# Woody5962/Ranked-List-Truncation

Hardware: AMD Instinct MI355X
Metric: ranked-lists/sec (fwd+bwd) at len=300; F1@k vs CPU ref (higher is better)
Workload: dtype f32 (operands, accumulation, storage); products by exact 3xbf16 split, 6 MFMA products, per-product error < 2^-23; 1 GPU; AttnCut + DivLoss(js,f1,augmented) [BASELINE configs[1]], batch 4096 lists/GPU x len 300, full train step incl. Adam and cut metrics; global_batch=4096, seq_len=300, parallelism=dp1

## Files before the change

### ranked-list-truncation_amd/csrc/attention6h.hip

```cpp
#include "attention_common.h"
#include "split6.h"
#include <stdlib.h>

namespace {

constexpr int KTH = 64;
constexpr int PLH = KTH * 64;
constexpr int IMGH = 3 * PLH;
constexpr int RECH = IMGH * 2;

__device__ __forceinline__ f32x4 mmh(bf16x8 a, bf16x8 b, f32x4 c) { return __builtin_amdgcn_mfma_f32_16x16x32_bf16(a, b, c, 0, 0, 0); }

__host__ __device__ inline int swz(int row) { return 2 * ((row >> 1) & 3); }

__host__ __device__ inline size_t a6h_img_block(int npair, int ntile) { return (size_t)npair * (ntile + 1) * RECH; }
__global__ __launch_bounds__(256) void attn6h_prepare_kernel(const float* __restrict__ src0, const float* __restrict__ src1, size_t ld,
                                                             int S, int B, int H, uint8_t* __restrict__ img0, uint8_t* __restrict__ img1) {
    const int tid = threadIdx.x, ntile = rlt_cdiv_dev(B, KTH);
    const int pair = blockIdx.x / (ntile + 1), tile = blockIdx.x % (ntile + 1);
    const int s_ = pair / H, h = pair % H;
    const float* base = (blockIdx.y ? src1 : src0) + (size_t)s_ * B * ld + h * 64;
    uint16_t* rec = reinterpret_cast<uint16_t*>((blockIdx.y ? img1 : img0) + ((size_t)pair * (ntile + 1) + tile) * RECH);
    const int r = tid >> 2, row = tile * KTH + r, c0 = 2 * (tid & 3);
    const bool ok = row < B;
    const float* p = base + (size_t)min(row, B - 1) * ld + 8 * c0;
#pragma unroll
    for (int u = 0; u < 2; ++u) {
        const float4 v0 = *reinterpret_cast<const float4*>(p + 8 * u), v1 = *reinterpret_cast<const float4*>(p + 8 * u + 4);
        const float x[8] = {ok ? v0.x : 0.f, ok ? v0.y : 0.f, ok ? v0.z : 0.f, ok ? v0.w : 0.f,
                            ok ? v1.x : 0.f, ok ? v1.y : 0.f, ok ? v1.z : 0.f, ok ? v1.w : 0.f};
        bf16x8 hh_, mm_, ll_;
        split8x3_by_pair(x, hh_, mm_, ll_);
        uint16_t* im = rec + r * 64 + ((c0 + u) ^ swz(r)) * 8;
        *reinterpret_cast<bf16x8*>(im) = hh_;
        *reinterpret_cast<bf16x8*>(im + PLH) = mm_;
        *reinterpret_cast<bf16x8*>(im + 2 * PLH) = ll_;
    }
}

#ifndef RLT_A6H_FWD1_BODY
#define RLT_A6H_FWD1_BODY "attention6h_fwd1_body.inc"
#define RLT_A6H_FWD1_BODY_DROP "attention6h_fwd1_body_drop.inc"
#endif
#ifdef RLT_A6H_STAMPS
__device__ unsigned long long a6h_stamps[4 * 4 * 18];
#define A6H_STAMP(k) do { if (blockIdx.x == 64 && lane == 0 && t >= 8 && t < 12) \
    a6h_stamps[(wv * 4 + (t - 8)) * 18 + (k)] = __builtin_amdgcn_s_memtime(); } while (0)
#else
#define A6H_STAMP(k) do { } while (0)
#endif

template <bool DROP>
__global__ __launch_bounds__(256, 1) void attn6h_fwd1_kernel(AttnArgs a) {
    constexpr int NB = 4;
    extern __shared__ __attribute__((aligned(16))) float smem[];
    uint16_t* img0 = reinterpret_cast<uint16_t*>(smem);
    uint32_t* htab = reinterpret_cast<uint32_t*>(img0 + 4 * IMGH);
    const int tid = threadIdx.x, lane = tid & 63, wv = tid >> 6;
    const int l15 = lane & 15, g = lane >> 4;
    const int B = a.B, H = a.H, E = H * 64;
    const size_t ld = (size_t)3 * E;
    int pair, rt;
    map_block(blockIdx.x, a.S * H, rlt_cdiv_dev(B, 256), pair, rt);
    const int s_ = pair / H, h = pair % H;
    const float* base = a.qkv + (size_t)s_ * B * ld + h * 64;
    const int row0 = rt * 256 + wv * 64;

    int offR[2], offT[4];
    {
        const int swr = swz(l15);
#pragma unroll
        for (int ks = 0; ks < 2; ++ks) offR[ks] = l15 * 64 + (((4 * ks + g) ^ swr) * 8);
        const int rowt = 4 * g + (l15 >> 2), swt = swz(rowt);
#pragma unroll
        for (int db = 0; db < 4; ++db) offT[db] = rowt * 64 + (((2 * db) ^ swt) + ((l15 & 3) >> 1)) * 8 + 4 * (l15 & 1);
    }
    bf16x8 sel[2];
    {
        uint32_t s0[2] = {0u, 0u};
        if ((l15 >> 2) == g) s0[(l15 & 3) >> 1] = (l15 & 1) ? 0xBF800000u : 0x0000BF80u;
        sel[0] = frag4(s0[0], s0[1], 0u, 0u);
        sel[1] = frag4(0u, 0u, s0[0], s0[1]);
    }

    bf16x8 qf[NB][3][2];
    f32x4 seed_s[NB], acc[NB][4], acc2[NB][4];
    float l_run[NB], m_ref[NB];
    uint32_t hq[NB];
    const uint32_t ps = DROP ? pair_seed(a.seed, pair) : 0u;
    const float inv_keep = DROP ? 1.f / (1.f - a.drop_p) : 1.f;
    const float qmul = a.scale * LOG2E;
#pragma unroll
    for (int n = 0; n < NB; ++n) {
        const int r = row0 + 16 * n + l15, rc = min(r, B - 1);
        hq[n] = DROP ? rlt_row_hash(ps, (uint32_t)r) : 0u;
        const float* qp = base + (size_t)rc * ld;
#pragma unroll
        for (int ks = 0; ks < 2; ++ks) {
            const float4 v0 = *reinterpret_cast<const float4*>(qp + 32 * ks + 8 * g), v1 = *reinterpret_cast<const float4*>(qp + 32 * ks + 8 * g + 4);
            const float x[8] = {v0.x * qmul, v0.y * qmul, v0.z * qmul, v0.w * qmul, v1.x * qmul, v1.y * qmul, v1.z * qmul, v1.w * qmul};
            split8x3_by_pair(x, qf[n][0][ks], qf[n][1][ks], qf[n][2][ks]);
        }
#pragma unroll
        for (int db = 0; db < 4; ++db) { acc[n][db] = f32x4{0.f, 0.f, 0.f, 0.f}; acc2[n][db] = f32x4{0.f, 0.f, 0.f, 0.f}; }
        l_run[n] = 0.f;
    }
    const int nt = B / KTH;
    const int npair = a.S * H;
    const uint8_t* rec0 = reinterpret_cast<const uint8_t*>(a.img) + ((size_t)0 * npair + pair) * (size_t)(nt + 1) * RECH;
    const uint8_t* rec1 = reinterpret_cast<const uint8_t*>(a.img) + ((size_t)1 * npair + pair) * (size_t)(nt + 1) * RECH;
    auto dma = [&](int j, int tile, uint16_t* ibuf) __attribute__((always_inline)) {
        const int q = j % 6, grp = q < 4 ? 0 : 4;
        const uint8_t* rec = (j < 6 ? rec0 : rec1) + (size_t)tile * RECH + (6 * wv + grp) * 1024 + lane * 16;
        if (q == grp) {
            const uint32_t dst = __builtin_amdgcn_readfirstlane(
                (uint32_t)(uintptr_t)(__attribute__((address_space(3))) uint8_t*)(reinterpret_cast<uint8_t*>(ibuf) + (j / 6) * RECH + (6 * wv + grp) * 1024));
            asm volatile("s_mov_b32 m0, %0\n\ts_nop 0" :: "s"(dst) : "memory");
        }
        asm volatile("global_load_lds_dwordx4 %0, off offset:%1" :: "v"(rec), "n"((q - grp) * 1024) : "memory");
    };
#pragma unroll
    for (int j = 0; j < 12; ++j) dma(j, 0, img0);
    if (DROP) htab[lane] = rlt_col_hash(ps, (uint32_t)lane);
    asm volatile("s_waitcnt vmcnt(0)" ::: "memory");
    __syncthreads();
#pragma unroll
    for (int n = 0; n < NB; ++n) {
        float tmax = -INFINITY;
#pragma unroll
        for (int kb = 0; kb < 2; ++kb) {
            f32x4 t = {0.f, 0.f, 0.f, 0.f};
#pragma unroll
            for (int p = 0; p < 6; ++p)
#pragma unroll
                for (int ks = 0; ks < 2; ++ks)
                    t = mmh(*reinterpret_cast<const bf16x8*>(img0 + x6_plane_a(p) * PLH + 16 * kb * 64 + offR[ks]), qf[n][x6_plane_b(p)][ks], t);
            tmax = fmaxf(fmaxf(fmaxf(t[0], t[1]), fmaxf(t[2], t[3])), tmax);
        }
        m_ref[n] = col_max4(tmax);
        seed_s[n] = f32x4{-m_ref[n], -m_ref[n], -m_ref[n], -m_ref[n]};
    }

    f32x4 sc[4][2];
    uint32_t pln[3][4][4];
    bf16x8 kf[2][3][2];
    v4s vt[3][4][2];
    uint4 hcv[2][2];
    hcv[0][0] = hcv[0][1] = hcv[1][0] = hcv[1][1] = make_uint4(0u, 0u, 0u, 0u);
#pragma unroll
    for (int i = 0; i < 4; ++i)
#pragma unroll
        for (int kb = 0; kb < 2; ++kb) sc[i][kb] = f32x4{0.f, 0.f, 0.f, 0.f};
#pragma unroll
    for (int i = 0; i < 3 * 4 * 4; ++i) (&pln[0][0][0])[i] = 0u;
#pragma unroll
    for (int i = 0; i < 12; ++i) (&kf[0][0][0])[i] = frag4(0u, 0u, 0u, 0u);
#pragma unroll
    for (int i = 0; i < 24; ++i) (&vt[0][0][0])[i] = v4s{0, 0, 0, 0};

    for (int t = 0; t <= nt; ++t) {
        const int cur = t & 1;
        const uint16_t* Ic = img0 + cur * 2 * IMGH;
        uint16_t* In = img0 + (cur ^ 1) * 2 * IMGH;
        const int t_next = min(t + 1, nt);
        const float livef = t < nt ? 1.f : 0.f;
        const float prevf = t > 0 ? 1.f : 0.f;
#pragma unroll
        for (int n = 0; n < NB; ++n) {
#pragma unroll
            for (int i = 0; i < 6; ++i) asm volatile("" : "+a"((&qf[n][0][0])[i]));
#pragma unroll
            for (int db = 0; db < 4; ++db) asm volatile("" : "+a"(acc[n][db]), "+a"(acc2[n][db]));
        }
        asm volatile("" : "+a"(sel[0]), "+a"(sel[1]));
#define GAP_END __builtin_amdgcn_sched_barrier(0)
        auto mma_va = [&](f32x4& d, bf16x8 av, bf16x8 bv) __attribute__((always_inline)) {
            asm volatile("v_mfma_f32_16x16x32_bf16 %0, %1, %2, %0" : "+v"(d) : "v"(av), "a"(bv));
        };
        auto mma_va_c = [&](f32x4& d, bf16x8 av, bf16x8 bv, const f32x4& cv) __attribute__((always_inline)) {
            asm volatile("v_mfma_f32_16x16x32_bf16 %0, %1, %2, %3" : "=&v"(d) : "v"(av), "a"(bv), "v"(cv));
        };
        auto mma_av = [&](f32x4& d, bf16x8 av, bf16x8 bv) __attribute__((always_inline)) {
            asm volatile("v_mfma_f32_16x16x32_bf16 %0, %1, %2, %0" : "+v"(d) : "a"(av), "v"(bv));
        };
        auto mma_out = [&](f32x4& d, bf16x8 av, bf16x8 bv) __attribute__((always_inline)) {
            asm volatile("v_mfma_f32_16x16x32_bf16 %0, %1, %2, %0" : "+a"(d) : "v"(av), "v"(bv));
        };
        auto m_s = [&](int it, int n, int k) __attribute__((always_inline)) {
            const int kb = k / 12, p = (k % 12) / 2, ks = k % 2;
            if (k % 12 == 0) mma_va_c(sc[it][kb], kf[kb][x6_plane_a(p)][ks], qf[n][x6_plane_b(p)][ks], seed_s[n]);
            else mma_va(sc[it][kb], kf[kb][x6_plane_a(p)][ks], qf[n][x6_plane_b(p)][ks]);
        };
        auto plane = [&](int lvl, int it) __attribute__((always_inline)) {
            return frag4(pln[lvl][it][0], pln[lvl][it][1], pln[lvl][it][2], pln[lvl][it][3]);
        };
        auto m_r = [&](int it, int which, int level, int kb) __attribute__((always_inline)) {
            mma_av(sc[it][kb], sel[kb], plane(level - 1, it));
        };
        auto m_o = [&](int it, int n, int which, int k) __attribute__((always_inline)) {
            const int p = k >> 2, db = k & 3;
            const v4s x = vt[x6_plane_a(p)][db][0], y = vt[x6_plane_a(p)][db][1];
            mma_out(p < 5 ? acc2[n][db] : acc[n][db], cat_frag(x, y), plane(x6_plane_b(p), it));
        };
        auto e_exp = [&](int it, int kb, int r) __attribute__((always_inline)) { sc[it][kb][r] = rlt_exp2(sc[it][kb][r]); };
        auto e_exp_p = [&](int it, int kb, int r) __attribute__((always_inline)) { sc[it][kb][r] = rlt_exp2(sc[it][kb][r]) * prevf; };
        auto e_sum = [&](int it, int n, int kb, int r) __attribute__((always_inline)) { l_run[n] = __builtin_fmaf(sc[it][kb][r], livef, l_run[n]); };
        auto e_sum_p = [&](int it, int n, int kb, int r) __attribute__((always_inline)) { l_run[n] += sc[it][kb][r]; };
        auto c_pk = [&](int it, int which, int lvl, int j) __attribute__((always_inline)) {
            const f32x4& tile = sc[it][j >> 1];
            pln[lvl][it][j] = pk2(tile[2 * (j & 1)], tile[2 * (j & 1) + 1]);
        };
        auto rd_row = [&](int mat, int kb, int pl, int ks, int b32) __attribute__((always_inline)) {
            kf[kb][pl][ks] = *reinterpret_cast<const bf16x8*>(Ic + pl * PLH + (32 * b32 + 16 * kb) * 64 + offR[ks]);
        };
        auto rd_tr = [&](int mat, int pl, int db, int half, int b32) __attribute__((always_inline)) {
            vt[pl][db][half] = tr_read(Ic + IMGH + pl * PLH + (32 * b32 + 16 * half) * 64 + offT[db]);
        };
        auto st_dma = [&](int j) __attribute__((always_inline)) { dma(j, t_next, In); };
        const uint32_t* Hc = htab + cur * KTH;
        auto rd_hc = [&](int fb, int kb, int b32) __attribute__((always_inline)) {
            hcv[fb][kb] = *reinterpret_cast<const uint4*>(Hc + 32 * b32 + 16 * kb + 4 * g);
        };
        auto st_hcol = [&]() __attribute__((always_inline)) {
            htab[(cur ^ 1) * KTH + lane] = rlt_col_hash(ps, (uint32_t)(t_next * KTH + lane));
        };
        auto e_drop = [&](int it, int n, int kb, int r, int fb) __attribute__((always_inline)) {
            const uint4& h4 = hcv[fb][kb];
            const uint32_t hc = r == 0 ? h4.x : r == 1 ? h4.y : r == 2 ? h4.z : h4.w;
            sc[it][kb][r] = rlt_keep_rc(hq[n], hc, a.drop_thr) ? sc[it][kb][r] * inv_keep : 0.f;
        };
        if constexpr (DROP) {
#include RLT_A6H_FWD1_BODY_DROP
        } else {
#include RLT_A6H_FWD1_BODY
        }
#undef GAP_END
        A6H_STAMP(16);
        asm volatile("s_waitcnt vmcnt(0)" ::: "memory");
        __syncthreads();
        A6H_STAMP(17);
    }
    bool bad = false;
    float inv[NB], lse[NB];
#pragma unroll
    for (int n = 0; n < NB; ++n) {
        const float l_tot = col_sum4(l_run[n]);
        bad |= !(l_tot > 0.f && l_tot <= 1.2676506e30f);
        inv[n] = 1.f / l_tot;
        lse[n] = (m_ref[n] + log2f(l_tot)) * LN2;
    }
    const int any_bad = __syncthreads_or(bad ? 1 : 0);
    if (tid == 0 && a.redo) a.redo[blockIdx.x] = any_bad ? 1u : 0u;
#pragma unroll
    for (int n = 0; n < NB; ++n) {
        const int q = row0 + 16 * n + l15;
        if (q < B) {
            float* orow = a.o + ((size_t)s_ * B + q) * E + h * 64 + 4 * g;
#pragma unroll
            for (int db = 0; db < 4; ++db) {
                const f32x4 o = acc[n][db] + acc2[n][db];
                *reinterpret_cast<float4*>(orow + 16 * db) = make_float4(o[0] * inv[n], o[1] * inv[n], o[2] * inv[n], o[3] * inv[n]);
            }
            if (g == 0) a.lse_o[((size_t)s_ * H + h) * B + q] = lse[n];
        }
    }
}

}

#ifdef RLT_A6H_STAMPS
extern "C" int rlt_debug_a6h_stamps(unsigned long long* out) {
    return (int)hipMemcpyFromSymbol(out, HIP_SYMBOL(a6h_stamps), sizeof(unsigned long long) * 4 * 4 * 18);
}
#endif

size_t rlt_attn6h_fwd_images_bytes(int S, int B, int H) { return 2 * a6h_img_block(S * H, rlt_cdiv(B, KTH)); }

int rlt_attn6h_prepare2(int what0, int slot0, int what1, int slot1, const AttnArgs& a, hipStream_t st) {
    const int npair = a.S * a.H, ntile = rlt_cdiv(a.B, KTH), E = a.H * 64;
    uint8_t* img = reinterpret_cast<uint8_t*>(const_cast<void*>(a.img));
    const size_t blk = a6h_img_block(npair, ntile);
    RLT_CHECK_ARG((what0 == 3) == (what1 == 3));
    const float* s0 = what0 == 3 ? a.dout : a.qkv + what0 * E;
    const float* s1 = what1 == 3 ? a.dout : a.qkv + what1 * E;
    hipLaunchKernelGGL(attn6h_prepare_kernel, dim3(npair * (ntile + 1), what1 == what0 && slot1 == slot0 ? 1 : 2), dim3(256), 0, st,
                       s0, s1, what0 == 3 ? (size_t)E : (size_t)3 * E, a.S, a.B, a.H, img + slot0 * blk, img + slot1 * blk);
    return RLT_LAUNCH_RESULT();
}

int rlt_attn6h_run(int which, const AttnArgs& a, hipStream_t st) {
    RLT_CHECK_ARG(which == 0 && a.img && a.redo && a.B % KTH == 0);
    const size_t shm = (size_t)4 * IMGH * sizeof(uint16_t) + 2 * KTH * sizeof(uint32_t);
    const dim3 grid(a.S * a.H * rlt_cdiv(a.B, 256));
    int rc;
    if (a.drop_p > 0.f) {
        if ((rc = rlt_allow_lds(attn6h_fwd1_kernel<true>, shm))) return rc;
        hipLaunchKernelGGL(attn6h_fwd1_kernel<true>, grid, dim3(256), shm, st, a);
    } else {
        if ((rc = rlt_allow_lds(attn6h_fwd1_kernel<false>, shm))) return rc;
        hipLaunchKernelGGL(attn6h_fwd1_kernel<false>, grid, dim3(256), shm, st, a);
    }
    return RLT_LAUNCH_RESULT();
}
```

### ranked-list-truncation_amd/csrc/attention_common.h

```cpp
#pragma once
#include "common.h"

struct AttnArgs {
    const float* qkv; const float* out; const float* dout; const float* lse; const float* delta;
    const void* img; const void* dimg;
    float* o; float* lse_o; float* dqkv;
    int S, B, H;
    float scale;
    float drop_p; uint32_t drop_thr, seed;
    uint32_t* redo;
};

#define RLT_DMA_ASM(dst, src)                                                                                         \
    do {                                                                                                              \
        uint32_t m0_keep_;                                                                                            \
        asm volatile("s_mov_b32 %0, m0\n\ts_mov_b32 m0, %1\n\ts_nop 0\n\tglobal_load_lds_dwordx4 %2, off\n\ts_mov_b32 m0, %0" \
                     : "=&s"(m0_keep_) : "s"(dst), "v"(src) : "memory");                                              \
    } while (0)

namespace {

constexpr int KT = 64;
constexpr int QT = 128;
constexpr float LOG2E = 1.4426950408889634f;
constexpr float LN2 = 0.6931471805599453f;


__device__ __forceinline__ uint32_t pair_seed(uint32_t seed, int pair) { return rlt_mix32(seed ^ ((uint32_t)pair * 0x9E3779B9U)); }

__device__ __forceinline__ void map_block(int bid, int npair, int ntile, int& pair, int& tile) {
    if ((npair & 7) == 0) {
        const int xcd = bid & 7, j = bid >> 3;
        pair = (j / ntile) * 8 + xcd;
        tile = j % ntile;
    } else {
        pair = bid / ntile;
        tile = bid % ntile;
    }
}

template <int HD>
__device__ __forceinline__ void store_acc_T(float* __restrict__ dst_row, int hh, const f32x16 (&acc)[(HD + 31) / 32],
                                            float mul) {
    constexpr int DT = (HD + 31) / 32;
#pragma unroll
    for (int dt = 0; dt < DT; ++dt)
#pragma unroll
        for (int g = 0; g < 4; ++g) {
            const int d0 = dt * 32 + 8 * g + 4 * hh;
            if (d0 < HD) {
                float4 v;
                v.x = acc[dt][4 * g + 0] * mul; v.y = acc[dt][4 * g + 1] * mul;
                v.z = acc[dt][4 * g + 2] * mul; v.w = acc[dt][4 * g + 3] * mul;
                *reinterpret_cast<float4*>(dst_row + d0) = v;
            }
        }
}


}

int rlt_attn_f32_run(int kernel, int which, const AttnArgs& a, int HD, hipStream_t st);
int rlt_attn_delta_run(const float* out, const float* dout, int S, int B, int H, int HD, float* delta, hipStream_t st);
int rlt_attn16_run(int which, const AttnArgs& a, hipStream_t st);
size_t rlt_attn3_images_bytes(int S, int B, int H, int HD, int nmat);
int rlt_attn3_run(int which, const AttnArgs& a, int HD, void* images, void* dimages, hipStream_t st);
size_t rlt_attn6_images_bytes(int S, int B, int H, int HD, int nmat);
int rlt_attn6_prepare(bool dO, const AttnArgs& a, int HD, hipStream_t st);
int rlt_attn6_run(int kernel, int which, const AttnArgs& a, int HD, hipStream_t st);
size_t rlt_attn6n_fwd_images_bytes(int S, int B, int H);
size_t rlt_attn6n_images_bytes(int S, int B, int H);
int rlt_attn6n_prepare_at(int what, int slot, const AttnArgs& a, hipStream_t st);
int rlt_attn6n_prepare(int what, const AttnArgs& a, hipStream_t st);
int rlt_attn6n_run(int kernel, int which, const AttnArgs& a, hipStream_t st);
size_t rlt_attn6h_fwd_images_bytes(int S, int B, int H);
int rlt_attn6h_prepare2(int what0, int slot0, int what1, int slot1, const AttnArgs& a, hipStream_t st);
int rlt_attn6h_run(int which, const AttnArgs& a, hipStream_t st);
```

### ranked-list-truncation_amd/csrc/attention_dispatch.hip

```cpp
#include "attention_plan.h"
#include "attention_common.h"
#include <stdlib.h>
#include <string.h>

namespace {

struct AttnEnv {
    int mode;
    bool attn6;
    bool attn6_img;
    bool attn16;
    bool a6n;
    bool a6n_1;
    bool a6n_img;
    bool a6n_f1;
    bool a6h;
    bool a6_pp;
    bool a6_dkv1;
    bool a6_dq1;
    bool attn_sb;
    bool attn_sb_dq;
    bool dkv_occ1;
};
const AttnEnv& attn_env() {
    static const AttnEnv env = [] {
        auto on = [](const char* e, bool dflt) { return e ? atoi(e) != 0 : dflt; };
        AttnEnv v;
        const char* m = getenv("RLT_ATTN_MODE");
        v.mode = !m ? -1 : (!strcmp(m, "bf16x3") || !strcmp(m, "1")) ? 1 : 0;
        v.attn6 = on(getenv("RLT_ATTN6"), true);
        v.attn6_img = on(getenv("RLT_ATTN6_IMG"), false);
        v.attn16 = on(getenv("RLT_ATTN16"), true);
        v.a6n = on(getenv("RLT_A6N"), true);
        v.a6n_1 = on(getenv("RLT_A6N_1"), true);
        v.a6n_img = on(getenv("RLT_A6N_IMG"), true);
        v.a6n_f1 = on(getenv("RLT_A6N_F1"), true);
        v.a6h = on(getenv("RLT_A6H"), true);
        v.a6_pp = on(getenv("RLT_A6_PP"), true);
        v.a6_dkv1 = on(getenv("RLT_A6_DKV1"), true);
        v.a6_dq1 = on(getenv("RLT_A6_DQ1"), true);
        v.attn_sb = on(getenv("RLT_ATTN_SB"), true);
        v.attn_sb_dq = getenv("RLT_ATTN_SB_DQ") != nullptr;
        const char* o = getenv("RLT_DKV_OCC");
        v.dkv_occ1 = o && atoi(o) == 1;
        return v;
    }();
    return env;
}

bool hd_ok(int HD) { return HD == 16 || HD == 32 || HD == 64 || HD == 128; }
bool drop_ok(float drop_p) { return drop_p >= 0.f && drop_p < 1.f; }
size_t delta_bytes(int S, int B, int H) { return ((size_t)S * H * B * sizeof(float) + 1023) / 1024 * 1024; }
size_t flags_bytes(int S, int B, int H) { return ((size_t)S * H * rlt_cdiv(B, 256) * sizeof(uint32_t) + 255) / 256 * 256; }

}

AttnPlan attn_plan(int S, int B, int H, int HD, float drop_p, bool have_images) {
    const AttnEnv& e = attn_env();
    const int prec = rlt_precision();
    const bool drop = drop_p > 0.f;
    const bool x3 = HD <= 64 && (e.mode >= 0 ? e.mode == 1 : prec == RLT_PRECISION_BF16X3);
    const bool x6 = HD <= 64 && e.mode < 0 && prec == RLT_PRECISION_BF16X6 && e.attn6;
    const bool staged = x6 && e.attn6_img;
    const bool pipe16 = x6 && !staged && HD == 16 && B >= 512 && !drop && e.a6n && e.a6n_1 && e.a6n_img;
    const bool pipe16_fwd = pipe16 && B % 128 == 0 && e.a6n_f1;
    const bool pipe64_fwd = x6 && !staged && HD == 64 && B >= 512 && B % 64 == 0 && e.a6h;

    AttnPlan p{};
    p.delta_bytes = delta_bytes(S, B, H);
    if (x3) {
        p.images_kind = RLT_ATTN_IMAGES_X3_QKV; p.images_bytes = rlt_attn3_images_bytes(S, B, H, HD, 3); p.images_retained = 1;
        p.ws_kind = RLT_ATTN_WS_X3_DO; p.ws_extra_bytes = rlt_attn3_images_bytes(S, B, H, HD, 1);
    } else if (staged) {
        p.images_kind = RLT_ATTN_IMAGES_X6_QKV; p.images_bytes = rlt_attn6_images_bytes(S, B, H, HD, 3); p.images_retained = 1;
        p.ws_kind = RLT_ATTN_WS_X6_DO; p.ws_extra_bytes = rlt_attn6_images_bytes(S, B, H, HD, 1);
    } else {
        if (pipe16_fwd || pipe64_fwd) {
            p.images_kind = pipe16_fwd ? RLT_ATTN_IMAGES_X6N_KV : RLT_ATTN_IMAGES_X6H_KV;
            p.flags_offset = pipe16_fwd ? rlt_attn6n_fwd_images_bytes(S, B, H) : rlt_attn6h_fwd_images_bytes(S, B, H);
            p.flags_bytes = flags_bytes(S, B, H);
            p.images_bytes = p.flags_offset + p.flags_bytes;
        }
        if (pipe16) { p.ws_kind = RLT_ATTN_WS_X6N_BLOCKS; p.ws_extra_bytes = rlt_attn6n_images_bytes(S, B, H); }
    }
    p.ws_bytes = p.delta_bytes + p.ws_extra_bytes;

    const int f32 = HD == 16 && e.attn16 ? RLT_ATTN_F32_HD16 : RLT_ATTN_F32;
    p.fwd = HD == 64 && e.attn_sb ? RLT_ATTN_F32_SB : f32;
    p.dkv = f32 == RLT_ATTN_F32 && (HD == 128 || e.dkv_occ1) ? RLT_ATTN_F32_OCC1 : f32;
    p.dq = HD == 64 && e.attn_sb && e.attn_sb_dq ? RLT_ATTN_F32_SB : f32;
    p.bwd_prepare = RLT_ATTN_PREP_DELTA;
    p.ws_prepare_bytes = p.delta_bytes;
    p.ws_part_bytes = have_images || !x3 ? p.ws_bytes : p.delta_bytes;
    if (x3 && have_images) {
        p.fwd = p.dkv = p.dq = RLT_ATTN_X3;
        p.fwd_prepare = RLT_ATTN_PREP_Q | RLT_ATTN_PREP_K | RLT_ATTN_PREP_V;
        p.bwd_prepare = RLT_ATTN_PREP_DELTA | RLT_ATTN_PREP_DO;
        p.ws_prepare_bytes = p.ws_bytes;
    } else if (x6) {
        const int two_w = staged && have_images ? RLT_ATTN_X6_IMG
                        : HD == 16 && e.a6n ? (B >= 512 ? RLT_ATTN_X6N_2W_SEEDED : RLT_ATTN_X6N_2W) : RLT_ATTN_X6;
        p.fwd = p.dkv = p.dq = two_w;
        if (two_w == RLT_ATTN_X6_IMG) {
            p.fwd_prepare = RLT_ATTN_PREP_Q | RLT_ATTN_PREP_K | RLT_ATTN_PREP_V;
            p.bwd_prepare |= RLT_ATTN_PREP_DO;
            p.ws_prepare_bytes = p.ws_bytes;
        }
        if (HD == 64) {
            const bool small24 = (long long)B * 3 * H * HD < (1ll << 24);
            if (e.a6_pp) p.fwd = two_w == RLT_ATTN_X6_IMG ? RLT_ATTN_X6_PP_IMG : RLT_ATTN_X6_PP;
            if (e.a6_dkv1 && small24) p.dkv = RLT_ATTN_X6_DKV1;
            if (e.a6_dq1 && small24) p.dq = RLT_ATTN_X6_DQ1;
        }
        if (pipe64_fwd && have_images) {
            p.fwd = RLT_ATTN_X6H_PIPE; p.fwd_fixup = RLT_ATTN_X6_PP; p.fwd_prepare = RLT_ATTN_PREP_K | RLT_ATTN_PREP_V;
        }
        if (pipe16_fwd && have_images) {
            p.fwd = RLT_ATTN_X6N_PIPE; p.fwd_fixup = RLT_ATTN_X6N_2W_SEEDED; p.fwd_prepare = RLT_ATTN_PREP_K | RLT_ATTN_PREP_V;
        }
        if (pipe16) {
            p.dkv = p.dq = RLT_ATTN_X6N_PIPE;
            p.bwd_prepare |= RLT_ATTN_PREP_DO | RLT_ATTN_PREP_SEEDS;
            p.dkv_prepare = RLT_ATTN_PREP_Q;
            p.dq_prepare = RLT_ATTN_PREP_K | RLT_ATTN_PREP_V;
            p.ws_prepare_bytes = p.ws_bytes;
        }
    }
    return p;
}

namespace {

int run_kernel(int kernel, int which, const AttnArgs& a, int HD, void* images, void* dimages, hipStream_t st) {
    switch (kernel) {
    case RLT_ATTN_F32: case RLT_ATTN_F32_SB: case RLT_ATTN_F32_OCC1: return rlt_attn_f32_run(kernel, which, a, HD, st);
    case RLT_ATTN_F32_HD16: return rlt_attn16_run(which, a, st);
    case RLT_ATTN_X3: return rlt_attn3_run(which, a, HD, images, dimages, st);
    case RLT_ATTN_X6: case RLT_ATTN_X6_IMG: case RLT_ATTN_X6_PP: case RLT_ATTN_X6_PP_IMG: case RLT_ATTN_X6_DKV1: case RLT_ATTN_X6_DQ1:
        return rlt_attn6_run(kernel, which, a, HD, st);
    case RLT_ATTN_X6N_2W: case RLT_ATTN_X6N_2W_SEEDED: case RLT_ATTN_X6N_PIPE: return rlt_attn6n_run(kernel, which, a, st);
    case RLT_ATTN_X6H_PIPE: return rlt_attn6h_run(which, a, st);
    }
    return RLT_E_ARG;
}

int bwd_prepare(const float* out, const float* dout, const float* lse, int S, int B, int H, int HD,
                const void* images, void* ws, size_t ws_bytes, float drop_p, void* stream) {
    RLT_CHECK_ARG(out && dout && lse && ws && S > 0 && B > 0 && H > 0 && drop_ok(drop_p));
    RLT_CHECK_SHAPE(hd_ok(HD));
    const AttnPlan p = attn_plan(S, B, H, HD, drop_p, images != nullptr);
    if (ws_bytes < p.ws_prepare_bytes) return RLT_E_WORKSPACE;
    if (!rlt_aligned16(ws)) return RLT_E_ALIGN;
    hipStream_t st = rlt_stream(stream);
    uint8_t* extra = (uint8_t*)ws + p.delta_bytes;
    AttnArgs a{};
    a.dout = dout; a.lse = lse; a.delta = (const float*)ws; a.S = S; a.B = B; a.H = H;
    if (p.dkv == RLT_ATTN_X3) {
        a.o = const_cast<float*>(out);
        a.drop_p = drop_p;
        return rlt_attn3_run(3, a, HD, nullptr, extra, st);
    }
    int rc = rlt_attn_delta_run(out, dout, S, B, H, HD, (float*)ws, st);
    if (!rc && (p.bwd_prepare & RLT_ATTN_PREP_DO)) {
        if (p.ws_kind == RLT_ATTN_WS_X6_DO) { a.dimg = extra; rc = rlt_attn6_prepare(true, a, HD, st); }
        else { a.img = extra; rc = rlt_attn6n_prepare(3, a, st); }
    }
    if (!rc && (p.bwd_prepare & RLT_ATTN_PREP_SEEDS)) rc = rlt_attn6n_prepare(4, a, st);
    return rc;
}

int bwd_part(int which, const float* qkv, const float* dout, const float* lse, const void* images, void* ws, size_t ws_bytes,
             int S, int B, int H, int HD, float drop_p, uint32_t seed, float* dqkv, void* stream) {
    RLT_CHECK_ARG(qkv && dout && lse && ws && dqkv && S > 0 && B > 0 && H > 0 && drop_ok(drop_p));
    RLT_CHECK_SHAPE(hd_ok(HD));
    if (!(rlt_aligned16(qkv) && rlt_aligned16(dout) && rlt_aligned16(dqkv) && rlt_aligned16(ws))) return RLT_E_ALIGN;
    const AttnPlan p = attn_plan(S, B, H, HD, drop_p, images != nullptr);
    if (ws_bytes < p.ws_part_bytes) return RLT_E_WORKSPACE;
    const int kernel = which == 1 ? p.dkv : p.dq, prepare = which == 1 ? p.dkv_prepare : p.dq_prepare;
    uint8_t* extra = (uint8_t*)ws + p.delta_bytes;
    AttnArgs a{};
    a.qkv = qkv; a.dout = dout; a.lse = lse; a.delta = (const float*)ws; a.dqkv = dqkv;
    a.S = S; a.B = B; a.H = H;
    a.scale = 1.0f / sqrtf((float)HD);
    a.drop_p = drop_p; a.drop_thr = rlt_drop_threshold(drop_p); a.seed = seed;
    if (kernel == RLT_ATTN_X6_IMG) { a.img = images; a.dimg = extra; }
    if (kernel == RLT_ATTN_X6N_PIPE) a.img = extra;
    hipStream_t st = rlt_stream(stream);
    int rc = 0;
    for (int what = 0; what < 3 && !rc; ++what)
        if (prepare & (1 << what)) rc = rlt_attn6n_prepare(what, a, st);
    return rc ? rc : run_kernel(kernel, which, a, HD, const_cast<void*>(images), extra, st);
}

}

extern "C" {

int rlt_list_attention_plan(int S, int B, int H, int HD, float drop_p, int have_images, int precision, rlt_attention_plan* out) {
    RLT_PREC_SCOPE(precision);
    RLT_CHECK_ARG(out && S > 0 && B > 0 && H > 0 && drop_ok(drop_p));
    RLT_CHECK_SHAPE(hd_ok(HD));
    *out = attn_plan(S, B, H, HD, drop_p, have_images != 0);
    return 0;
}

size_t rlt_list_attention_fwd_workspace(int S, int B, int H, int HD, float drop_p, int precision) {
    RLT_PREC_SCOPE_SZ(precision);
    if (S <= 0 || B <= 0 || H <= 0 || !hd_ok(HD)) return 0;
    return attn_plan(S, B, H, HD, drop_p, true).images_bytes;
}

int rlt_list_attention_images_retained(int S, int B, int H, int HD, int precision) {
    RLT_PREC_SCOPE_SZ(precision);
    if (S <= 0 || B <= 0 || H <= 0 || !hd_ok(HD)) return 0;
    return attn_plan(S, B, H, HD, 0.f, true).images_retained;
}

int rlt_list_attention_fwd(const float* qkv, int S, int B, int H, int HD, float drop_p, uint32_t seed,
                           float* out, float* lse, void* images, size_t images_bytes, int precision, void* stream) {
    RLT_PREC_SCOPE(precision);
    RLT_CHECK_ARG(qkv && out && lse && S > 0 && B > 0 && H > 0 && drop_ok(drop_p));
    RLT_CHECK_SHAPE(hd_ok(HD));
    if (!(rlt_aligned16(qkv) && rlt_aligned16(out))) return RLT_E_ALIGN;
    AttnPlan p = attn_plan(S, B, H, HD, drop_p, images != nullptr);
    if (p.fwd_prepare && p.images_retained) {
        if (images_bytes < p.images_bytes) return RLT_E_WORKSPACE;
        if (!rlt_aligned16(images)) return RLT_E_ALIGN;
    } else if (p.fwd_prepare && !(rlt_aligned16(images) && images_bytes >= p.images_bytes)) {
        p = attn_plan(S, B, H, HD, drop_p, false);
    }
    AttnArgs a{};
    a.qkv = qkv; a.o = out; a.lse_o = lse; a.S = S; a.B = B; a.H = H;
    a.scale = 1.0f / sqrtf((float)HD);
    a.drop_p = drop_p; a.drop_thr = rlt_drop_threshold(drop_p); a.seed = seed;
    if (p.fwd_prepare) a.img = images;
    if (p.fwd_fixup) a.redo = reinterpret_cast<uint32_t*>(reinterpret_cast<uint8_t*>(images) + p.flags_offset);
    hipStream_t st = rlt_stream(stream);
    int rc = 0;
    switch (p.fwd) {
    case RLT_ATTN_X6_IMG: case RLT_ATTN_X6_PP_IMG: rc = rlt_attn6_prepare(false, a, HD, st); break;
    case RLT_ATTN_X6N_PIPE: rc = rlt_attn6n_prepare_at(1, 0, a, st); if (!rc) rc = rlt_attn6n_prepare_at(2, 1, a, st); break;
    case RLT_ATTN_X6H_PIPE: rc = rlt_attn6h_prepare2(1, 0, 2, 1, a, st); break;
    }
    if (!rc) rc = run_kernel(p.fwd, 0, a, HD, images, nullptr, st);
    if (!rc && p.fwd_fixup) rc = run_kernel(p.fwd_fixup, 0, a, HD, nullptr, nullptr, st);
    return rc;
}

size_t rlt_list_attention_bwd_workspace(int S, int B, int H, int HD, float drop_p, int precision) {
    RLT_PREC_SCOPE_SZ(precision);
    if (S <= 0 || B <= 0 || H <= 0 || !hd_ok(HD)) return 0;
    return attn_plan(S, B, H, HD, drop_p, true).ws_bytes;
}

int rlt_list_attention_bwd_prepare(const float* out, const float* dout, const float* lse, int S, int B, int H, int HD, float drop_p,
                                   const void* images, void* ws, size_t ws_bytes, int precision, void* stream) {
    RLT_PREC_SCOPE(precision);
    return bwd_prepare(out, dout, lse, S, B, H, HD, images, ws, ws_bytes, drop_p, stream);
}

int rlt_list_attention_bwd_dkv(const float* qkv, const float* dout, const float* lse, const void* images, void* ws, size_t ws_bytes,
                               int S, int B, int H, int HD, float drop_p, uint32_t seed, float* dqkv, int precision, void* stream) {
    RLT_PREC_SCOPE(precision);
    return bwd_part(1, qkv, dout, lse, images, ws, ws_bytes, S, B, H, HD, drop_p, seed, dqkv, stream);
}

int rlt_list_attention_bwd_dq(const float* qkv, const float* dout, const float* lse, const void* images, void* ws, size_t ws_bytes,
                              int S, int B, int H, int HD, float drop_p, uint32_t seed, float* dqkv, int precision, void* stream) {
    RLT_PREC_SCOPE(precision);
    return bwd_part(2, qkv, dout, lse, images, ws, ws_bytes, S, B, H, HD, drop_p, seed, dqkv, stream);
}

int rlt_list_attention_bwd(const float* qkv, const float* out, const float* dout, const float* lse,
                           int S, int B, int H, int HD, float drop_p, uint32_t seed, const void* images, float* dqkv,
                           void* ws, size_t ws_bytes, int precision, void* stream) {
    RLT_PREC_SCOPE(precision);
    RLT_CHECK_ARG(drop_ok(drop_p));
    int rc = bwd_prepare(out, dout, lse, S, B, H, HD, images, ws, ws_bytes, drop_p, stream);
    if (!rc) rc = bwd_part(1, qkv, dout, lse, images, ws, ws_bytes, S, B, H, HD, drop_p, seed, dqkv, stream);
    if (!rc) rc = bwd_part(2, qkv, dout, lse, images, ws, ws_bytes, S, B, H, HD, drop_p, seed, dqkv, stream);
    return rc;
}

}
```

### ranked-list-truncation_amd/csrc/gemm.hip

```cpp
#include "common.h"
#include "gemm6s.h"
#include "gemm_plan.h"
#include "split6.h"
#include <type_traits>

namespace {

constexpr int BM = 128, BN = 128, LDT = 132;

struct GemmArgs {
    const float* A; const float* B; float* C;
    const float* bias; const float* bias2;
    int M, N, K, lda, ldb, ldc;
    int vecA, vecB;
    int flags;
    int kchunk;
    float* slab;
    int tiles_m, tiles_n;
    const float* mask; int ldmask;
    float* colsum;
    float* cs_slab;
    float drop_p; uint32_t drop_thr, seed;
    float mask_scale;
    int slab_xcd;
// ... 1414 lines not shown
            vals6e<BKC>(vb, p, a, b, c, d);
            split4x3<true>(a, b, c, d, hi, mid, lo);
            *reinterpret_cast<uint2*>(wb + dB[p]) = hi;
            *reinterpret_cast<uint2*>(wb + dB[p] + HB6) = mid;
            *reinterpret_cast<uint2*>(wb + dB[p] + 2 * HB6) = lo;
        }
    };
    bf16x8 a[4][3], b[2][3];
    auto frag_a = [&](const uint16_t* base, int i, int q) { a[i][q] = *reinterpret_cast<const bf16x8*>(base + arow + q * HB6 + i * 32 * 16); };
    auto frag_b = [&](const uint16_t* base, int j, int q) { b[j & 1][q] = *reinterpret_cast<const bf16x8*>(base + brow + q * HB6 + j * 32 * 16); };

    {
        const float* pa = srcA(0); const float* pb = srcB(0);
#pragma unroll
        for (int i = 0; i < 4; ++i) { load6e<AKC>(pa, g.lda, i, ra[0][i]); load6e<BKC>(pb, g.ldb, i, rb[0][i]); }
        pa = srcA(1); pb = srcB(1);
#pragma unroll
        for (int i = 0; i < 4; ++i) { load6e<AKC>(pa, g.lda, i, ra[1][i]); load6e<BKC>(pb, g.ldb, i, rb[1][i]); }
        if (want_cs) { add_cs(ra[0]); add_cs(ra[1]); }
        stash_all(lds, ra[0], rb[0]);
        stash_all(lds + KB6, ra[1], rb[1]);
        if (PERSIST) decode_next();
        pa = srcA(2); pb = srcB(2);
#pragma unroll
        for (int i = 0; i < 4; ++i) { load6e<AKC>(pa, g.lda, i, ra[0][i]); load6e<BKC>(pb, g.ldb, i, rb[0][i]); }
        pa = srcA(3); pb = srcB(3);
#pragma unroll
        for (int i = 0; i < 4; ++i) { load6e<AKC>(pa, g.lda, i, ra[1][i]); load6e<BKC>(pb, g.ldb, i, rb[1][i]); }
    }
    __syncthreads();
#pragma unroll
    for (int q = 0; q < 3; ++q) { frag_a(lds, 0, q); frag_a(lds, 1, q); frag_b(lds, 0, q); }

    auto slot = [&](auto par_tag, int buf, int wbuf, int nbuf, const float* pa, const float* pb) {
        constexpr int PAR = decltype(par_tag)::value;
        const uint16_t* base = lds + buf * KB6;
        const uint16_t* nbase = lds + nbuf * KB6;
        uint16_t* wb = lds + wbuf * KB6;
        Split6 su;
#define GAP_END __builtin_amdgcn_sched_barrier(0)
#define MM(i_, j_, k_) acc[(i_) >> 1][(i_) & 1][j_] = __builtin_amdgcn_mfma_f32_32x32x16_bf16( \
            a[i_][(k_) == 0 || (k_) == 3 ? 1 : (k_) == 1 ? 2 : 0], b[(j_) & 1][(k_) == 0 || (k_) == 4 ? 1 : (k_) == 2 ? 2 : 0], acc[(i_) >> 1][(i_) & 1][j_], 0, 0, 0)
#define SP(p_, k_) do { float x0_, x1_, x2_, x3_; \
            if ((p_) < 4) vals6e<AKC>(ra[PAR], (p_) & 3, x0_, x1_, x2_, x3_); else vals6e<BKC>(rb[PAR], (p_) & 3, x0_, x1_, x2_, x3_); \
            split6_part(su, x0_, x1_, x2_, x3_, k_); } while (0)
#define ST(p_) do { const int d_ = (p_) < 4 ? dA[(p_) & 3] : dB[(p_) & 3]; \
            *reinterpret_cast<uint2*>(wb + d_) = su.hi; *reinterpret_cast<uint2*>(wb + d_ + HB6) = su.mid; \
            *reinterpret_cast<uint2*>(wb + d_ + 2 * HB6) = su.lo; \
            if ((p_) < 4) { if (AKC) load6e<AKC>(pa, g.lda, (p_) & 3, ra[PAR][(p_) & 3]); \
                            else if ((p_) == 3) { for (int i_ = 0; i_ < 4; ++i_) load6e<AKC>(pa, g.lda, i_, ra[PAR][i_]); } } \
            else { if (BKC) load6e<BKC>(pb, g.ldb, (p_) & 3, rb[PAR][(p_) & 3]); \
                   else if ((p_) == 7) { for (int i_ = 0; i_ < 4; ++i_) load6e<BKC>(pb, g.ldb, i_, rb[PAR][i_]); } } } while (0)
#define RA(i_, q_, n_) frag_a((n_) ? nbase : base, i_, q_)
#define RB(j_, q_, n_) frag_b((n_) ? nbase : base, j_, q_)
#include "gemm6e_slot.inc"
#undef GAP_END
#undef MM
#undef SP
#undef ST
#undef RA
#undef RB
    };

    int u = 0;
    while (true) {
        for (int s = 0; s < nks; s += 2) {
            const int u1 = u == 2 ? 0 : u + 1, u2 = u1 == 2 ? 0 : u1 + 1;
            if (want_cs && s + 2 < nks) add_cs(ra[0]);
            slot(std::integral_constant<int, 0>{}, u, u2, u1, srcA(s + 4), srcB(s + 4));
            __syncthreads();
            if (want_cs && s + 3 < nks) add_cs(ra[1]);
            slot(std::integral_constant<int, 1>{}, u1, u, u2, srcA(s + 5), srcB(s + 5));
            __syncthreads();
            u = u2;
        }
        write_output_simple<4>(g, acc[0], m0 + wm * 128, n0 + wn * 128, l31, hh, zslab);
        write_output_simple<4>(g, acc[1], m0 + wm * 128 + 64, n0 + wn * 128, l31, hh, zslab);
        if (!PERSIST || !has_next) break;
        m0 = nm0; n0 = nn0;
        decode_next();
#pragma unroll
        for (int i = 0; i < 4; ++i)
#pragma unroll
            for (int j = 0; j < 4; ++j)
#pragma unroll
                for (int r = 0; r < 16; ++r) acc[i >> 1][i & 1][j][r] = 0.f;
    }
    if (want_cs) {
        float4* red = reinterpret_cast<float4*>(gsm);
        __syncthreads();
        red[tid] = csum;
        __syncthreads();
        if (tid < 64) {
            float4 t = red[4 * tid];
#pragma unroll
            for (int j = 1; j < 4; ++j) {
                const float4 o = red[4 * tid + j];
                t.x += o.x; t.y += o.y; t.z += o.z; t.w += o.w;
            }
            float* dst = (g.cs_slab ? g.cs_slab + (size_t)zslab * g.M : g.colsum) + m0 + 4 * tid;
            dst[0] = t.x; dst[1] = t.y; dst[2] = t.z; dst[3] = t.w;
        }
    }
}

__device__ __forceinline__ float4 f4add(float4 a, float4 b) { return make_float4(a.x + b.x, a.y + b.y, a.z + b.z, a.w + b.w); }
__global__ __launch_bounds__(256) void splitk_reduce_kernel(GemmArgs g, int nsplit) {
    const size_t mn = (size_t)g.M * g.N;
    const size_t stride = (size_t)gridDim.x * 256;
    if ((g.N & 3) == 0) {
        const float4* slab4 = reinterpret_cast<const float4*>(g.slab);
        const size_t mn4 = mn / 4;
        for (size_t i = (size_t)blockIdx.x * 256 + threadIdx.x; i < mn4; i += stride) {
            float4 a0 = make_float4(0.f, 0.f, 0.f, 0.f), a1 = a0, a2 = a0, a3 = a0;
            int z = 0;
            for (; z + 3 < nsplit; z += 4) {
                a0 = f4add(a0, slab4[(size_t)z * mn4 + i]);
                a1 = f4add(a1, slab4[(size_t)(z + 1) * mn4 + i]);
                a2 = f4add(a2, slab4[(size_t)(z + 2) * mn4 + i]);
                a3 = f4add(a3, slab4[(size_t)(z + 3) * mn4 + i]);
            }
            for (; z < nsplit; ++z) a0 = f4add(a0, slab4[(size_t)z * mn4 + i]);
            const float4 v4 = f4add(f4add(a0, a1), f4add(a2, a3));
            const float v[4] = {v4.x, v4.y, v4.z, v4.w};
            const int row = (int)((4 * i) / g.N), col0 = (int)(4 * i - (size_t)row * g.N);
#pragma unroll
            for (int e = 0; e < 4; ++e) {
                const int col = col0 + e;
                float bv = 0.f;
                if (g.bias) bv += g.bias[col];
                if (g.bias2) bv += g.bias2[col];
                float* dst = g.C + (size_t)row * g.ldc + col;
                *dst = gemm_epilogue(g, v[e], bv, row, col, dst);
            }
        }
    } else {
        for (size_t i = (size_t)blockIdx.x * 256 + threadIdx.x; i < mn; i += stride) {
            float v = 0.f;
            for (int z = 0; z < nsplit; ++z) v += g.slab[(size_t)z * mn + i];
            const int row = (int)(i / g.N), col = (int)(i - (size_t)row * g.N);
            float bv = 0.f;
            if (g.bias) bv += g.bias[col];
            if (g.bias2) bv += g.bias2[col];
            float* dst = g.C + (size_t)row * g.ldc + col;
            *dst = gemm_epilogue(g, v, bv, row, col, dst);
        }
    }
    if (g.cs_slab)
        for (size_t i = (size_t)blockIdx.x * 256 + threadIdx.x; i < (size_t)g.M; i += stride) {
            float c0 = 0.f, c1 = 0.f, c2 = 0.f, c3 = 0.f;
            int z = 0;
            for (; z + 3 < nsplit; z += 4) {
                c0 += g.cs_slab[(size_t)z * g.M + i];
                c1 += g.cs_slab[(size_t)(z + 1) * g.M + i];
                c2 += g.cs_slab[(size_t)(z + 2) * g.M + i];
                c3 += g.cs_slab[(size_t)(z + 3) * g.M + i];
            }
            for (; z < nsplit; ++z) c0 += g.cs_slab[(size_t)z * g.M + i];
            g.colsum[i] = (c0 + c1) + (c2 + c3);
        }
}

#if defined(RLT_STAMPS)
extern "C" int rlt_debug_g6c_stamps(unsigned long long* host, size_t n) {
    return (int)hipMemcpyFromSymbol(host, HIP_SYMBOL(rlt_g6c_stamp_buf), n * sizeof(unsigned long long));
}
extern "C" int rlt_debug_gemm_stamps(unsigned long long* host, size_t n) {
    return (int)hipMemcpyFromSymbol(host, HIP_SYMBOL(rlt_gemm_stamp_buf), n * sizeof(unsigned long long));
}
#endif

constexpr int CS_ROWS_PER_WG = 512;
__global__ __launch_bounds__(256) void colsum_partial_kernel(const float* __restrict__ X, int ldx, int T, int N,
                                                             float* __restrict__ partial) {
    const int col = blockIdx.x * 64 + (threadIdx.x & 63);
    const int rphase = threadIdx.x >> 6;
    const int r0 = blockIdx.y * CS_ROWS_PER_WG, r1 = min(T, r0 + CS_ROWS_PER_WG);
    float acc = 0.f;
    if (col < N)
        for (int r = r0 + rphase; r < r1; r += 4) acc += X[(size_t)r * ldx + col];
    __shared__ float sm[4][64];
    sm[rphase][threadIdx.x & 63] = acc;
    __syncthreads();
    if (threadIdx.x < 64 && col < N)
        partial[(size_t)blockIdx.y * N + col] = sm[0][threadIdx.x] + sm[1][threadIdx.x] + sm[2][threadIdx.x] + sm[3][threadIdx.x];
}
__global__ __launch_bounds__(256) void segment_colsum_kernel(const float* __restrict__ X, int ldx, int R, int N,
                                                             float* __restrict__ out, int ldo, int accumulate) {
    const int g = blockIdx.x;
    const int lane = threadIdx.x & 63, rphase = threadIdx.x >> 6;
    __shared__ float sm[4][64];
    for (int c0 = 0; c0 < N; c0 += 64) {
        const int col = c0 + lane;
        float acc = 0.f;
        if (col < N)
            for (int r = rphase; r < R; r += 4) acc += X[((size_t)g * R + r) * ldx + col];
        sm[rphase][lane] = acc;
        __syncthreads();
        if (threadIdx.x < 64 && col < N) {
            const float v = sm[0][lane] + sm[1][lane] + sm[2][lane] + sm[3][lane];
            float* dst = out + (size_t)g * ldo + col;
            *dst = accumulate ? *dst + v : v;
        }
        __syncthreads();
    }
}

__global__ __launch_bounds__(256) void relu_bwd_kernel(float* __restrict__ dX, const float* __restrict__ Y, size_t n) {
    for (size_t i = (size_t)blockIdx.x * 256 + threadIdx.x; i < n; i += (size_t)gridDim.x * 256)
        if (!(Y[i] > 0.f)) dX[i] = 0.f;
}
__global__ __launch_bounds__(256) void scale_kernel(float* __restrict__ x, const float* __restrict__ s, size_t n) {
    const float f = s[0];
    for (size_t i = (size_t)blockIdx.x * 256 + threadIdx.x; i < n; i += (size_t)gridDim.x * 256) x[i] *= f;
}

constexpr int NDW_CHUNKS = 2048;
__global__ __launch_bounds__(256) void narrow_dw_partial_kernel(const float* __restrict__ A, int lda, const float* __restrict__ X,
                                                                int ldx, int I, int T, int M, int rows_per_wg,
                                                                float* __restrict__ partial) {
    const int m4 = blockIdx.y * 256 + threadIdx.x;
    const int t0 = blockIdx.x * rows_per_wg, t1 = min(T, t0 + rows_per_wg);
    float4 a0 = make_float4(0.f, 0.f, 0.f, 0.f), a1 = a0, a2 = a0, ab = a0;
    if (4 * m4 < M) {
        const float* ap = A + 4 * m4;
        for (int t = t0; t < t1; ++t) {
            const float4 v = *reinterpret_cast<const float4*>(ap + (size_t)t * lda);
            const float* xr = X + (size_t)t * ldx;
            const float x0 = xr[0], x1 = I > 1 ? xr[1] : 0.f, x2 = I > 2 ? xr[2] : 0.f;
            a0.x += v.x * x0; a0.y += v.y * x0; a0.z += v.z * x0; a0.w += v.w * x0;
            a1.x += v.x * x1; a1.y += v.y * x1; a1.z += v.z * x1; a1.w += v.w * x1;
            a2.x += v.x * x2; a2.y += v.y * x2; a2.z += v.z * x2; a2.w += v.w * x2;
            ab.x += v.x; ab.y += v.y; ab.z += v.z; ab.w += v.w;
        }
        float* pr = partial + (size_t)blockIdx.x * 4 * M + 4 * m4;
        *reinterpret_cast<float4*>(pr) = a0;
        *reinterpret_cast<float4*>(pr + M) = a1;
        *reinterpret_cast<float4*>(pr + 2 * M) = a2;
        *reinterpret_cast<float4*>(pr + 3 * M) = ab;
    }
}
__global__ __launch_bounds__(256) void narrow_dw_scatter_kernel(const float* __restrict__ sums, int M, int I,
                                                                float* __restrict__ dW, float* __restrict__ db) {
    const int m = blockIdx.x * 256 + threadIdx.x;
    if (m >= M) return;
    for (int f = 0; f < I; ++f) dW[(size_t)m * I + f] = sums[(size_t)f * M + m];
    if (db) db[m] = sums[(size_t)3 * M + m];
}

int ew_grid(size_t n) { size_t g = (n + 1023) / 1024; return (int)(g < 1 ? 1 : (g > 4096 ? 4096 : g)); }

constexpr bool family_is(int family, int bm, int bn, size_t lds) {
    return GEMM_FAMILY[family].bm == bm && GEMM_FAMILY[family].bn == bn && GEMM_FAMILY[family].lds == lds;
}
static_assert(family_is(RLT_GEMM_F32, BM, BN, (size_t)4 * 16 * LDT * sizeof(float)) &&
              family_is(RLT_GEMM_3, BM, BN, (size_t)2 * 4 * TILE3 * sizeof(uint16_t)) &&
              family_is(RLT_GEMM_3B, BM2, BN2, (size_t)2 * 4 * PL2 * sizeof(uint16_t)) &&
              family_is(RLT_GEMM_6, BM6, BN6, (size_t)2 * BUF6 * sizeof(uint16_t)) &&
              family_is(RLT_GEMM_6B, BM2, BN2, (size_t)6 * PL2 * sizeof(uint16_t)) &&
              family_is(RLT_GEMM_6C, BM2, BN2, (size_t)3 * KB6 * sizeof(uint16_t)) &&
              family_is(RLT_GEMM_6E, BM2, BN2, (size_t)3 * KB6 * sizeof(uint16_t)), "gemm_plan.h: GEMM_FAMILY");

template <typename F>
int with_layout(bool ta, bool tb, F f) {
    if (ta) return tb ? f(BoolTag<true>{}, BoolTag<true>{}) : f(BoolTag<true>{}, BoolTag<false>{});
    return tb ? f(BoolTag<false>{}, BoolTag<true>{}) : f(BoolTag<false>{}, BoolTag<false>{});
}

thread_local rlt_gemm_dispatch rlt_gemm_dispatch_rec = {};

template <typename Kern>
int launch(Kern kern, const GemmPlan& p, const GemmArgs& g, hipStream_t st) {
    const int rc = rlt_allow_lds(kern, p.lds_bytes);
    if (rc) return rc;
    rlt_gemm_dispatch_rec = p.d;
    hipLaunchKernelGGL(kern, dim3(p.grid_x, 1, p.grid_z), dim3(p.wg), p.lds_bytes, st, g);
    return RLT_LAUNCH_RESULT();
}

}

extern "C" {

int rlt_gemm_last_dispatch(rlt_gemm_dispatch* out) {
    RLT_CHECK_ARG(out);
    *out = rlt_gemm_dispatch_rec;
    return 0;
}

int rlt_gemm(int ta, int tb, int M, int N, int K,
             const float* A, int lda, const float* B, int ldb, float* C, int ldc,
             const float* bias, const float* bias2, int flags,
             void* ws, size_t ws_bytes, int precision, void* stream) {
    RLT_PREC_SCOPE(precision);
    return rlt_gemm_ex(ta, tb, M, N, K, A, lda, B, ldb, C, ldc, bias, bias2, flags, nullptr, 0, 1.0f, nullptr,
                       0.0f, 0u, ws, ws_bytes, RLT_PRECISION_DEFAULT, stream);
}

static int gemm_run(int ta, int tb, int M, int N, int K,
                    const float* A, int lda, const float* B, int ldb, float* C, int ldc,
                    const float* bias, const float* bias2, int flags,
                    const float* relu_mask, int ldmask, float mask_scale, float* colsum_a,
                    float drop_p, uint32_t seed, uint32_t* bits_out, const uint32_t* bits_in,
                    void* ws, size_t ws_bytes, void* stream) {
    rlt_gemm_dispatch_rec = rlt_gemm_dispatch{};
    RLT_CHECK_ARG(A && B && C && M > 0 && N > 0 && K > 0);
    RLT_CHECK_ARG(lda >= (ta ? M : K) && ldb >= (tb ? K : N) && ldc >= N);
    RLT_CHECK_ARG(!relu_mask || ldmask >= N);
    RLT_CHECK_ARG(!colsum_a || ta);
    RLT_CHECK_ARG(drop_p >= 0.f && drop_p < 1.f);

    GemmCall c{};
    c.ta = ta; c.tb = tb; c.M = M; c.N = N; c.K = K; c.lda = lda; c.ldb = ldb; c.ldc = ldc; c.flags = flags;
    auto bit = [](bool on, int b) { return on ? b : 0; };
    c.aligned16 = bit(rlt_aligned16(A), RLT_GEMM_PTR_A) | bit(rlt_aligned16(B), RLT_GEMM_PTR_B) | bit(rlt_aligned16(C), RLT_GEMM_PTR_C) |
                  bit(rlt_aligned16(bias), RLT_GEMM_PTR_BIAS) | bit(rlt_aligned16(bias2), RLT_GEMM_PTR_BIAS2) |
                  bit(rlt_aligned16(bits_out), RLT_GEMM_PTR_BITS_OUT) | bit(rlt_aligned16(bits_in), RLT_GEMM_PTR_BITS_IN);
    c.present = bit(bias, RLT_GEMM_PTR_BIAS) | bit(bias2, RLT_GEMM_PTR_BIAS2) | bit(bits_out, RLT_GEMM_PTR_BITS_OUT) |
                bit(bits_in, RLT_GEMM_PTR_BITS_IN) | bit(relu_mask, RLT_GEMM_PTR_RELU_MASK) | bit(colsum_a, RLT_GEMM_PTR_COLSUM);
    c.drop = drop_p > 0.f; c.ws_null = ws == nullptr; c.ws_bytes = ws_bytes;

    const GemmPlan p = gemm_plan(c);
    if (p.rc) return p.rc;

    hipStream_t st = rlt_stream(stream);
    if (p.d.family == RLT_GEMM_6S) {
        const Gemm6sArgs s6{A, B, C, bias, bias2, M, N, K, lda, ldb, ldc, bits_out, bits_in, mask_scale};
        const int rc = rlt_gemm6s_launch(s6, p, &rlt_gemm_dispatch_rec, st);
        return rc ? rc : RLT_LAUNCH_RESULT();
    }
    const int ns = p.d.ns;
    GemmArgs g;
    g.mask = relu_mask; g.ldmask = ldmask; g.colsum = colsum_a;
    g.bits_out = bits_out; g.bits_in = bits_in; g.ldbits = N;
    g.mask_scale = mask_scale; g.drop_p = drop_p; g.drop_thr = rlt_drop_threshold(drop_p); g.seed = seed;
    g.A = A; g.B = B; g.C = C; g.bias = bias; g.bias2 = bias2;
    g.M = M; g.N = N; g.K = K; g.lda = lda; g.ldb = ldb; g.ldc = ldc;
    g.vecA = (lda % 4 == 0) && rlt_aligned16(A);
    g.vecB = (ldb % 4 == 0) && rlt_aligned16(B);
    g.flags = flags;
    g.tiles_m = p.tiles_m; g.tiles_n = p.tiles_n;
    g.kchunk = p.d.kchunk;
    g.slab_xcd = p.d.slab_xcd;
    g.slab = ns > 1 ? (float*)ws : nullptr;
    g.cs_slab = (ns > 1 && colsum_a) ? (float*)ws + (size_t)ns * M * N : nullptr;
    const int rc = with_layout(ta, tb, [&](auto TA, auto TB) {
        constexpr bool A_ = decltype(TA)::value, B_ = decltype(TB)::value;
        auto go = [&](auto kern) { return launch(kern, p, g, st); };
        const bool persistent = !A_ && p.d.persistent;
        switch (p.d.family) {
        case RLT_GEMM_6E:
            if constexpr (!A_) if (persistent) return go(gemm6e_kernel<A_, B_, true>);
            return go(gemm6e_kernel<A_, B_, false>);
        case RLT_GEMM_6C:
            if constexpr (!A_) if (persistent) return go(gemm6c_kernel<A_, B_, true>);
            return go(gemm6c_kernel<A_, B_, false>);
        case RLT_GEMM_3B:
            if constexpr (!A_) if (persistent) return go(gemm3b_kernel<A_, B_, true>);
            return go(gemm3b_kernel<A_, B_>);
        case RLT_GEMM_6B: return go(gemm6b_kernel<A_, B_>);
        case RLT_GEMM_6: return go(gemm6_kernel<A_, B_>);
        case RLT_GEMM_3: return p.d.fast ? go(gemm3_kernel<A_, B_, true>) : go(gemm3_kernel<A_, B_, false>);
        case RLT_GEMM_F32: return p.d.fast ? go(gemm_kernel<A_, B_, 16, 4, true>) : go(gemm_kernel<A_, B_, 16, 4, false>);
        }
        return (int)RLT_E_ARG;
    });
    if (rc) return rc;
    if (p.reduce)
        hipLaunchKernelGGL(splitk_reduce_kernel, dim3(ew_grid((size_t)M * N)), dim3(256), 0, st, g, ns);
    return RLT_LAUNCH_RESULT();
}

int rlt_gemm_ex(int ta, int tb, int M, int N, int K,
                const float* A, int lda, const float* B, int ldb, float* C, int ldc,
                const float* bias, const float* bias2, int flags,
                const float* relu_mask, int ldmask, float mask_scale, float* colsum_a,
                float drop_p, uint32_t seed,
                void* ws, size_t ws_bytes, int precision, void* stream) {
    RLT_PREC_SCOPE(precision);
    return gemm_run(ta, tb, M, N, K, A, lda, B, ldb, C, ldc, bias, bias2, flags, relu_mask, ldmask, mask_scale, colsum_a,
                    drop_p, seed, nullptr, nullptr, ws, ws_bytes, stream);
}

size_t rlt_gemm_bits_words(int M, int N) { return M > 0 && N > 0 ? (size_t)rlt_cdiv(M, 32) * N : 0; }

int rlt_gemm_bits(int ta, int tb, int M, int N, int K,
                  const float* A, int lda, const float* B, int ldb, float* C, int ldc,
                  const float* bias, int flags, float drop_p, uint32_t seed,
                  uint32_t* relu_bits_out, const uint32_t* mask_bits_in, float mask_scale,
                  int precision, void* stream) {
    RLT_PREC_SCOPE(precision);
    RLT_CHECK_ARG((relu_bits_out != nullptr) != (mask_bits_in != nullptr));
    RLT_CHECK_ARG(!relu_bits_out || (flags & RLT_GEMM_RELU));
    RLT_CHECK_ARG(drop_p == 0.f || relu_bits_out);
    RLT_CHECK_SHAPE(N % 32 == 0);
    return gemm_run(ta, tb, M, N, K, A, lda, B, ldb, C, ldc, bias, nullptr, flags, nullptr, 0, mask_scale, nullptr,
                    drop_p, seed, relu_bits_out, mask_bits_in, nullptr, 0, stream);
}

size_t rlt_colsum_workspace(int T, int N) {
    if (T <= 0 || N <= 0) return 0;
    return (size_t)rlt_cdiv(T, CS_ROWS_PER_WG) * N * sizeof(float);
}

int rlt_colsum(const float* X, int ldx, int T, int N, float* out, int accumulate,
               void* ws, size_t ws_bytes, void* stream) {
    RLT_CHECK_ARG(X && out && ws && T > 0 && N > 0 && ldx >= N);
    if (ws_bytes < rlt_colsum_workspace(T, N)) return RLT_E_WORKSPACE;
    const int nchunk = rlt_cdiv(T, CS_ROWS_PER_WG);
    hipStream_t st = rlt_stream(stream);
    hipLaunchKernelGGL(colsum_partial_kernel, dim3(rlt_cdiv(N, 64), nchunk), dim3(256), 0, st, X, ldx, T, N, (float*)ws);
    hipLaunchKernelGGL(rlt_rows_reduce_kernel, dim3(rlt_cdiv(N, 16)), dim3(256), 0, st, (const float*)ws, nchunk, N, N, N, out, out, accumulate);
    return RLT_LAUNCH_RESULT();
}

int rlt_segment_colsum(const float* X, int ldx, int G, int R, int N, float* out, int ldo,
                       int accumulate, void* stream) {
    RLT_CHECK_ARG(X && out && G > 0 && R > 0 && N > 0 && ldx >= N && ldo >= N);
    hipLaunchKernelGGL(segment_colsum_kernel, dim3(G), dim3(256), 0, rlt_stream(stream), X, ldx, R, N, out, ldo, accumulate);
    return RLT_LAUNCH_RESULT();
}

size_t rlt_narrow_dw_workspace(int T, int M) {
    if (T <= 0 || M <= 0) return 0;
    const int rows = rlt_cdiv(T, NDW_CHUNKS);
    const int nchunk = rlt_cdiv(T, rows);
    return ((size_t)nchunk * 4 * M + (size_t)4 * M) * sizeof(float);
}

int rlt_narrow_dw(const float* A, int lda, const float* X, int ldx, int I, int T, int M,
                  float* dW, float* db, void* ws, size_t ws_bytes, void* stream) {
    RLT_CHECK_ARG(A && X && dW && ws && T > 0 && M > 0 && lda >= M && ldx >= I);
    RLT_CHECK_SHAPE(I >= 1 && I <= 3 && M % 4 == 0 && lda % 4 == 0);
    if (!rlt_aligned16(A)) return RLT_E_ALIGN;
    if (ws_bytes < rlt_narrow_dw_workspace(T, M)) return RLT_E_WORKSPACE;
    const int rows = rlt_cdiv(T, NDW_CHUNKS);
    const int nchunk = rlt_cdiv(T, rows);
    float* partial = (float*)ws;
    float* sums = partial + (size_t)nchunk * 4 * M;
    hipStream_t st = rlt_stream(stream);
    hipLaunchKernelGGL(narrow_dw_partial_kernel, dim3(nchunk, rlt_cdiv(M, 1024)), dim3(256), 0, st, A, lda, X, ldx, I, T, M, rows, partial);
    hipLaunchKernelGGL(rlt_rows_reduce_kernel, dim3(rlt_cdiv(4 * M, 16)), dim3(256), 0, st, (const float*)partial, nchunk, 4 * M,
                       4 * M, 4 * M, sums, sums, 0);
    hipLaunchKernelGGL(narrow_dw_scatter_kernel, dim3(rlt_cdiv(M, 256)), dim3(256), 0, st, (const float*)sums, M, I, dW, db);
    return RLT_LAUNCH_RESULT();
}

int rlt_relu_bwd(float* dX, const float* Y, size_t n, void* stream) {
    RLT_CHECK_ARG(dX && Y && n > 0);
    hipLaunchKernelGGL(relu_bwd_kernel, dim3(ew_grid(n)), dim3(256), 0, rlt_stream(stream), dX, Y, n);
    return RLT_LAUNCH_RESULT();
}

int rlt_scale(float* x, const float* scale, size_t n, void* stream) {
    RLT_CHECK_ARG(x && scale && n > 0);
    hipLaunchKernelGGL(scale_kernel, dim3(ew_grid(n)), dim3(256), 0, rlt_stream(stream), x, scale, n);
    return RLT_LAUNCH_RESULT();
}

}
```

### ranked-list-truncation_amd/csrc/gemm6s.h

```cpp
#pragma once
#include <stddef.h>
#include <stdint.h>
#include <hip/hip_runtime.h>
#include "gemm_plan.h"

struct Gemm6sArgs {
    const float* A; const float* B; float* C;
    const float* bias; const float* bias2;
    int M, N, K, lda, ldb, ldc;
    uint32_t* bits_out;
    const uint32_t* bits_in;
    float mask_scale;
};
int rlt_gemm6s_launch(const Gemm6sArgs& g, const GemmPlan& p, rlt_gemm_dispatch* rec, hipStream_t st);
```

### ranked-list-truncation_amd/csrc/gemm6s.hip

```cpp
#include "common.h"
#include "gemm6s.h"
#include "split6.h"
#include <type_traits>

namespace {

typedef unsigned int u32x4 __attribute__((ext_vector_type(4)));

template <int KS> constexpr int gs_rowb() { return 64 * KS; }
template <int KS> constexpr int gs_plane() { return 32 * gs_rowb<KS>(); }
template <int KS> constexpr int gs_buf() { return 3 * gs_plane<KS>(); }
template <int KS> constexpr int gs_wl() { return KS > 4 ? 4 * 4 * (KS - 4) * 64 * 16 : 0; }
template <int KS> constexpr size_t gs_lds() { return (size_t)2 * gs_buf<KS>() + gs_wl<KS>(); }
static_assert(gs_lds<8>() == 160 * 1024, "the K = 256 streaming product fills LDS exactly");

__device__ __forceinline__ __amdgpu_buffer_rsrc_t rsrc_s(const void* p, uint32_t bytes) {
    return __builtin_amdgcn_make_buffer_rsrc(const_cast<void*>(p), 0, bytes, 0x00020000);
}

template <int KS, int NCB, bool TB, int EPI>
__global__ __launch_bounds__(256, 1) void gemm6s_kernel(Gemm6sArgs g) {
    static_assert(NCB == 4 || (NCB == 2 && KS == 4 && EPI < 2), "128-column panels: K = 128, plain epilogues");
    constexpr int PW = 64 * NCB, WC = 16 * NCB;
    constexpr int GS_PLANE = gs_plane<KS>(), GS_BUF = gs_buf<KS>(), ROWB = gs_rowb<KS>(), CPR = 4 * KS, RPP = 256 / CPR, NI = 32 / RPP;
    extern __shared__ __attribute__((aligned(16))) uint8_t sm6s[];
    const int tid = threadIdx.x, lane = tid & 63, w = __builtin_amdgcn_readfirstlane(tid >> 6), n = lane & 15, q = lane >> 4;
    const int npanel = g.N / PW;
    const int panel = __builtin_amdgcn_readfirstlane(blockIdx.x % npanel), stream = __builtin_amdgcn_readfirstlane(blockIdx.x / npanel),
              nstream = __builtin_amdgcn_readfirstlane(gridDim.x / npanel);
    const int nblk = (g.M + 31) / 32;
    uint4* wl_s = reinterpret_cast<uint4*>(sm6s + 2 * GS_BUF);
    (void)wl_s;

    bf16x8 wh[NCB][KS], wm[NCB][KS], wlv[NCB][4];
    f32x4 bv[NCB];
#pragma unroll
    for (int pass = 0; pass < 2; ++pass) {
#pragma unroll
        for (int cb = 0; cb < NCB; ++cb) {
            const int col = PW * panel + WC * w + 16 * cb + n;
            const float* wp = TB ? g.B + (size_t)col * g.ldb + 8 * q : g.B + (size_t)(8 * q) * g.ldb + col;
#pragma unroll
            for (int ks = 0; ks < (pass ? 4 : KS); ++ks) {
                asm volatile("" : "+v"(wp));
                float v[8];
                if (TB) {
                    const float4 v0 = *reinterpret_cast<const float4*>(wp + 32 * ks), v1 = *reinterpret_cast<const float4*>(wp + 32 * ks + 4);
                    v[0] = v0.x; v[1] = v0.y; v[2] = v0.z; v[3] = v0.w; v[4] = v1.x; v[5] = v1.y; v[6] = v1.z; v[7] = v1.w;
                } else {
#pragma unroll
                    for (int j = 0; j < 8; ++j) v[j] = wp[(size_t)(32 * ks + j) * g.ldb];
                }
                uint2 h0, m0, l0, h1, m1, l1;
                split4x3<true>(v[0], v[1], v[2], v[3], h0, m0, l0);
                split4x3<true>(v[4], v[5], v[6], v[7], h1, m1, l1);
                if (pass == 0) {
                    wh[cb][ks] = frag4(h0.x, h0.y, h1.x, h1.y);
                    wm[cb][ks] = frag4(m0.x, m0.y, m1.x, m1.y);
                    asm volatile("" : "+a"(wh[cb][ks]), "+a"(wm[cb][ks]) : : "memory");
                    if (KS > 4 && ks >= 4) wl_s[((w * 4 + cb) * (KS - 4) + (ks - 4)) * 64 + lane] = make_uint4(l0.x, l0.y, l1.x, l1.y);
                } else {
                    wlv[cb][ks] = frag4(l0.x, l0.y, l1.x, l1.y);
                    asm volatile("" : "+v"(wlv[cb][ks]) : : "memory");
                }
            }
            if (pass == 0) {
                const int c4 = PW * panel + WC * w + 16 * cb + 4 * q;
                f32x4 b = {0.f, 0.f, 0.f, 0.f};
                if (g.bias) { const float4 t = *reinterpret_cast<const float4*>(g.bias + c4); b += f32x4{t.x, t.y, t.z, t.w}; }
                if (g.bias2) { const float4 t = *reinterpret_cast<const float4*>(g.bias2 + c4); b += f32x4{t.x, t.y, t.z, t.w}; }
                bv[cb] = b;
            }
        }
    }

    const int sc = tid % CPR, sr = tid / CPR;
    const uint32_t voff_a = (uint32_t)sr * g.lda * 4u + sc * 32u;
    uint32_t wro[NI];
#pragma unroll
    for (int i = 0; i < NI; ++i) wro[i] = (uint32_t)(sr + RPP * i) * ROWB + 16u * (sc ^ ((sr + RPP * i) & 15));
    uint32_t rdo[4];
#pragma unroll
    for (int j = 0; j < 4; ++j) rdo[j] = n * ROWB + 64u * (j ^ (n >> 2)) + 16u * (q ^ (n & 3));
    const uint8_t* wlrd = sm6s + 2 * GS_BUF + w * (4 * (KS - 4) * 1024) + lane * 16;
    const uint32_t voff_c = (uint32_t)n * g.ldc * 4u + ((uint32_t)WC * w + 4u * q) * 4u;
    const uint32_t voff_bo = lane < 16 ? ((uint32_t)WC * w + lane) * 4u : 0x7fff0000u;
    const uint32_t voff_bi = ((uint32_t)WC * w + 4u * q) * 4u;
    uint32_t bm[5];
#pragma unroll
    for (int r = 0; r < 4; ++r) bm[r] = (lane & 3) == r ? 0xffffffffu : 0u;
    bm[4] = ((lane >> 2) & 3) < 2 ? 0xffffffffu : 0u;
    const uint32_t bsh = 16u * ((lane >> 2) & 1);
#pragma unroll
    for (int r = 0; r < 5; ++r) asm volatile("" : "+v"(bm[r]));

    auto blk_of = [&](int i) { return stream + i * nstream; };
    auto rows_of = [&](int i) { const int r = g.M - 32 * blk_of(i); return __builtin_amdgcn_readfirstlane(i < 0 ? 0 : r < 0 ? 0 : r > 32 ? 32 : r); };
    auto rs_a = [&](int i) { return rsrc_s(g.A + (size_t)(i < 0 ? 0 : blk_of(i)) * 32 * g.lda, (uint32_t)rows_of(i) * g.lda * 4u); };
    auto rs_bits = [&](int i) {
        const uint32_t* base = EPI == 2 ? g.bits_out : g.bits_in;
        return rsrc_s(base + (size_t)(i < 0 ? 0 : blk_of(i)) * g.N + PW * panel, rows_of(i) > 0 ? (uint32_t)PW * 4u : 0u);
    };
    auto rs_c = [&](int i) { return rsrc_s(g.C + (size_t)(i < 0 ? 0 : blk_of(i)) * 32 * g.ldc + PW * panel, (uint32_t)rows_of(i) * g.ldc * 4u); };
    const int nb = __builtin_amdgcn_readfirstlane(stream < nblk ? (nblk - stream + nstream - 1) / nstream : 0);

    f32x4 acc[2][NCB], xs[2 * NI];
    u32x4 bw[NCB];
    bf16x8 bfr[2][3], lfr[NCB];
    uint4 sph, spm, spl;
    const f32x4 z4 = {0.f, 0.f, 0.f, 0.f};
#pragma unroll
    for (int i = 0; i < 2 * NCB; ++i) { acc[i / NCB][i % NCB] = z4; }
#pragma unroll
    for (int i = 0; i < 2 * NI; ++i) xs[i] = z4;
#pragma unroll
    for (int i = 0; i < 6; ++i) (&bfr[0][0])[i] = frag4(0u, 0u, 0u, 0u);
#pragma unroll
    for (int i = 0; i < NCB; ++i) lfr[i] = frag4(0u, 0u, 0u, 0u);
    sph = spm = spl = make_uint4(0u, 0u, 0u, 0u);
#pragma unroll
    for (int cb = 0; cb < NCB; ++cb) bw[cb] = u32x4{0u, 0u, 0u, 0u};
    auto load_x = [&](int i4, int part, __amdgpu_buffer_rsrc_t r) __attribute__((always_inline)) {
        xs[2 * i4 + part] = __builtin_bit_cast(f32x4, __builtin_amdgcn_raw_buffer_load_b128(r, voff_a + 16u * part, (uint32_t)(RPP * i4) * g.lda * 4u, 0));
    };
    auto split_x = [&](int i4, int part) __attribute__((always_inline)) {
        f32x4 &a = xs[2 * i4], &b = xs[2 * i4 + 1];
        if (part == 0) { sph = make_uint4(pk2(a[0], a[1]), pk2(a[2], a[3]), pk2(b[0], b[1]), pk2(b[2], b[3])); asm("" : "+v"(sph.x), "+v"(sph.y), "+v"(sph.z), "+v"(sph.w)); }
        if (part == 1) { a[0] -= lo16(sph.x); a[1] -= hi16(sph.x); a[2] -= lo16(sph.y); a[3] -= hi16(sph.y); }
        if (part == 2) { b[0] -= lo16(sph.z); b[1] -= hi16(sph.z); b[2] -= lo16(sph.w); b[3] -= hi16(sph.w); }
        if (part == 3) { spm = make_uint4(pk2(a[0], a[1]), pk2(a[2], a[3]), pk2(b[0], b[1]), pk2(b[2], b[3])); asm("" : "+v"(spm.x), "+v"(spm.y), "+v"(spm.z), "+v"(spm.w)); }
        if (part == 4) { a[0] -= lo16(spm.x); a[1] -= hi16(spm.x); a[2] -= lo16(spm.y); a[3] -= hi16(spm.y); }
        if (part == 5) { b[0] -= lo16(spm.z); b[1] -= hi16(spm.z); b[2] -= lo16(spm.w); b[3] -= hi16(spm.w); }
        if (part == 6) spl = make_uint4(pk2(a[0], a[1]), pk2(a[2], a[3]), pk2(b[0], b[1]), pk2(b[2], b[3]));
    };
    auto write_x = [&](int buf, int i4, int pl) __attribute__((always_inline)) {
        *reinterpret_cast<uint4*>(sm6s + buf * GS_BUF + pl * GS_PLANE + wro[i4]) = pl == 0 ? sph : pl == 1 ? spm : spl;
    };
    {
        const __amdgpu_buffer_rsrc_t r0 = rs_a(0), r1 = rs_a(1);
#pragma unroll
        for (int i4 = 0; i4 < NI; ++i4) { load_x(i4, 0, r0); load_x(i4, 1, r0); }
#pragma unroll
        for (int i4 = 0; i4 < NI; ++i4) {
#pragma unroll
            for (int part = 0; part < 7; ++part) split_x(i4, part);
#pragma unroll
            for (int pl = 0; pl < 3; ++pl) write_x(0, i4, pl);
            load_x(i4, 0, r1);
            load_x(i4, 1, r1);
        }
#pragma unroll
        for (int i = 0; i < 2 * NI; ++i) asm volatile("" : "+v"(xs[i]));
    }
    __syncthreads();

#define GAP_END __builtin_amdgcn_sched_barrier(0)
    auto tick = [&](auto XC, int i) __attribute__((always_inline)) {
        constexpr int X = decltype(XC)::value, Y = 1 - X;
        const __amdgpu_buffer_rsrc_t rc0 = rs_c(i), rc1 = rs_c(i - 1), ra2 = rs_a(i + 2);
        const __amdgpu_buffer_rsrc_t rb0 = EPI >= 2 ? rs_bits(i) : rc0, rb1 = EPI == 2 ? rs_bits(i - 1) : rc1;
        (void)rb0; (void)rb1;
        auto RB = [&](int half, int ks, int pl) __attribute__((always_inline)) {
            bfr[(KS * half + ks) & 1][pl] = *reinterpret_cast<const bf16x8*>(sm6s + X * GS_BUF + pl * GS_PLANE + half * 16 * ROWB + 256 * (ks >> 2) + rdo[ks & 3]);
        };
        auto RL = [&](int ks, int cb) __attribute__((always_inline)) { lfr[cb] = *reinterpret_cast<const bf16x8*>(wlrd + 1024 * ((KS - 4) * cb + ks - 4)); };
        auto MG = [&](int half, int ks, int p, int cb, int first) __attribute__((always_inline)) {
            const int bp = p == 2 ? 2 : (p == 0 || p == 4) ? 1 : 0;
            const bf16x8 xv = bfr[(KS * half + ks) & 1][bp];
            f32x4& d = acc[half][cb];
            if (p == 1) {
                const bf16x8 lv = ks < 4 ? wlv[cb][ks < 4 ? ks : 0] : lfr[cb];
                asm volatile("v_mfma_f32_16x16x32_bf16 %0, %1, %2, %0" : "+v"(d) : "v"(lv), "v"(xv));
            } else {
                const bf16x8 av = (p == 0 || p == 3) ? wm[cb][ks] : wh[cb][ks];
                const f32x4 seed = bv[cb];
                if (first) asm volatile("v_mfma_f32_16x16x32_bf16 %0, %1, %2, %3" : "+v"(d) : "a"(av), "v"(xv), "v"(seed));
                else asm volatile("v_mfma_f32_16x16x32_bf16 %0, %1, %2, %0" : "+v"(d) : "a"(av), "v"(xv));
            }
        };
        auto EP = [&](int half, int cb) __attribute__((always_inline)) {
            f32x4 v = acc[half][cb];
            if (EPI == 3) {
                const uint32_t sh = 16 * half + n;
#pragma unroll
                for (int r = 0; r < 4; ++r) v[r] = ((bw[cb][r] >> sh) & 1u) ? v[r] * g.mask_scale : 0.f;
                if (half == 1) bw[cb] = __builtin_amdgcn_raw_buffer_load_b128(rb0, voff_bi + 64u * cb, 0, 0);
            }
            if (EPI == 1 || EPI == 2) v = f32x4{fmaxf(v[0], 0.f), fmaxf(v[1], 0.f), fmaxf(v[2], 0.f), fmaxf(v[3], 0.f)};
            if (EPI == 2) {
                const uint64_t b0 = __builtin_amdgcn_ballot_w64(v[0] > 0.f), b1 = __builtin_amdgcn_ballot_w64(v[1] > 0.f),
                               b2 = __builtin_amdgcn_ballot_w64(v[2] > 0.f), b3 = __builtin_amdgcn_ballot_w64(v[3] > 0.f);
                const uint32_t lo = ((uint32_t)b0 & bm[0]) | ((uint32_t)b1 & bm[1]) | ((uint32_t)b2 & bm[2]) | ((uint32_t)b3 & bm[3]);
                const uint32_t hi = ((uint32_t)(b0 >> 32) & bm[0]) | ((uint32_t)(b1 >> 32) & bm[1]) | ((uint32_t)(b2 >> 32) & bm[2]) | ((uint32_t)(b3 >> 32) & bm[3]);
                const uint32_t piece = ((lo & bm[4]) | (hi & ~bm[4])) >> bsh;
                __builtin_amdgcn_raw_buffer_store_b16((short)piece, half ? rb1 : rb0, voff_bo + 64u * cb + 2u * half, 0, 0);
            }
            __builtin_amdgcn_raw_buffer_store_b128(__builtin_bit_cast(u32x4, v), half ? rc1 : rc0, voff_c + 64u * cb, (uint32_t)(16 * half) * g.ldc * 4u, 0);
        };
        auto SX = [&](int i4, int part) __attribute__((always_inline)) { split_x(i4, part); };
        auto LX = [&](int i4, int part) __attribute__((always_inline)) { load_x(i4, part, ra2); };
        auto WX = [&](int i4, int pl) __attribute__((always_inline)) { write_x(Y, i4, pl); };
        RB(0, 0, 0); RB(0, 0, 1); RB(0, 0, 2);
        GAP_END;
        if constexpr (KS == 8) {
#include "gemm6s_body.inc"
        } else if constexpr (NCB == 4) {
#include "gemm6s_k128_body.inc"
        } else {
#include "gemm6s_k128n128_body.inc"
        }
        asm volatile("s_waitcnt lgkmcnt(0)\n\ts_barrier" ::: "memory");
    };
    const std::integral_constant<int, 0> H0;
    const std::integral_constant<int, 1> H1;
    for (int i = 0; i < nb + 1; i += 2) {
#pragma unroll
        for (int cb = 0; cb < NCB; ++cb)
#pragma unroll
            for (int k4 = 0; k4 < KS; k4 += 4)
                asm volatile("" : "+a"(wh[cb][k4]), "+a"(wh[cb][k4 + 1]), "+a"(wh[cb][k4 + 2]), "+a"(wh[cb][k4 + 3]), "+a"(wm[cb][k4]), "+a"(wm[cb][k4 + 1]),
                             "+a"(wm[cb][k4 + 2]), "+a"(wm[cb][k4 + 3]));
        tick(H0, i);
        tick(H1, i + 1);
    }
#undef GAP_END
}

}

static_assert(gs_lds<8>() == GEMM6S_LDS_K256 && gs_lds<4>() == GEMM6S_LDS_K128, "gemm_plan.h: the LDS bytes of the streaming kernels");

int rlt_gemm6s_launch(const Gemm6sArgs& g, const GemmPlan& p, rlt_gemm_dispatch* rec, hipStream_t st) {
    const int epi = p.d.epilogue;
    auto go = [&](auto kern) {
        const int rc = rlt_allow_lds(kern, p.lds_bytes);
        if (rc) return rc;
        *rec = p.d;
        hipLaunchKernelGGL(kern, dim3(p.grid_x), dim3(p.wg), p.lds_bytes, st, g);
        return 0;
    };
    auto by_epilogue = [&](auto KS, auto TB) {
        constexpr int KS_ = decltype(KS)::value;
        constexpr bool TB_ = decltype(TB)::value;
        return epi == 3 ? go(gemm6s_kernel<KS_, 4, TB_, 3>) : epi == 2 ? go(gemm6s_kernel<KS_, 4, TB_, 2>)
             : epi == 1 ? go(gemm6s_kernel<KS_, 4, TB_, 1>) : go(gemm6s_kernel<KS_, 4, TB_, 0>);
    };
    const std::integral_constant<int, 8> K256;
    const std::integral_constant<int, 4> K128;
    const bool k256 = p.d.kchunk == 256;
    if (p.d.narrow)
        return p.d.tb ? (epi ? go(gemm6s_kernel<4, 2, true, 1>) : go(gemm6s_kernel<4, 2, true, 0>))
                      : (epi ? go(gemm6s_kernel<4, 2, false, 1>) : go(gemm6s_kernel<4, 2, false, 0>));
    if (p.d.tb) return k256 ? by_epilogue(K256, std::true_type{}) : by_epilogue(K128, std::true_type{});
    return k256 ? by_epilogue(K256, std::false_type{}) : by_epilogue(K128, std::false_type{});
}
```

### ranked-list-truncation_amd/csrc/gemm_plan.h

```cpp
#pragma once
#include <stddef.h>
#include "../../include/rlt_hip.h"

typedef rlt_gemm_call GemmCall;

struct GemmPlan {
    int rc;
    rlt_gemm_dispatch d;
    int tiles_m, tiles_n;
    unsigned grid_x, grid_z, wg;
    size_t lds_bytes;
    bool reduce;
    size_t ws_bytes;
};
GemmPlan gemm_plan(const GemmCall& c);

struct GemmFamily { int bm, bn, wg; size_t lds; };
constexpr GemmFamily GEMM_FAMILY[] = {
    {0, 0, 0, 0},
    {128, 128, 256, 4 * 16 * 132 * 4},
    {128, 128, 256, 2 * 4 * 128 * 40 * 2},
    {256, 256, 512, 2 * 4 * 256 * 32 * 2},
    {256, 128, 512, 2 * 3 * (256 + 128) * 32 * 2},
    {256, 256, 512, 6 * 256 * 32 * 2},
    {256, 256, 512, 3 * 6 * 256 * 16 * 2},
    {256, 256, 256, 3 * 6 * 256 * 16 * 2},
    {32, 256, 256, 0},
};
constexpr size_t GEMM6S_LDS_K256 = 160 * 1024, GEMM6S_LDS_K128 = 48 * 1024;
```

### ranked-list-truncation_amd/csrc/gemm_plan.hip

```cpp
#define RLT_HOST_ONLY
#include "gemm_plan.h"
#include "common.h"
#include <stdlib.h>
#include <string.h>

namespace {

struct GemmEnv {
    int mode;
    bool nofast;
    bool no_big;
    int persist;
    bool persist_nn;
    int persist6;
    bool small6;
    bool gemm6c;
    bool gemm6e;
    bool gemm6e_all;
    bool gemm6s;
    int split_kmin;
    int split_target;
    bool no_slab_xcd;
};
const GemmEnv& gemm_env() {
    static const GemmEnv env = [] {
        auto num = [](const char* name, int dflt) { const char* e = getenv(name); return e ? atoi(e) : dflt; };
        GemmEnv v;
        const char* m = getenv("RLT_GEMM_MODE");
        v.mode = !m ? -1 : (!strcmp(m, "bf16x6") || !strcmp(m, "2")) ? 2 : (!strcmp(m, "bf16x3") || !strcmp(m, "1")) ? 1 : 0;
        v.nofast = num("RLT_GEMM_NOFAST", 0) != 0;
        v.no_big = num("RLT_GEMM_NO_BIG", 0) != 0;
        v.persist = num("RLT_GEMM_PERSIST", 256);
        v.persist_nn = num("RLT_GEMM_PERSIST_NN", 0) != 0;
        v.persist6 = num("RLT_GEMM6_PERSIST", 256);
        v.small6 = getenv("RLT_GEMM6_SMALL") != nullptr;
        v.gemm6c = num("RLT_GEMM6C", 1) != 0;
        v.gemm6e = num("RLT_GEMM6E", 1) != 0;
        v.gemm6e_all = num("RLT_GEMM6E_ALL", 0) != 0;
        v.gemm6s = num("RLT_GEMM6S", 1) != 0;
        v.split_kmin = num("RLT_GEMM_SPLIT_KMIN", 1024);
        v.split_target = num("RLT_GEMM_SPLIT_TARGET", 1024);
        v.no_slab_xcd = getenv("RLT_GEMM_NO_SLAB_XCD") != nullptr;
        return v;
    }();
    return env;
}

int wanted_slabs(int M, int N, int K) {
    const GemmEnv& e = gemm_env();
    const long long tiles = (long long)rlt_cdiv(M, 128) * rlt_cdiv(N, 128);
    if (tiles >= 256 || K < e.split_kmin) return 1;
    long long want = e.split_target / tiles > 0 ? e.split_target / tiles : 1;
    const long long per = K >= 4096 ? 512 : 256;
    const long long maxs = K / per > 0 ? K / per : 1;
    if (want > maxs) want = maxs;
    if (want > 256) want = 256;
    if (want >= 8) want = want / 8 * 8;
    return (int)want;
}
size_t slab_bytes(int slabs, int M, int N) { return slabs > 1 ? ((size_t)slabs * M * N + (size_t)slabs * M) * sizeof(float) : 0; }

}

GemmPlan gemm_plan(const GemmCall& c) {
    const GemmEnv& e = gemm_env();
    const int mode = e.mode >= 0 ? e.mode : rlt_precision();
    const int M = c.M, N = c.N, K = c.K;
    const bool ta = c.ta != 0, tb = c.tb != 0;
    auto has = [&](int bit) { return (c.present & bit) != 0; };
    auto al = [&](int bit) { return (c.aligned16 & bit) != 0; };
    const bool bias = has(RLT_GEMM_PTR_BIAS), bias2 = has(RLT_GEMM_PTR_BIAS2), mask = has(RLT_GEMM_PTR_RELU_MASK),
               colsum = has(RLT_GEMM_PTR_COLSUM), bits_out = has(RLT_GEMM_PTR_BITS_OUT), bits_in = has(RLT_GEMM_PTR_BITS_IN);
    const bool relu = (c.flags & RLT_GEMM_RELU) != 0, accumulate = (c.flags & RLT_GEMM_ACCUMULATE) != 0, drop = c.drop != 0;
    const bool vec = c.lda % 4 == 0 && al(RLT_GEMM_PTR_A) && c.ldb % 4 == 0 && al(RLT_GEMM_PTR_B);

    GemmPlan p{};
    const int want = bits_out || bits_in ? 1 : wanted_slabs(M, N, K);
    p.ws_bytes = slab_bytes(want, M, N);
    int ns = want;
    if (ns > 1 && (c.ws_null || c.ws_bytes < p.ws_bytes)) {
        if (c.ws_null && c.ws_bytes == 0) ns = 1;
        else { p.rc = RLT_E_WORKSPACE; return p; }
    }
    const int kchunk = rlt_cdiv(rlt_cdiv(K, ns), 32) * 32;
    ns = rlt_cdiv(K, kchunk);
    const int slab_xcd = ns > 1 && ns % 8 == 0 && !e.no_slab_xcd;

    const bool wide = N % 256 == 0;
    const bool gemm6s = mode == 2 && e.gemm6s && !ta && ns == 1 && !mask && !colsum && !drop && !accumulate &&
        (!bits_in || (!bias && !bias2 && !relu)) && !(bits_out && bits_in) &&
        (K == 256 || K == 128) && (wide || (K == 128 && N % 128 == 0 && !bits_out && !bits_in)) && N <= 256 * 256 && M >= 32 * 256 &&
        vec && c.ldc % 4 == 0 && al(RLT_GEMM_PTR_C) && (!bias || al(RLT_GEMM_PTR_BIAS)) && (!bias2 || al(RLT_GEMM_PTR_BIAS2)) &&
        (!bits_out || al(RLT_GEMM_PTR_BITS_OUT)) && (!bits_in || al(RLT_GEMM_PTR_BITS_IN)) &&
        (size_t)c.lda * 4 * 32 < (1u << 31) && (size_t)c.ldc * 4 * 32 < (1u << 31);
    const bool tile6 = mode == 2 && vec && M % 256 == 0 && N % 128 == 0 && K % 32 == 0;
    const bool big6 = tile6 && wide && !e.small6;
    const bool pipe6 = big6 && e.gemm6c && kchunk >= 64 && (K % kchunk == 0 || K % kchunk >= 64);
    const bool plain_epilogue = !mask && !bits_in && !bits_out && !drop;
    const bool big3 = mode == 1 && !e.no_big && vec && M % 256 == 0 && N % 256 == 0 && K % 32 == 0;
    const int family = gemm6s ? RLT_GEMM_6S
                     : pipe6 ? (e.gemm6e && plain_epilogue && (ta || K >= 1024 || K == 768 || e.gemm6e_all) ? RLT_GEMM_6E : RLT_GEMM_6C)
                     : big6 ? RLT_GEMM_6B
                     : tile6 ? RLT_GEMM_6
                     : big3 ? RLT_GEMM_3B
                     : mode == 1 ? RLT_GEMM_3 : RLT_GEMM_F32;
    const GemmFamily& f = GEMM_FAMILY[family];
    p.wg = f.wg;
    p.lds_bytes = f.lds;
    p.reduce = ns > 1;

    if (family == RLT_GEMM_6S) {
        if (bits_out && !relu) { p.rc = -1; return p; }
        const int narrow = !wide;
        const int npanel = N / (narrow ? 128 : 256), nblk = (M + 31) / 32;
        int nstream = 256 / npanel;
        if (nstream < 1) nstream = 1;
        if (nstream > nblk) nstream = nblk;
        p.tiles_m = nstream; p.tiles_n = npanel;
        p.grid_x = npanel * nstream; p.grid_z = 1;
        p.lds_bytes = K == 256 ? GEMM6S_LDS_K256 : GEMM6S_LDS_K128;
        p.d = rlt_gemm_dispatch{family, 0, tb, 1, 0, 1, K, 0, bits_in ? 3 : bits_out ? 2 : relu ? 1 : 0, narrow};
        return p;
    }
    p.tiles_m = rlt_cdiv(M, f.bm); p.tiles_n = rlt_cdiv(N, f.bn);
    const long long tiles = (long long)p.tiles_m * p.tiles_n;
    const bool small = family == RLT_GEMM_F32 || family == RLT_GEMM_3;
    const bool fast = !small || (!e.nofast && vec && K % 4 == 0 && K >= 4 && (!ta || (M % 4 == 0 && M >= 4)) && (tb || (N % 4 == 0 && N >= 4)));
    const int wgs = family == RLT_GEMM_3B ? e.persist : e.persist6;
    const bool persistent = !ta && ns == 1 && wgs > 0 && wgs % 8 == 0 && tiles > wgs &&
        (family == RLT_GEMM_3B ? (tb || (e.persist_nn && !bits_in)) && K / 32 >= 2 : family == RLT_GEMM_6C || family == RLT_GEMM_6E);
    p.grid_x = persistent ? wgs : (unsigned)(tiles * (slab_xcd ? ns : 1));
    p.grid_z = slab_xcd ? 1 : ns;
    p.d = rlt_gemm_dispatch{family, ta, tb, fast, persistent, ns, kchunk, slab_xcd, 0, 0};
    return p;
}

extern "C" {

size_t rlt_gemm_workspace(int ta, int tb, int M, int N, int K) {
    (void)ta; (void)tb;
    if (M <= 0 || N <= 0 || K <= 0) return 0;
    return slab_bytes(wanted_slabs(M, N, K), M, N);
}

int rlt_gemm_plan(const rlt_gemm_call* c, int precision, rlt_gemm_dispatch* out) {
    RLT_PREC_SCOPE(precision);
    RLT_CHECK_ARG(c && out && c->M > 0 && c->N > 0 && c->K > 0);
    RLT_CHECK_ARG(c->lda >= (c->ta ? c->M : c->K) && c->ldb >= (c->tb ? c->K : c->N) && c->ldc >= c->N);
    RLT_CHECK_ARG(!(c->present & RLT_GEMM_PTR_COLSUM) || c->ta);
    const GemmPlan p = gemm_plan(*c);
    *out = p.d;
    return p.rc;
}

}
```

### ranked-list-truncation_amd/csrc/path.hip

```cpp
#include "common.h"
#include <stdio.h>
#include <stdlib.h>

namespace {

constexpr size_t ALIGN = 256;
inline size_t rup(size_t b) { return (b + ALIGN - 1) / ALIGN * ALIGN; }

struct Cursor {
    uint8_t* base; size_t off, cap;
    explicit Cursor(void* p, size_t cap_ = (size_t)-1) : base((uint8_t*)p), off(0), cap(cap_) {}
    template <typename T = float> T* take(size_t bytes) {
        T* p = (T*)(base ? base + off : nullptr);
#ifdef RLT_BOUNDS_CHECK
        if (base && cap != (size_t)-1 && off + bytes > cap) {
            fprintf(stderr, "rlt bounds check: region of %zu bytes at offset %zu leaves a %zu-byte buffer\n", bytes, off, cap);
            abort();
        }
#endif
        off += rup(bytes);
        return p;
    }
};

struct EncDims { int S, B, E, H, FF; size_t T; int HD; bool bits; };

inline int enc_dims(int S, int B, int E, int H, int FF, EncDims& d) {
    if (S <= 0 || B <= 0 || E <= 0 || H <= 0 || FF <= 0 || E % H) return RLT_E_ARG;
    d = EncDims{S, B, E, H, FF, (size_t)S * B, E / H, FF % 32 == 0};
    if ((size_t)S * B > 0x7fffffffu) return RLT_E_SHAPE;
    return 0;
}

struct EncStash {
    float *qkv, *att, *lse, *proj, *st1, *h1, *hid, *ff, *st2;
    uint32_t* bits;
    void* images; size_t images_bytes;
    size_t bytes;
};
inline EncStash enc_stash(const EncDims& d, void* base, size_t cap = (size_t)-1) {
    Cursor c(base, cap);
    EncStash s{};
    const size_t T = d.T, f = sizeof(float);
    s.qkv = c.take(T * 3 * d.E * f);
    s.att = c.take(T * d.E * f);
    s.lse = c.take((size_t)d.S * d.H * d.B * f);
    s.proj = c.take(T * d.E * f);
    s.st1 = c.take(T * 2 * f);
    s.h1 = c.take(T * d.E * f);
    s.hid = c.take(T * d.FF * f);
    s.bits = d.bits ? c.take<uint32_t>(rlt_gemm_bits_words((int)T, d.FF) * sizeof(uint32_t)) : nullptr;
    s.ff = c.take(T * d.E * f);
    s.st2 = c.take(T * 2 * f);
    const bool keep = rlt_list_attention_images_retained(d.S, d.B, d.H, d.HD, RLT_PRECISION_DEFAULT) != 0;
    s.images_bytes = keep ? rlt_list_attention_fwd_workspace(d.S, d.B, d.H, d.HD, 0.f, RLT_PRECISION_DEFAULT) : 0;
    s.images = s.images_bytes ? c.take<uint8_t>(s.images_bytes) : nullptr;
    s.bytes = c.off;
    return s;
}
inline size_t enc_fwd_images_scratch(const EncDims& d, float drop_p) {
    if (rlt_list_attention_images_retained(d.S, d.B, d.H, d.HD, RLT_PRECISION_DEFAULT)) return 0;
    return rlt_list_attention_fwd_workspace(d.S, d.B, d.H, d.HD, drop_p, RLT_PRECISION_DEFAULT);
}

struct EncScratch {
    float *dz2, *dr2, *dhid, *dr1, *datt, *dqkv;
    void *attn_ws, *ln_ws, *gemm_ws;
    size_t attn_ws_bytes, ln_ws_bytes, gemm_ws_bytes, bytes;
};
inline size_t enc_gemm_ws(const EncDims& d) {
    const int T = (int)d.T;
    size_t m = 0;
    auto up = [&](size_t v) { if (v > m) m = v; };
    up(rlt_gemm_workspace(1, 0, d.E, d.FF, T));
    up(rlt_gemm_workspace(1, 0, d.FF, d.E, T));
    up(rlt_gemm_workspace(1, 0, d.E, d.E, T));
    up(rlt_gemm_workspace(1, 0, 3 * d.E, d.E, T));
    up(rlt_gemm_workspace(0, 1, T, 3 * d.E, d.E));
    up(rlt_gemm_workspace(0, 1, T, d.FF, d.E));
    up(rlt_gemm_workspace(0, 1, T, d.E, d.FF));
    up(rlt_gemm_workspace(0, 0, T, d.FF, d.E));
    up(rlt_gemm_workspace(0, 0, T, d.E, d.FF));
    up(rlt_gemm_workspace(0, 0, T, d.E, 3 * d.E));
    return m;
}
inline EncScratch enc_scratch(const EncDims& d, bool drop, void* base, size_t cap = (size_t)-1) {
    Cursor c(base, cap);
    EncScratch w{};
    const size_t T = d.T, f = sizeof(float);
    w.dz2 = c.take(T * d.E * f);
    w.dr2 = drop ? c.take(T * d.E * f) : nullptr;
    const size_t mid = c.off;
    w.dhid = c.take(T * d.FF * f);
    const size_t end_ffn = c.off;
    c.off = mid;
    w.dr1 = drop ? c.take(T * d.E * f) : nullptr;
    w.datt = c.take(T * d.E * f);
    w.dqkv = c.take(T * 3 * d.E * f);
    w.attn_ws_bytes = rlt_list_attention_bwd_workspace(d.S, d.B, d.H, d.HD, drop ? 0.5f : 0.f, RLT_PRECISION_DEFAULT);
    w.attn_ws = c.take<uint8_t>(w.attn_ws_bytes);
    if (c.off < end_ffn) c.off = end_ffn;
    w.ln_ws_bytes = rlt_add_layernorm_bwd_workspace((int)T, d.E);
    w.ln_ws = c.take<uint8_t>(w.ln_ws_bytes);
    w.gemm_ws_bytes = enc_gemm_ws(d);
    w.gemm_ws = c.take<uint8_t>(w.gemm_ws_bytes);
    w.bytes = c.off;
    return w;
}

#define RLT_TRY(expr) do { int rc_ = (expr); if (rc_) return rc_; } while (0)

inline int gemm(int ta, int tb, int M, int N, int K, const float* A, int lda, const float* B, int ldb, float* C, int ldc,
                const float* bias, int flags, float* colsum_a, void* ws, size_t ws_bytes, void* st) {
    return rlt_gemm_ex(ta, tb, M, N, K, A, lda, B, ldb, C, ldc, bias, nullptr, flags, nullptr, 0, 1.f, colsum_a, 0.f, 0u,
                       ws, ws_bytes, RLT_PRECISION_DEFAULT, st);
}

struct LstmStash { float *gates[2], *c[2], *h0; size_t bytes; };
inline LstmStash lstm_stash(size_t T, void* base, size_t cap = (size_t)-1) {
    Cursor cur(base, cap);
    LstmStash s{};
    for (int l = 0; l < 2; ++l) {
        s.gates[l] = cur.take(T * 1024 * sizeof(float));
        s.c[l] = cur.take(T * 256 * sizeof(float));
    }
    s.h0 = cur.take(T * 256 * sizeof(float));
    s.bytes = cur.off;
    return s;
}
struct LstmScratch { float *wcat, *bcat, *dh0, *dwcat, *dbcat; void* ws; size_t ws_bytes, bytes; };
inline LstmScratch lstm_scratch(size_t T, int I, void* base, size_t cap = (size_t)-1) {
    Cursor cur(base, cap);
    LstmScratch w{};
    const int Imax = I > 256 ? I : 256;
    w.wcat = cur.take((size_t)1024 * Imax * sizeof(float));
    w.bcat = cur.take(2 * 1024 * sizeof(float));
    w.dh0 = cur.take(T * 256 * sizeof(float));
    w.dwcat = cur.take((size_t)1024 * Imax * sizeof(float));
    w.dbcat = cur.take(1024 * sizeof(float));
    size_t m = rlt_narrow_dw_workspace((int)T, 1024);
    auto up = [&](size_t v) { if (v > m) m = v; };
    up(rlt_gemm_workspace(1, 0, 1024, Imax, (int)T));
    up(rlt_gemm_workspace(1, 0, 512, 128, (int)T));
    up(rlt_gemm_workspace(0, 1, (int)T, 1024, Imax));
    up(rlt_gemm_workspace(0, 0, (int)T, Imax, 1024));
    w.ws_bytes = m;
    w.ws = cur.take<uint8_t>(m);
    w.bytes = cur.off;
    return w;
}

__global__ __launch_bounds__(256) void pack2_kernel(const float* __restrict__ a, const float* __restrict__ b, size_t n,
                                                    float* __restrict__ out) {
    for (size_t i = (size_t)blockIdx.x * 256 + threadIdx.x; i < 2 * n; i += (size_t)gridDim.x * 256)
        out[i] = i < n ? a[i] : b[i - n];
}
__global__ __launch_bounds__(256) void unpack2_kernel(const float* __restrict__ in, size_t n, float* __restrict__ a,
                                                      float* __restrict__ b) {
    for (size_t i = (size_t)blockIdx.x * 256 + threadIdx.x; i < 2 * n; i += (size_t)gridDim.x * 256) {
        if (i < n) a[i] = in[i]; else b[i - n] = in[i];
    }
}
inline int pack2(const float* a, const float* b, size_t n, float* out, hipStream_t st) {
    const int grid = (int)((2 * n + 255) / 256 < 512 ? (2 * n + 255) / 256 : 512);
    hipLaunchKernelGGL(pack2_kernel, dim3(grid), dim3(256), 0, st, a, b, n, out);
    return RLT_LAUNCH_RESULT();
}
inline int unpack2(const float* in, size_t n, float* a, float* b, hipStream_t st) {
    const int grid = (int)((2 * n + 255) / 256 < 512 ? (2 * n + 255) / 256 : 512);
    hipLaunchKernelGGL(unpack2_kernel, dim3(grid), dim3(256), 0, st, in, n, a, b);
    return RLT_LAUNCH_RESULT();
}

int lstm_layer_fwd(const float* x, int I, const rlt_lstm_layer_weights& w, int S, int B, float* gates, float* c, float* h,
                   const LstmScratch& sc, void* stream, const rlt_sparse_batch* sp = nullptr) {
    const int T = S * B;
    if (sp) {
        RLT_TRY(rlt_sparse_inproj_fwd(sp, S, B, w.w_ih[0], w.w_ih[1], w.b_ih[0], w.b_hh[0], w.b_ih[1], w.b_hh[1], gates, stream));
        return rlt_bilstm_rec_fwd(gates, w.w_hh[0], w.w_hh[1], S, B, h, c, RLT_PRECISION_DEFAULT, stream);
    }
    if (I <= 3)
        return rlt_bilstm_rec_fwd_x(x, I, w.w_ih[0], w.b_ih[0], w.b_hh[0], w.w_ih[1], w.b_ih[1], w.b_hh[1], w.w_hh[0], w.w_hh[1],
                                    S, B, gates, h, c, RLT_PRECISION_DEFAULT, stream);
    hipStream_t st = rlt_stream(stream);
    RLT_TRY(pack2(w.w_ih[0], w.w_ih[1], (size_t)512 * I, sc.wcat, st));
    RLT_TRY(pack2(w.b_ih[0], w.b_ih[1], 512, sc.bcat, st));
    RLT_TRY(pack2(w.b_hh[0], w.b_hh[1], 512, sc.bcat + 1024, st));
    RLT_TRY(rlt_gemm_ex(0, 1, T, 1024, I, x, I, sc.wcat, I, gates, 1024, sc.bcat, sc.bcat + 1024, 0, nullptr, 0, 1.f, nullptr,
                        0.f, 0u, sc.ws, sc.ws_bytes, RLT_PRECISION_DEFAULT, stream));
    return rlt_bilstm_rec_fwd(gates, w.w_hh[0], w.w_hh[1], S, B, h, c, RLT_PRECISION_DEFAULT, stream);
}

int lstm_layer_bwd(const float* x, int I, const rlt_lstm_layer_weights& w, const float* h, float* gates, const float* c,
                   const float* dh, int S, int B, float* dx, const rlt_lstm_layer_grads& g, const LstmScratch& sc, void* stream,
                   const rlt_sparse_batch* sp = nullptr, void* sp_ws = nullptr, size_t sp_ws_bytes = 0) {
    const int T = S * B;
    hipStream_t st = rlt_stream(stream);
    RLT_TRY(rlt_bilstm_rec_bwd(gates, c, w.w_hh[0], w.w_hh[1], dh, S, B, RLT_PRECISION_DEFAULT, stream));
    const float* dA = gates;
    if (sp) {
        RLT_TRY(rlt_sparse_inproj_bwd(sp, S, B, dA, g.w_ih[0], g.w_ih[1], g.b_ih[0], g.b_hh[0], g.b_ih[1], g.b_hh[1],
                                      sp_ws, sp_ws_bytes, stream));
    } else if (I <= 3) {
        RLT_TRY(rlt_narrow_dw(dA, 1024, x, I, I, T, 1024, sc.dwcat, sc.dbcat, sc.ws, sc.ws_bytes, stream));
    } else {
        RLT_TRY(gemm(1, 0, 1024, I, T, dA, 1024, x, I, sc.dwcat, I, nullptr, 0, sc.dbcat, sc.ws, sc.ws_bytes, stream));
    }
    if (!sp) {
        RLT_TRY(unpack2(sc.dwcat, (size_t)512 * I, g.w_ih[0], g.w_ih[1], st));
        RLT_TRY(unpack2(sc.dbcat, 512, g.b_ih[0], g.b_ih[1], st));
        RLT_TRY(unpack2(sc.dbcat, 512, g.b_hh[0], g.b_hh[1], st));
    }
    if (S > 1) {
        const int K = T - B;
        RLT_TRY(gemm(1, 0, 512, 128, K, dA + (size_t)B * 1024, 1024, h, 256, g.w_hh[0], 128, nullptr, 0, nullptr, sc.ws, sc.ws_bytes, stream));
        RLT_TRY(gemm(1, 0, 512, 128, K, dA + 512, 1024, h + (size_t)B * 256 + 128, 256, g.w_hh[1], 128, nullptr, 0, nullptr, sc.ws, sc.ws_bytes, stream));
    } else {
        RLT_TRY((int)hipMemsetAsync(g.w_hh[0], 0, 512 * 128 * sizeof(float), st));
        RLT_TRY((int)hipMemsetAsync(g.w_hh[1], 0, 512 * 128 * sizeof(float), st));
    }
    if (dx) {
        RLT_TRY(pack2(w.w_ih[0], w.w_ih[1], (size_t)512 * I, sc.wcat, st));
        RLT_TRY(gemm(0, 0, T, I, 1024, dA, 1024, sc.wcat, I, dx, I, nullptr, 0, nullptr, sc.ws, sc.ws_bytes, stream));
    }
    return 0;
}

bool lstm_weights_ok(const rlt_lstm_layer_weights& w) {
    for (int d = 0; d < 2; ++d)
        if (!w.w_ih[d] || !w.w_hh[d] || !w.b_ih[d] || !w.b_hh[d]) return false;
    return true;
}
bool lstm_grads_ok(const rlt_lstm_layer_grads& g) {
    for (int d = 0; d < 2; ++d)
        if (!g.w_ih[d] || !g.w_hh[d] || !g.b_ih[d] || !g.b_hh[d]) return false;
    return true;
}

}

extern "C" {

size_t rlt_workspace_bytes(int op, int S, int B, int E, int H, int FF, int train_dropout, int precision) {
    RLT_PREC_SCOPE_SZ(precision);
    if (op == RLT_OP_ENCODER_STASH || op == RLT_OP_ENCODER_BWD_WS || op == RLT_OP_ENCODER_FWD_WS) {
        EncDims d;
        if (enc_dims(S, B, E, H, FF, d)) return 0;
        if (op == RLT_OP_ENCODER_STASH) return enc_stash(d, nullptr).bytes;
        if (op == RLT_OP_ENCODER_FWD_WS) return rup(enc_gemm_ws(d)) + rup(enc_fwd_images_scratch(d, train_dropout ? 0.5f : 0.f));
        return enc_scratch(d, train_dropout != 0, nullptr).bytes;
    }
    if (op == RLT_OP_BILSTM_STASH || op == RLT_OP_BILSTM_WS) {
        if (S <= 0 || B <= 0 || E <= 0) return 0;
        const size_t T = (size_t)S * B;
        return op == RLT_OP_BILSTM_STASH ? lstm_stash(T, nullptr).bytes : lstm_scratch(T, E, nullptr).bytes;
    }
    return 0;
}

int rlt_encoder_layer_fwd(const float* x, const rlt_encoder_weights* w, int S, int B, int E, int H, int FF, float eps,
                          float drop_p, const uint32_t* seeds, float* y, void* stash, size_t stash_bytes,
                          void* ws, size_t ws_bytes, int precision, void* stream) {
    RLT_PREC_SCOPE(precision);
    RLT_CHECK_ARG(x && w && y && stash && drop_p >= 0.f && drop_p < 1.f && (drop_p == 0.f || seeds));
    RLT_CHECK_ARG(w->in_proj_weight && w->in_proj_bias && w->out_proj_weight && w->out_proj_bias && w->norm1_weight &&
                  w->norm1_bias && w->linear1_weight && w->linear1_bias && w->linear2_weight && w->linear2_bias &&
                  w->norm2_weight && w->norm2_bias);
    EncDims d;
    RLT_TRY(enc_dims(S, B, E, H, FF, d));
    const size_t gemm_ws = rup(enc_gemm_ws(d)), img_scratch = enc_fwd_images_scratch(d, drop_p);
    if (stash_bytes < enc_stash(d, nullptr).bytes || ws_bytes < gemm_ws + img_scratch || (gemm_ws + img_scratch && !ws)) return RLT_E_WORKSPACE;
    EncStash s = enc_stash(d, stash, stash_bytes);
    if (img_scratch) { s.images = static_cast<uint8_t*>(ws) + gemm_ws; s.images_bytes = img_scratch; }
    const int T = (int)d.T;
    const uint32_t s_attn = drop_p > 0.f ? seeds[0] : 0u, s_ln1 = drop_p > 0.f ? seeds[1] : 0u,
                   s_ffn = drop_p > 0.f ? seeds[2] : 0u, s_ln2 = drop_p > 0.f ? seeds[3] : 0u;
    RLT_TRY(gemm(0, 1, T, 3 * E, E, x, E, w->in_proj_weight, E, s.qkv, 3 * E, w->in_proj_bias, 0, nullptr, ws, ws_bytes, stream));
    RLT_TRY(rlt_list_attention_fwd(s.qkv, S, B, H, d.HD, drop_p, s_attn, s.att, s.lse, s.images, s.images_bytes, RLT_PRECISION_DEFAULT, stream));
    RLT_TRY(gemm(0, 1, T, E, E, s.att, E, w->out_proj_weight, E, s.proj, E, w->out_proj_bias, 0, nullptr, ws, ws_bytes, stream));
    RLT_TRY(rlt_add_layernorm_fwd(x, s.proj, w->norm1_weight, w->norm1_bias, T, E, eps, drop_p, s_ln1, s.h1, s.st1, stream));
    if (d.bits) {
        RLT_TRY(rlt_gemm_bits(0, 1, T, FF, E, s.h1, E, w->linear1_weight, E, s.hid, FF, w->linear1_bias, RLT_GEMM_RELU,
                              drop_p, s_ffn, s.bits, nullptr, 1.f, RLT_PRECISION_DEFAULT, stream));
    } else {
        RLT_TRY(rlt_gemm_ex(0, 1, T, FF, E, s.h1, E, w->linear1_weight, E, s.hid, FF, w->linear1_bias, nullptr, RLT_GEMM_RELU,
                            nullptr, 0, 1.f, nullptr, drop_p, s_ffn, ws, ws_bytes, RLT_PRECISION_DEFAULT, stream));
    }
    RLT_TRY(gemm(0, 1, T, E, FF, s.hid, FF, w->linear2_weight, FF, s.ff, E, w->linear2_bias, 0, nullptr, ws, ws_bytes, stream));
    return rlt_add_layernorm_fwd(s.h1, s.ff, w->norm2_weight, w->norm2_bias, T, E, eps, drop_p, s_ln2, y, s.st2, stream);
}

int rlt_encoder_layer_bwd(const float* x, const rlt_encoder_weights* w, int S, int B, int E, int H, int FF, float eps,
                          float drop_p, const uint32_t* seeds, const float* dy, const void* stash, size_t stash_bytes,
                          float* dx, const rlt_encoder_grads* g, void* ws, size_t ws_bytes, int precision, void* stream) {
    RLT_PREC_SCOPE(precision);
    (void)eps;
    RLT_CHECK_ARG(x && w && dy && stash && dx && g && ws && drop_p >= 0.f && drop_p < 1.f && (drop_p == 0.f || seeds));
    RLT_CHECK_ARG(g->in_proj_weight && g->in_proj_bias && g->out_proj_weight && g->out_proj_bias && g->norm1_weight &&
                  g->norm1_bias && g->linear1_weight && g->linear1_bias && g->linear2_weight && g->linear2_bias &&
                  g->norm2_weight && g->norm2_bias);
    EncDims d;
    RLT_TRY(enc_dims(S, B, E, H, FF, d));
    const bool drop = drop_p > 0.f;
    if (stash_bytes < enc_stash(d, nullptr).bytes || ws_bytes < enc_scratch(d, drop, nullptr).bytes) return RLT_E_WORKSPACE;
    const EncStash s = enc_stash(d, const_cast<void*>(stash), stash_bytes);
    const EncScratch k = enc_scratch(d, drop, ws, ws_bytes);
    const int T = (int)d.T;
    const uint32_t s_attn = drop ? seeds[0] : 0u, s_ln1 = drop ? seeds[1] : 0u, s_ln2 = drop ? seeds[3] : 0u;
    const float keep_scale = 1.f / (1.f - drop_p);
    RLT_TRY(rlt_add_layernorm_bwd(s.h1, s.ff, w->norm2_weight, s.st2, dy, T, E, drop_p, s_ln2, k.dz2, k.dr2,
                                  g->norm2_weight, g->norm2_bias, 0, k.ln_ws, k.ln_ws_bytes, stream));
    const float* dr2 = drop ? k.dr2 : k.dz2;
    RLT_TRY(gemm(1, 0, E, FF, T, dr2, E, s.hid, FF, g->linear2_weight, FF, nullptr, 0, g->linear2_bias, k.gemm_ws, k.gemm_ws_bytes, stream));
    if (d.bits) {
        RLT_TRY(rlt_gemm_bits(0, 0, T, FF, E, dr2, E, w->linear2_weight, FF, k.dhid, FF, nullptr, 0, 0.f, 0u, nullptr, s.bits,
                              keep_scale, RLT_PRECISION_DEFAULT, stream));
    } else {
        RLT_TRY(rlt_gemm_ex(0, 0, T, FF, E, dr2, E, w->linear2_weight, FF, k.dhid, FF, nullptr, nullptr, 0, s.hid, FF, keep_scale,
                            nullptr, 0.f, 0u, k.gemm_ws, k.gemm_ws_bytes, RLT_PRECISION_DEFAULT, stream));
    }
    RLT_TRY(gemm(1, 0, FF, E, T, k.dhid, FF, s.h1, E, g->linear1_weight, E, nullptr, 0, g->linear1_bias, k.gemm_ws, k.gemm_ws_bytes, stream));
    RLT_TRY(gemm(0, 0, T, E, FF, k.dhid, FF, w->linear1_weight, E, k.dz2, E, nullptr, RLT_GEMM_ACCUMULATE, nullptr, k.gemm_ws, k.gemm_ws_bytes, stream));
    RLT_TRY(rlt_add_layernorm_bwd(x, s.proj, w->norm1_weight, s.st1, k.dz2, T, E, drop_p, s_ln1, dx, k.dr1,
                                  g->norm1_weight, g->norm1_bias, 0, k.ln_ws, k.ln_ws_bytes, stream));
    const float* dr1 = drop ? k.dr1 : dx;
    RLT_TRY(gemm(1, 0, E, E, T, dr1, E, s.att, E, g->out_proj_weight, E, nullptr, 0, g->out_proj_bias, k.gemm_ws, k.gemm_ws_bytes, stream));
    RLT_TRY(gemm(0, 0, T, E, E, dr1, E, w->out_proj_weight, E, k.datt, E, nullptr, 0, nullptr, k.gemm_ws, k.gemm_ws_bytes, stream));
    RLT_TRY(rlt_list_attention_bwd(s.qkv, s.att, k.datt, s.lse, S, B, H, d.HD, drop_p, s_attn, s.images, k.dqkv,
                                   k.attn_ws, k.attn_ws_bytes, RLT_PRECISION_DEFAULT, stream));
    RLT_TRY(gemm(1, 0, 3 * E, E, T, k.dqkv, 3 * E, x, E, g->in_proj_weight, E, nullptr, 0, g->in_proj_bias, k.gemm_ws, k.gemm_ws_bytes, stream));
    return gemm(0, 0, T, E, 3 * E, k.dqkv, 3 * E, w->in_proj_weight, E, dx, E, nullptr, RLT_GEMM_ACCUMULATE, nullptr, k.gemm_ws, k.gemm_ws_bytes, stream);
}

int rlt_bilstm_fwd(const float* x, int I, const rlt_lstm_layer_weights* w, int S, int B, float* h_out,
                   void* stash, size_t stash_bytes, void* ws, size_t ws_bytes, int precision, void* stream) {
    RLT_PREC_SCOPE(precision);
    RLT_CHECK_ARG(x && w && h_out && stash && ws && I > 0 && S > 0 && B > 0 && lstm_weights_ok(w[0]) && lstm_weights_ok(w[1]));
    const size_t T = (size_t)S * B;
    RLT_CHECK_SHAPE(T <= 0x7fffffffu);
    if (stash_bytes < lstm_stash(T, nullptr).bytes || ws_bytes < lstm_scratch(T, I, nullptr).bytes) return RLT_E_WORKSPACE;
    const LstmStash s = lstm_stash(T, stash, stash_bytes);
    const LstmScratch k = lstm_scratch(T, I, ws, ws_bytes);
    RLT_TRY(lstm_layer_fwd(x, I, w[0], S, B, s.gates[0], s.c[0], s.h0, k, stream));
    return lstm_layer_fwd(s.h0, 256, w[1], S, B, s.gates[1], s.c[1], h_out, k, stream);
}

int rlt_bilstm_bwd(const float* x, int I, const rlt_lstm_layer_weights* w, const float* h_out, const float* dh_out, int S, int B,
                   void* stash, size_t stash_bytes, float* dx, const rlt_lstm_layer_grads* g,
                   void* ws, size_t ws_bytes, int precision, void* stream) {
    RLT_PREC_SCOPE(precision);
    RLT_CHECK_ARG(x && w && h_out && dh_out && stash && g && ws && I > 0 && S > 0 && B > 0);
    RLT_CHECK_ARG(lstm_weights_ok(w[0]) && lstm_weights_ok(w[1]) && lstm_grads_ok(g[0]) && lstm_grads_ok(g[1]));
    const size_t T = (size_t)S * B;
    RLT_CHECK_SHAPE(T <= 0x7fffffffu);
    if (stash_bytes < lstm_stash(T, nullptr).bytes || ws_bytes < lstm_scratch(T, I, nullptr).bytes) return RLT_E_WORKSPACE;
    const LstmStash s = lstm_stash(T, stash, stash_bytes);
    const LstmScratch k = lstm_scratch(T, I, ws, ws_bytes);
    RLT_TRY(lstm_layer_bwd(s.h0, 256, w[1], h_out, s.gates[1], s.c[1], dh_out, S, B, k.dh0, g[1], k, stream));
    return lstm_layer_bwd(x, I, w[0], s.h0, s.gates[0], s.c[0], k.dh0, S, B, dx, g[0], k, stream);
}

size_t rlt_bilstm_sparse_workspace(int S, int B, int Dn, int n_docs, int V, int n_chunks) {
    const size_t sp = rlt_sparse_inproj_workspace(S, B, Dn, n_docs, V, n_chunks);
    if (!sp) return 0;
    return lstm_scratch((size_t)S * B, 256, nullptr).bytes + rup(sp);
}

int rlt_bilstm_sparse_fwd(const rlt_sparse_batch* sb, const rlt_lstm_layer_weights* w, int S, int B, float* h_out,
                          void* stash, size_t stash_bytes, void* ws, size_t ws_bytes, int precision, void* stream) {
    RLT_PREC_SCOPE(precision);
    RLT_CHECK_ARG(sb && w && h_out && stash && ws && S > 0 && B > 0 && lstm_weights_ok(w[0]) && lstm_weights_ok(w[1]));
    const size_t T = (size_t)S * B;
    RLT_CHECK_SHAPE(T <= 0x7fffffffu);
    if (stash_bytes < lstm_stash(T, nullptr).bytes || ws_bytes < lstm_scratch(T, 256, nullptr).bytes) return RLT_E_WORKSPACE;
    const LstmStash s = lstm_stash(T, stash, stash_bytes);
    const LstmScratch k = lstm_scratch(T, 256, ws, ws_bytes);
    RLT_TRY(lstm_layer_fwd(nullptr, 0, w[0], S, B, s.gates[0], s.c[0], s.h0, k, stream, sb));
    return lstm_layer_fwd(s.h0, 256, w[1], S, B, s.gates[1], s.c[1], h_out, k, stream);
}

int rlt_bilstm_sparse_bwd(const rlt_sparse_batch* sb, const rlt_lstm_layer_weights* w, const float* h_out, const float* dh_out,
                          int S, int B, void* stash, size_t stash_bytes, const rlt_lstm_layer_grads* g,
                          void* ws, size_t ws_bytes, int precision, void* stream) {
    RLT_PREC_SCOPE(precision);
    RLT_CHECK_ARG(sb && w && h_out && dh_out && stash && g && ws && S > 0 && B > 0);
    RLT_CHECK_ARG(lstm_weights_ok(w[0]) && lstm_weights_ok(w[1]) && lstm_grads_ok(g[0]) && lstm_grads_ok(g[1]));
    const size_t T = (size_t)S * B;
    RLT_CHECK_SHAPE(T <= 0x7fffffffu);
    const size_t sp_bytes = rlt_sparse_inproj_workspace(S, B, sb->Dn, sb->n_docs, sb->V, sb->n_chunks);
    RLT_CHECK_ARG(sp_bytes > 0);
    const size_t dense_bytes = lstm_scratch(T, 256, nullptr).bytes;
    if (stash_bytes < lstm_stash(T, nullptr).bytes || ws_bytes < dense_bytes + rup(sp_bytes)) return RLT_E_WORKSPACE;
    const LstmStash s = lstm_stash(T, stash, stash_bytes);
    const LstmScratch k = lstm_scratch(T, 256, ws, dense_bytes);
    RLT_TRY(lstm_layer_bwd(s.h0, 256, w[1], h_out, s.gates[1], s.c[1], dh_out, S, B, k.dh0, g[1], k, stream));
    return lstm_layer_bwd(nullptr, 0, w[0], s.h0, s.gates[0], s.c[0], k.dh0, S, B, nullptr, g[0], k, stream,
                          sb, static_cast<uint8_t*>(ws) + dense_bytes, sp_bytes);
}

}
```

### ranked-list-truncation_amd/rlt_hip/build.py

```python
import os
import subprocess
import sys
from concurrent.futures import ThreadPoolExecutor

PKG_DIR = os.path.dirname(os.path.dirname(os.path.abspath(__file__)))
CSRC = os.path.join(PKG_DIR, "csrc")
LIB = os.path.join(CSRC, "librlt_hip.so")
HIPCC = os.environ.get("HIPCC", "/opt/rocm/bin/hipcc")
FLAGS = ["-O3", "--offload-arch=gfx950", "-fPIC", "-std=c++17", "-Wall", "-Wno-unused-function",
         "-ffp-contract=off"]
FILE_FLAGS = {"attention6.hip": ["-fno-slp-vectorize"], "attention6n.hip": ["-fno-slp-vectorize", "-mllvm", "-amdgpu-mfma-vgpr-form"],
              "attention6h.hip": ["-fno-slp-vectorize", "-mllvm", "-amdgpu-mfma-vgpr-form"],
              "lstm6w.hip": ["-fno-slp-vectorize"], "gemm6s.hip": ["-fno-slp-vectorize"]}


def sources():
    return sorted(os.path.join(CSRC, f) for f in os.listdir(CSRC) if f.endswith(".hip"))


def _stale(target, deps):
    if not os.path.exists(target):
        return True
    t = os.path.getmtime(target)
    return any(os.path.getmtime(d) > t for d in deps)


def build(force=False, verbose=True):
    srcs = sources()
    headers = [os.path.join(CSRC, f) for f in os.listdir(CSRC) if f.endswith((".h", ".inc"))]
    headers.append(os.path.join(os.path.dirname(PKG_DIR), "include", "rlt_hip.h"))
    objs = []
    jobs = []
    for s in srcs:
        o = s[:-4] + ".o"
        objs.append(o)
        if force or _stale(o, [s] + headers):
            jobs.append([HIPCC] + FLAGS + FILE_FLAGS.get(os.path.basename(s), []) + ["-c", s, "-o", o])

    def run(cmd):
        if verbose:
            print(" ".join(cmd), flush=True)
        res = subprocess.run(cmd, capture_output=True, text=True)
        if res.returncode != 0:
            raise RuntimeError("hipcc failed:\n" + res.stdout + res.stderr)
        if verbose and res.stderr.strip():
            print(res.stderr, file=sys.stderr)

    with ThreadPoolExecutor(max_workers=min(6, max(1, len(jobs)))) as ex:
        list(ex.map(run, jobs))
    if force or jobs or _stale(LIB, objs):
        run([HIPCC, "--offload-arch=gfx950", "-shared", "-fPIC", "-o", LIB] + objs)
    return LIB


SAN_LIB = os.path.join(CSRC, "librlt_hip_asan.so")
SAN_FLAGS = ["-O1", "-g", "-std=c++17", "-fPIC", "--offload-arch=gfx950", "--offload-host-only", "-fsanitize=address,undefined",
             "-fno-omit-frame-pointer", "-shared-libsan", "-DRLT_BOUNDS_CHECK", "-Wall", "-Wno-unused-function", "-ffp-contract=off"]


def sanitizer_runtime():
    res = subprocess.run([HIPCC, "-print-file-name=libclang_rt.asan-x86_64.so"], capture_output=True, text=True)
    path = res.stdout.strip()
    return path if os.path.isabs(path) and os.path.exists(path) else None


def build_sanitized(verbose=True):
    srcs = sources()
    headers = [os.path.join(CSRC, f) for f in os.listdir(CSRC) if f.endswith((".h", ".inc"))]
    headers.append(os.path.join(os.path.dirname(PKG_DIR), "include", "rlt_hip.h"))
    if _stale(SAN_LIB, srcs + headers + [os.path.abspath(__file__)]):
        def run(cmd):
            if verbose:
                print(" ".join(cmd), flush=True)
            res = subprocess.run(cmd, capture_output=True, text=True)
            if res.returncode != 0:
                raise RuntimeError("hipcc (sanitized host build) failed:\n" + res.stdout + res.stderr)
            return res.stdout
        objs = [src[:-4] + ".asan.o" for src in srcs]
        with ThreadPoolExecutor(max_workers=6) as ex:
            list(ex.map(lambda so: run([HIPCC] + SAN_FLAGS + ["-c", so[0], "-o", so[1]]), zip(srcs, objs)))
        undefined = sorted({l.split()[-1] for o in objs for l in run(["nm", "-u", o]).splitlines() if "__hip_fatbin_" in l})
        stub = SAN_LIB + ".fatbin_stubs.c"
        with open(stub, "w") as f:
            f.write("/* generated by rlt_hip/build.py: empty offload bundles for the host-only sanitizer build */\n")
            for sym in undefined:
                f.write('__attribute__((aligned(4096))) const char %s[32] = "__CLANG_OFFLOAD_BUNDLE__";\n' % sym)
        stub_o = stub[:-2] + ".o"
        run(["gcc", "-c", "-fPIC", stub, "-o", stub_o])
        run([HIPCC, "--offload-arch=gfx950", "--offload-host-only", "-fsanitize=address,undefined", "-shared-libsan", "-shared", "-fPIC",
             "-o", SAN_LIB] + objs + [stub_o])
        for f in objs + [stub, stub_o]:
            os.remove(f)
    return SAN_LIB


if __name__ == "__main__":
    if "--sanitize" in sys.argv:
        print(build_sanitized())
    else:
        print(build(force="--force" in sys.argv))
```

Baseline: 25740 lists/s.

## Fuse K/V bf16 split-image production into the in-projection GEMM epilogue

Adds a new epilogue (EPI 4) to the streaming 6-product GEMM that, besides storing qkv, splits each output into hi/mid/lo bf16 planes and writes them straight into the attention K/V image layout. The attention forward then skips the separate prepare kernel and runs only a small drain kernel that zeroes the padding tile. The aim is to avoid re-reading qkv from global memory and one kernel launch. In exchange the GEMM epilogue does extra splitting and scattered 64-bit stores, and the path only applies for K=256, N=768 with the pipelined attention plan.

Measured after the change: 25750 lists/s (median of 6 runs). No clear change (+0.1%).

```diff
diff --git a/ranked-list-truncation_amd/csrc/attention6h.hip b/ranked-list-truncation_amd/csrc/attention6h.hip
--- a/ranked-list-truncation_amd/csrc/attention6h.hip
+++ b/ranked-list-truncation_amd/csrc/attention6h.hip
@@ -36,6 +36,12 @@
         *reinterpret_cast<bf16x8*>(im + PLH) = mm_;
         *reinterpret_cast<bf16x8*>(im + 2 * PLH) = ll_;
     }
+}
+
+__global__ __launch_bounds__(256) void attn6h_drain_kernel(uint8_t* __restrict__ img, int ntile) {
+    uint4* rec = reinterpret_cast<uint4*>(img + ((size_t)blockIdx.x * (ntile + 1) + ntile) * RECH);
+#pragma unroll
+    for (int i = 0; i < RECH / 16 / 256; ++i) rec[i * 256 + threadIdx.x] = make_uint4(0u, 0u, 0u, 0u);
 }
 
 #ifndef RLT_A6H_FWD1_BODY
@@ -288,6 +294,13 @@
     return RLT_LAUNCH_RESULT();
 }
 
+int rlt_attn6h_drain2(const AttnArgs& a, hipStream_t st) {
+    RLT_CHECK_ARG(a.img && a.B % KTH == 0);
+    hipLaunchKernelGGL(attn6h_drain_kernel, dim3(2 * a.S * a.H), dim3(256), 0, st,
+                       reinterpret_cast<uint8_t*>(const_cast<void*>(a.img)), a.B / KTH);
+    return RLT_LAUNCH_RESULT();
+}
+
 int rlt_attn6h_run(int which, const AttnArgs& a, hipStream_t st) {
     RLT_CHECK_ARG(which == 0 && a.img && a.redo && a.B % KTH == 0);
     const size_t shm = (size_t)4 * IMGH * sizeof(uint16_t) + 2 * KTH * sizeof(uint32_t);
diff --git a/ranked-list-truncation_amd/csrc/attention_common.h b/ranked-list-truncation_amd/csrc/attention_common.h
--- a/ranked-list-truncation_amd/csrc/attention_common.h
+++ b/ranked-list-truncation_amd/csrc/attention_common.h
@@ -75,4 +75,8 @@
 int rlt_attn6n_run(int kernel, int which, const AttnArgs& a, hipStream_t st);
 size_t rlt_attn6h_fwd_images_bytes(int S, int B, int H);
 int rlt_attn6h_prepare2(int what0, int slot0, int what1, int slot1, const AttnArgs& a, hipStream_t st);
+int rlt_attn6h_drain2(const AttnArgs& a, hipStream_t st);
 int rlt_attn6h_run(int which, const AttnArgs& a, hipStream_t st);
+
+int rlt_list_attention_fwd_images_ready(const float* qkv, int S, int B, int H, int HD, float drop_p, uint32_t seed,
+                                        float* out, float* lse, void* images, size_t images_bytes, void* stream);
diff --git a/ranked-list-truncation_amd/csrc/attention_dispatch.hip b/ranked-list-truncation_amd/csrc/attention_dispatch.hip
--- a/ranked-list-truncation_amd/csrc/attention_dispatch.hip
+++ b/ranked-list-truncation_amd/csrc/attention_dispatch.hip
@@ -144,6 +144,37 @@
     return RLT_E_ARG;
 }
 
+int fwd(const float* qkv, int S, int B, int H, int HD, float drop_p, uint32_t seed, float* out, float* lse, void* images,
+        size_t images_bytes, bool images_ready, void* stream) {
+    RLT_CHECK_ARG(qkv && out && lse && S > 0 && B > 0 && H > 0 && drop_ok(drop_p));
+    RLT_CHECK_SHAPE(hd_ok(HD));
+    if (!(rlt_aligned16(qkv) && rlt_aligned16(out))) return RLT_E_ALIGN;
+    AttnPlan p = attn_plan(S, B, H, HD, drop_p, images != nullptr);
+    if (p.fwd_prepare && p.images_retained) {
+        if (images_bytes < p.images_bytes) return RLT_E_WORKSPACE;
+        if (!rlt_aligned16(images)) return RLT_E_ALIGN;
+    } else if (p.fwd_prepare && !(rlt_aligned16(images) && images_bytes >= p.images_bytes)) {
+        p = attn_plan(S, B, H, HD, drop_p, false);
+    }
+    RLT_CHECK_ARG(!images_ready || p.fwd == RLT_ATTN_X6H_PIPE);
+    AttnArgs a{};
+    a.qkv = qkv; a.o = out; a.lse_o = lse; a.S = S; a.B = B; a.H = H;
+    a.scale = 1.0f / sqrtf((float)HD);
+    a.drop_p = drop_p; a.drop_thr = rlt_drop_threshold(drop_p); a.seed = seed;
+    if (p.fwd_prepare) a.img = images;
+    if (p.fwd_fixup) a.redo = reinterpret_cast<uint32_t*>(reinterpret_cast<uint8_t*>(images) + p.flags_offset);
+    hipStream_t st = rlt_stream(stream);
+    int rc = 0;
+    switch (p.fwd) {
+    case RLT_ATTN_X6_IMG: case RLT_ATTN_X6_PP_IMG: rc = rlt_attn6_prepare(false, a, HD, st); break;
+    case RLT_ATTN_X6N_PIPE: rc = rlt_attn6n_prepare_at(1, 0, a, st); if (!rc) rc = rlt_attn6n_prepare_at(2, 1, a, st); break;
+    case RLT_ATTN_X6H_PIPE: rc = images_ready ? rlt_attn6h_drain2(a, st) : rlt_attn6h_prepare2(1, 0, 2, 1, a, st); break;
+    }
+    if (!rc) rc = run_kernel(p.fwd, 0, a, HD, images, nullptr, st);
+    if (!rc && p.fwd_fixup) rc = run_kernel(p.fwd_fixup, 0, a, HD, nullptr, nullptr, st);
+    return rc;
+}
+
 int bwd_prepare(const float* out, const float* dout, const float* lse, int S, int B, int H, int HD,
                 const void* images, void* ws, size_t ws_bytes, float drop_p, void* stream) {
     RLT_CHECK_ARG(out && dout && lse && ws && S > 0 && B > 0 && H > 0 && drop_ok(drop_p));
@@ -219,32 +250,7 @@
 int rlt_list_attention_fwd(const float* qkv, int S, int B, int H, int HD, float drop_p, uint32_t seed,
                            float* out, float* lse, void* images, size_t images_bytes, int precision, void* stream) {
     RLT_PREC_SCOPE(precision);
-    RLT_CHECK_ARG(qkv && out && lse && S > 0 && B > 0 && H > 0 && drop_ok(drop_p));
-    RLT_CHECK_SHAPE(hd_ok(HD));
-    if (!(rlt_aligned16(qkv) && rlt_aligned16(out))) return RLT_E_ALIGN;
-    AttnPlan p = attn_plan(S, B, H, HD, drop_p, images != nullptr);
-    if (p.fwd_prepare && p.images_retained) {
-        if (images_bytes < p.images_bytes) return RLT_E_WORKSPACE;
-        if (!rlt_aligned16(images)) return RLT_E_ALIGN;
-    } else if (p.fwd_prepare && !(rlt_aligned16(images) && images_bytes >= p.images_bytes)) {
-        p = attn_plan(S, B, H, HD, drop_p, false);
-    }
-    AttnArgs a{};
-    a.qkv = qkv; a.o = out; a.lse_o = lse; a.S = S; a.B = B; a.H = H;
-    a.scale = 1.0f / sqrtf((float)HD);
-    a.drop_p = drop_p; a.drop_thr = rlt_drop_threshold(drop_p); a.seed = seed;
-    if (p.fwd_prepare) a.img = images;
-    if (p.fwd_fixup) a.redo = reinterpret_cast<uint32_t*>(reinterpret_cast<uint8_t*>(images) + p.flags_offset);
-    hipStream_t st = rlt_stream(stream);
-    int rc = 0;
-    switch (p.fwd) {
-    case RLT_ATTN_X6_IMG: case RLT_ATTN_X6_PP_IMG: rc = rlt_attn6_prepare(false, a, HD, st); break;
-    case RLT_ATTN_X6N_PIPE: rc = rlt_attn6n_prepare_at(1, 0, a, st); if (!rc) rc = rlt_attn6n_prepare_at(2, 1, a, st); break;
-    case RLT_ATTN_X6H_PIPE: rc = rlt_attn6h_prepare2(1, 0, 2, 1, a, st); break;
-    }
-    if (!rc) rc = run_kernel(p.fwd, 0, a, HD, images, nullptr, st);
-    if (!rc && p.fwd_fixup) rc = run_kernel(p.fwd_fixup, 0, a, HD, nullptr, nullptr, st);
-    return rc;
+    return fwd(qkv, S, B, H, HD, drop_p, seed, out, lse, images, images_bytes, false, stream);
 }
 
 size_t rlt_list_attention_bwd_workspace(int S, int B, int H, int HD, float drop_p, int precision) {
@@ -283,3 +289,8 @@
 }
 
 }
+
+int rlt_list_attention_fwd_images_ready(const float* qkv, int S, int B, int H, int HD, float drop_p, uint32_t seed,
+                                        float* out, float* lse, void* images, size_t images_bytes, void* stream) {
+    return fwd(qkv, S, B, H, HD, drop_p, seed, out, lse, images, images_bytes, true, stream);
+}
diff --git a/ranked-list-truncation_amd/csrc/gemm.hip b/ranked-list-truncation_amd/csrc/gemm.hip
--- a/ranked-list-truncation_amd/csrc/gemm.hip
+++ b/ranked-list-truncation_amd/csrc/gemm.hip
@@ -1740,7 +1740,7 @@
                     const float* bias, const float* bias2, int flags,
                     const float* relu_mask, int ldmask, float mask_scale, float* colsum_a,
                     float drop_p, uint32_t seed, uint32_t* bits_out, const uint32_t* bits_in,
-                    void* ws, size_t ws_bytes, void* stream) {
+                    void* ws, size_t ws_bytes, void* stream, uint8_t* kv_img = nullptr, int kv_ntile = 0) {
     rlt_gemm_dispatch_rec = rlt_gemm_dispatch{};
     RLT_CHECK_ARG(A && B && C && M > 0 && N > 0 && K > 0);
     RLT_CHECK_ARG(lda >= (ta ? M : K) && ldb >= (tb ? K : N) && ldc >= N);
@@ -1763,7 +1763,8 @@
 
     hipStream_t st = rlt_stream(stream);
     if (p.d.family == RLT_GEMM_6S) {
-        const Gemm6sArgs s6{A, B, C, bias, bias2, M, N, K, lda, ldb, ldc, bits_out, bits_in, mask_scale};
+        RLT_CHECK_ARG(p.d.epilogue != 4 || (kv_img && rlt_aligned16(kv_img) && kv_ntile > 0 && M % (64 * kv_ntile) == 0));
+        const Gemm6sArgs s6{A, B, C, bias, bias2, M, N, K, lda, ldb, ldc, bits_out, bits_in, mask_scale, kv_img, kv_ntile};
         const int rc = rlt_gemm6s_launch(s6, p, &rlt_gemm_dispatch_rec, st);
         return rc ? rc : RLT_LAUNCH_RESULT();
     }
@@ -1816,8 +1817,8 @@
                 float drop_p, uint32_t seed,
                 void* ws, size_t ws_bytes, int precision, void* stream) {
     RLT_PREC_SCOPE(precision);
-    return gemm_run(ta, tb, M, N, K, A, lda, B, ldb, C, ldc, bias, bias2, flags, relu_mask, ldmask, mask_scale, colsum_a,
-                    drop_p, seed, nullptr, nullptr, ws, ws_bytes, stream);
+    return gemm_run(ta, tb, M, N, K, A, lda, B, ldb, C, ldc, bias, bias2, flags & ~RLT_GEMM_INTERNAL_FLAGS, relu_mask, ldmask, mask_scale,
+                    colsum_a, drop_p, seed, nullptr, nullptr, ws, ws_bytes, stream);
 }
 
 size_t rlt_gemm_bits_words(int M, int N) { return M > 0 && N > 0 ? (size_t)rlt_cdiv(M, 32) * N : 0; }
@@ -1832,9 +1833,22 @@
     RLT_CHECK_ARG(!relu_bits_out || (flags & RLT_GEMM_RELU));
     RLT_CHECK_ARG(drop_p == 0.f || relu_bits_out);
     RLT_CHECK_SHAPE(N % 32 == 0);
-    return gemm_run(ta, tb, M, N, K, A, lda, B, ldb, C, ldc, bias, nullptr, flags, nullptr, 0, mask_scale, nullptr,
+    return gemm_run(ta, tb, M, N, K, A, lda, B, ldb, C, ldc, bias, nullptr, flags & ~RLT_GEMM_INTERNAL_FLAGS, nullptr, 0, mask_scale, nullptr,
                     drop_p, seed, relu_bits_out, mask_bits_in, nullptr, 0, stream);
 }
+
+}
+
+int rlt_gemm_inproj_kv_images(int T, int E, int B, const float* x, const float* w, const float* bias, float* qkv, void* images,
+                              void* ws, size_t ws_bytes, int* wrote, void* stream) {
+    RLT_CHECK_ARG(wrote && images && B > 0 && B % 64 == 0 && T % B == 0);
+    const int rc = gemm_run(0, 1, T, 3 * E, E, x, E, w, E, qkv, 3 * E, bias, nullptr, RLT_GEMM_KV_IMAGES, nullptr, 0, 1.f, nullptr,
+                            0.f, 0u, nullptr, nullptr, ws, ws_bytes, stream, static_cast<uint8_t*>(images), B / 64);
+    *wrote = !rc && rlt_gemm_dispatch_rec.epilogue == 4;
+    return rc;
+}
+
+extern "C" {
 
 size_t rlt_colsum_workspace(int T, int N) {
     if (T <= 0 || N <= 0) return 0;
diff --git a/ranked-list-truncation_amd/csrc/gemm6s.h b/ranked-list-truncation_amd/csrc/gemm6s.h
--- a/ranked-list-truncation_amd/csrc/gemm6s.h
+++ b/ranked-list-truncation_amd/csrc/gemm6s.h
@@ -11,5 +11,11 @@
     uint32_t* bits_out;
     const uint32_t* bits_in;
     float mask_scale;
+    uint8_t* kv_img;
+    int kv_ntile;
 };
 int rlt_gemm6s_launch(const Gemm6sArgs& g, const GemmPlan& p, rlt_gemm_dispatch* rec, hipStream_t st);
+int rlt_gemm6s_kv_launch(const Gemm6sArgs& g, const GemmPlan& p, rlt_gemm_dispatch* rec, hipStream_t st);
+
+int rlt_gemm_inproj_kv_images(int T, int E, int B, const float* x, const float* w, const float* bias, float* qkv, void* images,
+                              void* ws, size_t ws_bytes, int* wrote, void* stream);
diff --git a/ranked-list-truncation_amd/csrc/gemm6s.hip b/ranked-list-truncation_amd/csrc/gemm6s.hip
--- a/ranked-list-truncation_amd/csrc/gemm6s.hip
+++ b/ranked-list-truncation_amd/csrc/gemm6s.hip
@@ -1,237 +1,11 @@
-#include "common.h"
-#include "gemm6s.h"
-#include "split6.h"
-#include <type_traits>
+#include "gemm6s_kernel.h"
 
-namespace {
-
-typedef unsigned int u32x4 __attribute__((ext_vector_type(4)));
-
-template <int KS> constexpr int gs_rowb() { return 64 * KS; }
-template <int KS> constexpr int gs_plane() { return 32 * gs_rowb<KS>(); }
-template <int KS> constexpr int gs_buf() { return 3 * gs_plane<KS>(); }
-template <int KS> constexpr int gs_wl() { return KS > 4 ? 4 * 4 * (KS - 4) * 64 * 16 : 0; }
-template <int KS> constexpr size_t gs_lds() { return (size_t)2 * gs_buf<KS>() + gs_wl<KS>(); }
-static_assert(gs_lds<8>() == 160 * 1024, "the K = 256 streaming product fills LDS exactly");
-
-__device__ __forceinline__ __amdgpu_buffer_rsrc_t rsrc_s(const void* p, uint32_t bytes) {
-    return __builtin_amdgcn_make_buffer_rsrc(const_cast<void*>(p), 0, bytes, 0x00020000);
-}
-
-template <int KS, int NCB, bool TB, int EPI>
-__global__ __launch_bounds__(256, 1) void gemm6s_kernel(Gemm6sArgs g) {
-    static_assert(NCB == 4 || (NCB == 2 && KS == 4 && EPI < 2), "128-column panels: K = 128, plain epilogues");
-    constexpr int PW = 64 * NCB, WC = 16 * NCB;
-    constexpr int GS_PLANE = gs_plane<KS>(), GS_BUF = gs_buf<KS>(), ROWB = gs_rowb<KS>(), CPR = 4 * KS, RPP = 256 / CPR, NI = 32 / RPP;
-    extern __shared__ __attribute__((aligned(16))) uint8_t sm6s[];
-    const int tid = threadIdx.x, lane = tid & 63, w = __builtin_amdgcn_readfirstlane(tid >> 6), n = lane & 15, q = lane >> 4;
-    const int npanel = g.N / PW;
-    const int panel = __builtin_amdgcn_readfirstlane(blockIdx.x % npanel), stream = __builtin_amdgcn_readfirstlane(blockIdx.x / npanel),
-              nstream = __builtin_amdgcn_readfirstlane(gridDim.x / npanel);
-    const int nblk = (g.M + 31) / 32;
-    uint4* wl_s = reinterpret_cast<uint4*>(sm6s + 2 * GS_BUF);
-    (void)wl_s;
-
-    bf16x8 wh[NCB][KS], wm[NCB][KS], wlv[NCB][4];
-    f32x4 bv[NCB];
-#pragma unroll
-    for (int pass = 0; pass < 2; ++pass) {
-#pragma unroll
-        for (int cb = 0; cb < NCB; ++cb) {
-            const int col = PW * panel + WC * w + 16 * cb + n;
-            const float* wp = TB ? g.B + (size_t)col * g.ldb + 8 * q : g.B + (size_t)(8 * q) * g.ldb + col;
-#pragma unroll
-            for (int ks = 0; ks < (pass ? 4 : KS); ++ks) {
-                asm volatile("" : "+v"(wp));
-                float v[8];
-                if (TB) {
-                    const float4 v0 = *reinterpret_cast<const float4*>(wp + 32 * ks), v1 = *reinterpret_cast<const float4*>(wp + 32 * ks + 4);
-                    v[0] = v0.x; v[1] = v0.y; v[2] = v0.z; v[3] = v0.w; v[4] = v1.x; v[5] = v1.y; v[6] = v1.z; v[7] = v1.w;
-                } else {
-#pragma unroll
-                    for (int j = 0; j < 8; ++j) v[j] = wp[(size_t)(32 * ks + j) * g.ldb];
-                }
-                uint2 h0, m0, l0, h1, m1, l1;
-                split4x3<true>(v[0], v[1], v[2], v[3], h0, m0, l0);
-                split4x3<true>(v[4], v[5], v[6], v[7], h1, m1, l1);
-                if (pass == 0) {
-                    wh[cb][ks] = frag4(h0.x, h0.y, h1.x, h1.y);
-                    wm[cb][ks] = frag4(m0.x, m0.y, m1.x, m1.y);
-                    asm volatile("" : "+a"(wh[cb][ks]), "+a"(wm[cb][ks]) : : "memory");
-                    if (KS > 4 && ks >= 4) wl_s[((w * 4 + cb) * (KS - 4) + (ks - 4)) * 64 + lane] = make_uint4(l0.x, l0.y, l1.x, l1.y);
-                } else {
-                    wlv[cb][ks] = frag4(l0.x, l0.y, l1.x, l1.y);
-                    asm volatile("" : "+v"(wlv[cb][ks]) : : "memory");
-                }
-            }
-            if (pass == 0) {
-                const int c4 = PW * panel + WC * w + 16 * cb + 4 * q;
-                f32x4 b = {0.f, 0.f, 0.f, 0.f};
-                if (g.bias) { const float4 t = *reinterpret_cast<const float4*>(g.bias + c4); b += f32x4{t.x, t.y, t.z, t.w}; }
-                if (g.bias2) { const float4 t = *reinterpret_cast<const float4*>(g.bias2 + c4); b += f32x4{t.x, t.y, t.z, t.w}; }
-                bv[cb] = b;
-            }
-        }
-    }
-
-    const int sc = tid % CPR, sr = tid / CPR;
-    const uint32_t voff_a = (uint32_t)sr * g.lda * 4u + sc * 32u;
-    uint32_t wro[NI];
-#pragma unroll
-    for (int i = 0; i < NI; ++i) wro[i] = (uint32_t)(sr + RPP * i) * ROWB + 16u * (sc ^ ((sr + RPP * i) & 15));
-    uint32_t rdo[4];
-#pragma unroll
-    for (int j = 0; j < 4; ++j) rdo[j] = n * ROWB + 64u * (j ^ (n >> 2)) + 16u * (q ^ (n & 3));
-    const uint8_t* wlrd = sm6s + 2 * GS_BUF + w * (4 * (KS - 4) * 1024) + lane * 16;
-    const uint32_t voff_c = (uint32_t)n * g.ldc * 4u + ((uint32_t)WC * w + 4u * q) * 4u;
-    const uint32_t voff_bo = lane < 16 ? ((uint32_t)WC * w + lane) * 4u : 0x7fff0000u;
-    const uint32_t voff_bi = ((uint32_t)WC * w + 4u * q) * 4u;
-    uint32_t bm[5];
-#pragma unroll
-    for (int r = 0; r < 4; ++r) bm[r] = (lane & 3) == r ? 0xffffffffu : 0u;
-    bm[4] = ((lane >> 2) & 3) < 2 ? 0xffffffffu : 0u;
-    const uint32_t bsh = 16u * ((lane >> 2) & 1);
-#pragma unroll
-    for (int r = 0; r < 5; ++r) asm volatile("" : "+v"(bm[r]));
-
-    auto blk_of = [&](int i) { return stream + i * nstream; };
-    auto rows_of = [&](int i) { const int r = g.M - 32 * blk_of(i); return __builtin_amdgcn_readfirstlane(i < 0 ? 0 : r < 0 ? 0 : r > 32 ? 32 : r); };
-    auto rs_a = [&](int i) { return rsrc_s(g.A + (size_t)(i < 0 ? 0 : blk_of(i)) * 32 * g.lda, (uint32_t)rows_of(i) * g.lda * 4u); };
-    auto rs_bits = [&](int i) {
-        const uint32_t* base = EPI == 2 ? g.bits_out : g.bits_in;
-        return rsrc_s(base + (size_t)(i < 0 ? 0 : blk_of(i)) * g.N + PW * panel, rows_of(i) > 0 ? (uint32_t)PW * 4u : 0u);
-    };
-    auto rs_c = [&](int i) { return rsrc_s(g.C + (size_t)(i < 0 ? 0 : blk_of(i)) * 32 * g.ldc + PW * panel, (uint32_t)rows_of(i) * g.ldc * 4u); };
-    const int nb = __builtin_amdgcn_readfirstlane(stream < nblk ? (nblk - stream + nstream - 1) / nstream : 0);
-
-    f32x4 acc[2][NCB], xs[2 * NI];
-    u32x4 bw[NCB];
-    bf16x8 bfr[2][3], lfr[NCB];
-    uint4 sph, spm, spl;
-    const f32x4 z4 = {0.f, 0.f, 0.f, 0.f};
-#pragma unroll
-    for (int i = 0; i < 2 * NCB; ++i) { acc[i / NCB][i % NCB] = z4; }
-#pragma unroll
-    for (int i = 0; i < 2 * NI; ++i) xs[i] = z4;
-#pragma unroll
-    for (int i = 0; i < 6; ++i) (&bfr[0][0])[i] = frag4(0u, 0u, 0u, 0u);
-#pragma unroll
-    for (int i = 0; i < NCB; ++i) lfr[i] = frag4(0u, 0u, 0u, 0u);
-    sph = spm = spl = make_uint4(0u, 0u, 0u, 0u);
-#pragma unroll
-    for (int cb = 0; cb < NCB; ++cb) bw[cb] = u32x4{0u, 0u, 0u, 0u};
-    auto load_x = [&](int i4, int part, __amdgpu_buffer_rsrc_t r) __attribute__((always_inline)) {
-        xs[2 * i4 + part] = __builtin_bit_cast(f32x4, __builtin_amdgcn_raw_buffer_load_b128(r, voff_a + 16u * part, (uint32_t)(RPP * i4) * g.lda * 4u, 0));
-    };
-    auto split_x = [&](int i4, int part) __attribute__((always_inline)) {
-        f32x4 &a = xs[2 * i4], &b = xs[2 * i4 + 1];
-        if (part == 0) { sph = make_uint4(pk2(a[0], a[1]), pk2(a[2], a[3]), pk2(b[0], b[1]), pk2(b[2], b[3])); asm("" : "+v"(sph.x), "+v"(sph.y), "+v"(sph.z), "+v"(sph.w)); }
-        if (part == 1) { a[0] -= lo16(sph.x); a[1] -= hi16(sph.x); a[2] -= lo16(sph.y); a[3] -= hi16(sph.y); }
-        if (part == 2) { b[0] -= lo16(sph.z); b[1] -= hi16(sph.z); b[2] -= lo16(sph.w); b[3] -= hi16(sph.w); }
-        if (part == 3) { spm = make_uint4(pk2(a[0], a[1]), pk2(a[2], a[3]), pk2(b[0], b[1]), pk2(b[2], b[3])); asm("" : "+v"(spm.x), "+v"(spm.y), "+v"(spm.z), "+v"(spm.w)); }
-        if (part == 4) { a[0] -= lo16(spm.x); a[1] -= hi16(spm.x); a[2] -= lo16(spm.y); a[3] -= hi16(spm.y); }
-        if (part == 5) { b[0] -= lo16(spm.z); b[1] -= hi16(spm.z); b[2] -= lo16(spm.w); b[3] -= hi16(spm.w); }
-        if (part == 6) spl = make_uint4(pk2(a[0], a[1]), pk2(a[2], a[3]), pk2(b[0], b[1]), pk2(b[2], b[3]));
-    };
-    auto write_x = [&](int buf, int i4, int pl) __attribute__((always_inline)) {
-        *reinterpret_cast<uint4*>(sm6s + buf * GS_BUF + pl * GS_PLANE + wro[i4]) = pl == 0 ? sph : pl == 1 ? spm : spl;
-    };
-    {
-        const __amdgpu_buffer_rsrc_t r0 = rs_a(0), r1 = rs_a(1);
-#pragma unroll
-        for (int i4 = 0; i4 < NI; ++i4) { load_x(i4, 0, r0); load_x(i4, 1, r0); }
-#pragma unroll
-        for (int i4 = 0; i4 < NI; ++i4) {
-#pragma unroll
-            for (int part = 0; part < 7; ++part) split_x(i4, part);
-#pragma unroll
-            for (int pl = 0; pl < 3; ++pl) write_x(0, i4, pl);
-            load_x(i4, 0, r1);
-            load_x(i4, 1, r1);
-        }
-#pragma unroll
-        for (int i = 0; i < 2 * NI; ++i) asm volatile("" : "+v"(xs[i]));
-    }
-    __syncthreads();
-
-#define GAP_END __builtin_amdgcn_sched_barrier(0)
-    auto tick = [&](auto XC, int i) __attribute__((always_inline)) {
-        constexpr int X = decltype(XC)::value, Y = 1 - X;
-        const __amdgpu_buffer_rsrc_t rc0 = rs_c(i), rc1 = rs_c(i - 1), ra2 = rs_a(i + 2);
-        const __amdgpu_buffer_rsrc_t rb0 = EPI >= 2 ? rs_bits(i) : rc0, rb1 = EPI == 2 ? rs_bits(i - 1) : rc1;
-        (void)rb0; (void)rb1;
-        auto RB = [&](int half, int ks, int pl) __attribute__((always_inline)) {
-            bfr[(KS * half + ks) & 1][pl] = *reinterpret_cast<const bf16x8*>(sm6s + X * GS_BUF + pl * GS_PLANE + half * 16 * ROWB + 256 * (ks >> 2) + rdo[ks & 3]);
-        };
-        auto RL = [&](int ks, int cb) __attribute__((always_inline)) { lfr[cb] = *reinterpret_cast<const bf16x8*>(wlrd + 1024 * ((KS - 4) * cb + ks - 4)); };
-        auto MG = [&](int half, int ks, int p, int cb, int first) __attribute__((always_inline)) {
-            const int bp = p == 2 ? 2 : (p == 0 || p == 4) ? 1 : 0;
-            const bf16x8 xv = bfr[(KS * half + ks) & 1][bp];
-            f32x4& d = acc[half][cb];
-            if (p == 1) {
-                const bf16x8 lv = ks < 4 ? wlv[cb][ks < 4 ? ks : 0] : lfr[cb];
-                asm volatile("v_mfma_f32_16x16x32_bf16 %0, %1, %2, %0" : "+v"(d) : "v"(lv), "v"(xv));
-            } else {
-                const bf16x8 av = (p == 0 || p == 3) ? wm[cb][ks] : wh[cb][ks];
-                const f32x4 seed = bv[cb];
-                if (first) asm volatile("v_mfma_f32_16x16x32_bf16 %0, %1, %2, %3" : "+v"(d) : "a"(av), "v"(xv), "v"(seed));
-                else asm volatile("v_mfma_f32_16x16x32_bf16 %0, %1, %2, %0" : "+v"(d) : "a"(av), "v"(xv));
-            }
-        };
-        auto EP = [&](int half, int cb) __attribute__((always_inline)) {
-            f32x4 v = acc[half][cb];
-            if (EPI == 3) {
-                const uint32_t sh = 16 * half + n;
-#pragma unroll
-                for (int r = 0; r < 4; ++r) v[r] = ((bw[cb][r] >> sh) & 1u) ? v[r] * g.mask_scale : 0.f;
-                if (half == 1) bw[cb] = __builtin_amdgcn_raw_buffer_load_b128(rb0, voff_bi + 64u * cb, 0, 0);
-            }
-            if (EPI == 1 || EPI == 2) v = f32x4{fmaxf(v[0], 0.f), fmaxf(v[1], 0.f), fmaxf(v[2], 0.f), fmaxf(v[3], 0.f)};
-            if (EPI == 2) {
-                const uint64_t b0 = __builtin_amdgcn_ballot_w64(v[0] > 0.f), b1 = __builtin_amdgcn_ballot_w64(v[1] > 0.f),
-                               b2 = __builtin_amdgcn_ballot_w64(v[2] > 0.f), b3 = __builtin_amdgcn_ballot_w64(v[3] > 0.f);
-                const uint32_t lo = ((uint32_t)b0 & bm[0]) | ((uint32_t)b1 & bm[1]) | ((uint32_t)b2 & bm[2]) | ((uint32_t)b3 & bm[3]);
-                const uint32_t hi = ((uint32_t)(b0 >> 32) & bm[0]) | ((uint32_t)(b1 >> 32) & bm[1]) | ((uint32_t)(b2 >> 32) & bm[2]) | ((uint32_t)(b3 >> 32) & bm[3]);
-                const uint32_t piece = ((lo & bm[4]) | (hi & ~bm[4])) >> bsh;
-                __builtin_amdgcn_raw_buffer_store_b16((short)piece, half ? rb1 : rb0, voff_bo + 64u * cb + 2u * half, 0, 0);
-            }
-            __builtin_amdgcn_raw_buffer_store_b128(__builtin_bit_cast(u32x4, v), half ? rc1 : rc0, voff_c + 64u * cb, (uint32_t)(16 * half) * g.ldc * 4u, 0);
-        };
-        auto SX = [&](int i4, int part) __attribute__((always_inline)) { split_x(i4, part); };
-        auto LX = [&](int i4, int part) __attribute__((always_inline)) { load_x(i4, part, ra2); };
-        auto WX = [&](int i4, int pl) __attribute__((always_inline)) { write_x(Y, i4, pl); };
-        RB(0, 0, 0); RB(0, 0, 1); RB(0, 0, 2);
-        GAP_END;
-        if constexpr (KS == 8) {
-#include "gemm6s_body.inc"
-        } else if constexpr (NCB == 4) {
-#include "gemm6s_k128_body.inc"
-        } else {
-#include "gemm6s_k128n128_body.inc"
-        }
-        asm volatile("s_waitcnt lgkmcnt(0)\n\ts_barrier" ::: "memory");
-    };
-    const std::integral_constant<int, 0> H0;
-    const std::integral_constant<int, 1> H1;
-    for (int i = 0; i < nb + 1; i += 2) {
-#pragma unroll
-        for (int cb = 0; cb < NCB; ++cb)
-#pragma unroll
-            for (int k4 = 0; k4 < KS; k4 += 4)
-                asm volatile("" : "+a"(wh[cb][k4]), "+a"(wh[cb][k4 + 1]), "+a"(wh[cb][k4 + 2]), "+a"(wh[cb][k4 + 3]), "+a"(wm[cb][k4]), "+a"(wm[cb][k4 + 1]),
-                             "+a"(wm[cb][k4 + 2]), "+a"(wm[cb][k4 + 3]));
-        tick(H0, i);
-        tick(H1, i + 1);
-    }
-#undef GAP_END
-}
-
-}
 
 static_assert(gs_lds<8>() == GEMM6S_LDS_K256 && gs_lds<4>() == GEMM6S_LDS_K128, "gemm_plan.h: the LDS bytes of the streaming kernels");
 
 int rlt_gemm6s_launch(const Gemm6sArgs& g, const GemmPlan& p, rlt_gemm_dispatch* rec, hipStream_t st) {
     const int epi = p.d.epilogue;
+    if (epi == 4) return rlt_gemm6s_kv_launch(g, p, rec, st);
     auto go = [&](auto kern) {
         const int rc = rlt_allow_lds(kern, p.lds_bytes);
         if (rc) return rc;
diff --git a/ranked-list-truncation_amd/csrc/gemm6s_kernel.h b/ranked-list-truncation_amd/csrc/gemm6s_kernel.h
--- /dev/null
+++ b/ranked-list-truncation_amd/csrc/gemm6s_kernel.h
@@ -0,0 +1,253 @@
+#pragma once
+#include "common.h"
+#include "gemm6s.h"
+#include "split6.h"
+#include <type_traits>
+
+namespace {
+
+typedef unsigned int u32x4 __attribute__((ext_vector_type(4)));
+typedef unsigned int u32x2 __attribute__((ext_vector_type(2)));
+
+template <int KS> constexpr int gs_rowb() { return 64 * KS; }
+template <int KS> constexpr int gs_plane() { return 32 * gs_rowb<KS>(); }
+template <int KS> constexpr int gs_buf() { return 3 * gs_plane<KS>(); }
+template <int KS> constexpr int gs_wl() { return KS > 4 ? 4 * 4 * (KS - 4) * 64 * 16 : 0; }
+template <int KS> constexpr size_t gs_lds() { return (size_t)2 * gs_buf<KS>() + gs_wl<KS>(); }
+static_assert(gs_lds<8>() == 160 * 1024, "the K = 256 streaming product fills LDS exactly");
+
+__device__ __forceinline__ __amdgpu_buffer_rsrc_t rsrc_s(const void* p, uint32_t bytes) {
+    return __builtin_amdgcn_make_buffer_rsrc(const_cast<void*>(p), 0, bytes, 0x00020000);
+}
+
+template <int KS, int NCB, bool TB, int EPI>
+__global__ __launch_bounds__(256, 1) void gemm6s_kernel(Gemm6sArgs g) {
+    static_assert(NCB == 4 || (NCB == 2 && KS == 4 && EPI < 2), "128-column panels: K = 128, plain epilogues");
+    static_assert(EPI != 4 || (KS == 8 && NCB == 4 && TB), "the image epilogue: the attention in-projection");
+    constexpr int PW = 64 * NCB, WC = 16 * NCB;
+    constexpr int GS_PLANE = gs_plane<KS>(), GS_BUF = gs_buf<KS>(), ROWB = gs_rowb<KS>(), CPR = 4 * KS, RPP = 256 / CPR, NI = 32 / RPP;
+    extern __shared__ __attribute__((aligned(16))) uint8_t sm6s[];
+    const int tid = threadIdx.x, lane = tid & 63, w = __builtin_amdgcn_readfirstlane(tid >> 6), n = lane & 15, q = lane >> 4;
+    const int npanel = g.N / PW;
+    const int panel = __builtin_amdgcn_readfirstlane(blockIdx.x % npanel), stream = __builtin_amdgcn_readfirstlane(blockIdx.x / npanel),
+              nstream = __builtin_amdgcn_readfirstlane(gridDim.x / npanel);
+    const int nblk = (g.M + 31) / 32;
+    uint4* wl_s = reinterpret_cast<uint4*>(sm6s + 2 * GS_BUF);
+    (void)wl_s;
+
+    bf16x8 wh[NCB][KS], wm[NCB][KS], wlv[NCB][4];
+    f32x4 bv[NCB];
+#pragma unroll
+    for (int pass = 0; pass < 2; ++pass) {
+#pragma unroll
+        for (int cb = 0; cb < NCB; ++cb) {
+            const int col = PW * panel + WC * w + 16 * cb + n;
+            const float* wp = TB ? g.B + (size_t)col * g.ldb + 8 * q : g.B + (size_t)(8 * q) * g.ldb + col;
+#pragma unroll
+            for (int ks = 0; ks < (pass ? 4 : KS); ++ks) {
+                asm volatile("" : "+v"(wp));
+                float v[8];
+                if (TB) {
+                    const float4 v0 = *reinterpret_cast<const float4*>(wp + 32 * ks), v1 = *reinterpret_cast<const float4*>(wp + 32 * ks + 4);
+                    v[0] = v0.x; v[1] = v0.y; v[2] = v0.z; v[3] = v0.w; v[4] = v1.x; v[5] = v1.y; v[6] = v1.z; v[7] = v1.w;
+                } else {
+#pragma unroll
+                    for (int j = 0; j < 8; ++j) v[j] = wp[(size_t)(32 * ks + j) * g.ldb];
+                }
+                uint2 h0, m0, l0, h1, m1, l1;
+                split4x3<true>(v[0], v[1], v[2], v[3], h0, m0, l0);
+                split4x3<true>(v[4], v[5], v[6], v[7], h1, m1, l1);
+                if (pass == 0) {
+                    wh[cb][ks] = frag4(h0.x, h0.y, h1.x, h1.y);
+                    wm[cb][ks] = frag4(m0.x, m0.y, m1.x, m1.y);
+                    asm volatile("" : "+a"(wh[cb][ks]), "+a"(wm[cb][ks]) : : "memory");
+                    if (KS > 4 && ks >= 4) wl_s[((w * 4 + cb) * (KS - 4) + (ks - 4)) * 64 + lane] = make_uint4(l0.x, l0.y, l1.x, l1.y);
+                } else {
+                    wlv[cb][ks] = frag4(l0.x, l0.y, l1.x, l1.y);
+                    asm volatile("" : "+v"(wlv[cb][ks]) : : "memory");
+                }
+            }
+            if (pass == 0) {
+                const int c4 = PW * panel + WC * w + 16 * cb + 4 * q;
+                f32x4 b = {0.f, 0.f, 0.f, 0.f};
+                if (g.bias) { const float4 t = *reinterpret_cast<const float4*>(g.bias + c4); b += f32x4{t.x, t.y, t.z, t.w}; }
+                if (g.bias2) { const float4 t = *reinterpret_cast<const float4*>(g.bias2 + c4); b += f32x4{t.x, t.y, t.z, t.w}; }
+                bv[cb] = b;
+            }
+        }
+    }
+
+    const int sc = tid % CPR, sr = tid / CPR;
+    const uint32_t voff_a = (uint32_t)sr * g.lda * 4u + sc * 32u;
+    uint32_t wro[NI];
+#pragma unroll
+    for (int i = 0; i < NI; ++i) wro[i] = (uint32_t)(sr + RPP * i) * ROWB + 16u * (sc ^ ((sr + RPP * i) & 15));
+    uint32_t rdo[4];
+#pragma unroll
+    for (int j = 0; j < 4; ++j) rdo[j] = n * ROWB + 64u * (j ^ (n >> 2)) + 16u * (q ^ (n & 3));
+    const uint8_t* wlrd = sm6s + 2 * GS_BUF + w * (4 * (KS - 4) * 1024) + lane * 16;
+    const uint32_t voff_c = (uint32_t)n * g.ldc * 4u + ((uint32_t)WC * w + 4u * q) * 4u;
+    const uint32_t voff_bo = lane < 16 ? ((uint32_t)WC * w + lane) * 4u : 0x7fff0000u;
+    const uint32_t voff_bi = ((uint32_t)WC * w + 4u * q) * 4u;
+    const uint32_t voff_i = 128u * n + 32u * ((n >> 1) & 3) + 8u * q;
+    uint32_t bm[5];
+#pragma unroll
+    for (int r = 0; r < 4; ++r) bm[r] = (lane & 3) == r ? 0xffffffffu : 0u;
+    bm[4] = ((lane >> 2) & 3) < 2 ? 0xffffffffu : 0u;
+    const uint32_t bsh = 16u * ((lane >> 2) & 1);
+#pragma unroll
+    for (int r = 0; r < 5; ++r) asm volatile("" : "+v"(bm[r]));
+
+    auto blk_of = [&](int i) { return stream + i * nstream; };
+    auto rows_of = [&](int i) { const int r = g.M - 32 * blk_of(i); return __builtin_amdgcn_readfirstlane(i < 0 ? 0 : r < 0 ? 0 : r > 32 ? 32 : r); };
+    auto rs_a = [&](int i) { return rsrc_s(g.A + (size_t)(i < 0 ? 0 : blk_of(i)) * 32 * g.lda, (uint32_t)rows_of(i) * g.lda * 4u); };
+    auto rs_bits = [&](int i) {
+        const uint32_t* base = EPI == 2 ? g.bits_out : g.bits_in;
+        return rsrc_s(base + (size_t)(i < 0 ? 0 : blk_of(i)) * g.N + PW * panel, rows_of(i) > 0 ? (uint32_t)PW * 4u : 0u);
+    };
+    auto rs_c = [&](int i) { return rsrc_s(g.C + (size_t)(i < 0 ? 0 : blk_of(i)) * 32 * g.ldc + PW * panel, (uint32_t)rows_of(i) * g.ldc * 4u); };
+    const uint32_t kv_nt = EPI == 4 ? (uint32_t)g.kv_ntile : 1u;
+    const uint32_t kv_block = EPI == 4 ? __builtin_amdgcn_readfirstlane((uint32_t)(g.M / 64) / kv_nt * 4u * (kv_nt + 1u)) : 0u;
+    const uint32_t kv_bytes = panel > 0 ? 24576u : 0u;
+    auto rs_img = [&](int i) {
+        const uint32_t gt = (uint32_t)(i < 0 ? 0 : blk_of(i)) >> 1;
+        const uint32_t pos = __builtin_amdgcn_readfirstlane(gt / kv_nt), tile = gt - pos * kv_nt;
+        const uint32_t rec = (panel > 1 ? kv_block : 0u) + (4u * pos + (uint32_t)w) * (kv_nt + 1u) + tile;
+        return rsrc_s(g.kv_img + (size_t)rec * 24576, rows_of(i) > 0 ? kv_bytes : 0u);
+    };
+    const int nb = __builtin_amdgcn_readfirstlane(stream < nblk ? (nblk - stream + nstream - 1) / nstream : 0);
+
+    f32x4 acc[2][NCB], xs[2 * NI];
+    u32x4 bw[NCB];
+    bf16x8 bfr[2][3], lfr[NCB];
+    uint4 sph, spm, spl;
+    const f32x4 z4 = {0.f, 0.f, 0.f, 0.f};
+#pragma unroll
+    for (int i = 0; i < 2 * NCB; ++i) { acc[i / NCB][i % NCB] = z4; }
+#pragma unroll
+    for (int i = 0; i < 2 * NI; ++i) xs[i] = z4;
+#pragma unroll
+    for (int i = 0; i < 6; ++i) (&bfr[0][0])[i] = frag4(0u, 0u, 0u, 0u);
+#pragma unroll
+    for (int i = 0; i < NCB; ++i) lfr[i] = frag4(0u, 0u, 0u, 0u);
+    sph = spm = spl = make_uint4(0u, 0u, 0u, 0u);
+#pragma unroll
+    for (int cb = 0; cb < NCB; ++cb) bw[cb] = u32x4{0u, 0u, 0u, 0u};
+    auto load_x = [&](int i4, int part, __amdgpu_buffer_rsrc_t r) __attribute__((always_inline)) {
+        xs[2 * i4 + part] = __builtin_bit_cast(f32x4, __builtin_amdgcn_raw_buffer_load_b128(r, voff_a + 16u * part, (uint32_t)(RPP * i4) * g.lda * 4u, 0));
+    };
+    auto split_x = [&](int i4, int part) __attribute__((always_inline)) {
+        f32x4 &a = xs[2 * i4], &b = xs[2 * i4 + 1];
+        if (part == 0) { sph = make_uint4(pk2(a[0], a[1]), pk2(a[2], a[3]), pk2(b[0], b[1]), pk2(b[2], b[3])); asm("" : "+v"(sph.x), "+v"(sph.y), "+v"(sph.z), "+v"(sph.w)); }
+        if (part == 1) { a[0] -= lo16(sph.x); a[1] -= hi16(sph.x); a[2] -= lo16(sph.y); a[3] -= hi16(sph.y); }
+        if (part == 2) { b[0] -= lo16(sph.z); b[1] -= hi16(sph.z); b[2] -= lo16(sph.w); b[3] -= hi16(sph.w); }
+        if (part == 3) { spm = make_uint4(pk2(a[0], a[1]), pk2(a[2], a[3]), pk2(b[0], b[1]), pk2(b[2], b[3])); asm("" : "+v"(spm.x), "+v"(spm.y), "+v"(spm.z), "+v"(spm.w)); }
+        if (part == 4) { a[0] -= lo16(spm.x); a[1] -= hi16(spm.x); a[2] -= lo16(spm.y); a[3] -= hi16(spm.y); }
+        if (part == 5) { b[0] -= lo16(spm.z); b[1] -= hi16(spm.z); b[2] -= lo16(spm.w); b[3] -= hi16(spm.w); }
+        if (part == 6) spl = make_uint4(pk2(a[0], a[1]), pk2(a[2], a[3]), pk2(b[0], b[1]), pk2(b[2], b[3]));
+    };
+    auto write_x = [&](int buf, int i4, int pl) __attribute__((always_inline)) {
+        *reinterpret_cast<uint4*>(sm6s + buf * GS_BUF + pl * GS_PLANE + wro[i4]) = pl == 0 ? sph : pl == 1 ? spm : spl;
+    };
+    {
+        const __amdgpu_buffer_rsrc_t r0 = rs_a(0), r1 = rs_a(1);
+#pragma unroll
+        for (int i4 = 0; i4 < NI; ++i4) { load_x(i4, 0, r0); load_x(i4, 1, r0); }
+#pragma unroll
+        for (int i4 = 0; i4 < NI; ++i4) {
+#pragma unroll
+            for (int part = 0; part < 7; ++part) split_x(i4, part);
+#pragma unroll
+            for (int pl = 0; pl < 3; ++pl) write_x(0, i4, pl);
+            load_x(i4, 0, r1);
+            load_x(i4, 1, r1);
+        }
+#pragma unroll
+        for (int i = 0; i < 2 * NI; ++i) asm volatile("" : "+v"(xs[i]));
+    }
+    __syncthreads();
+
+#define GAP_END __builtin_amdgcn_sched_barrier(0)
+    auto tick = [&](auto XC, int i) __attribute__((always_inline)) {
+        constexpr int X = decltype(XC)::value, Y = 1 - X;
+        const __amdgpu_buffer_rsrc_t rc0 = rs_c(i), rc1 = rs_c(i - 1), ra2 = rs_a(i + 2);
+        const __amdgpu_buffer_rsrc_t rb0 = EPI >= 2 ? rs_bits(i) : rc0, rb1 = EPI == 2 ? rs_bits(i - 1) : rc1;
+        (void)rb0; (void)rb1;
+        const __amdgpu_buffer_rsrc_t ri0 = EPI == 4 ? rs_img(i) : rc0, ri1 = EPI == 4 ? rs_img(i - 1) : rc1;
+        const uint32_t io0 = EPI == 4 ? (uint32_t)(blk_of(i) & 1) * 4096u : 0u, io1 = EPI == 4 ? (uint32_t)((i < 1 ? 0 : blk_of(i - 1)) & 1) * 4096u + 2048u : 0u;
+        (void)ri0; (void)ri1; (void)io0; (void)io1;
+        auto RB = [&](int half, int ks, int pl) __attribute__((always_inline)) {
+            bfr[(KS * half + ks) & 1][pl] = *reinterpret_cast<const bf16x8*>(sm6s + X * GS_BUF + pl * GS_PLANE + half * 16 * ROWB + 256 * (ks >> 2) + rdo[ks & 3]);
+        };
+        auto RL = [&](int ks, int cb) __attribute__((always_inline)) { lfr[cb] = *reinterpret_cast<const bf16x8*>(wlrd + 1024 * ((KS - 4) * cb + ks - 4)); };
+        auto MG = [&](int half, int ks, int p, int cb, int first) __attribute__((always_inline)) {
+            const int bp = p == 2 ? 2 : (p == 0 || p == 4) ? 1 : 0;
+            const bf16x8 xv = bfr[(KS * half + ks) & 1][bp];
+            f32x4& d = acc[half][cb];
+            if (p == 1) {
+                const bf16x8 lv = ks < 4 ? wlv[cb][ks < 4 ? ks : 0] : lfr[cb];
+                asm volatile("v_mfma_f32_16x16x32_bf16 %0, %1, %2, %0" : "+v"(d) : "v"(lv), "v"(xv));
+            } else {
+                const bf16x8 av = (p == 0 || p == 3) ? wm[cb][ks] : wh[cb][ks];
+                const f32x4 seed = bv[cb];
+                if (first) asm volatile("v_mfma_f32_16x16x32_bf16 %0, %1, %2, %3" : "+v"(d) : "a"(av), "v"(xv), "v"(seed));
+                else asm volatile("v_mfma_f32_16x16x32_bf16 %0, %1, %2, %0" : "+v"(d) : "a"(av), "v"(xv));
+            }
+        };
+        auto EP = [&](int half, int cb) __attribute__((always_inline)) {
+            f32x4 v = acc[half][cb];
+            if (EPI == 3) {
+                const uint32_t sh = 16 * half + n;
+#pragma unroll
+                for (int r = 0; r < 4; ++r) v[r] = ((bw[cb][r] >> sh) & 1u) ? v[r] * g.mask_scale : 0.f;
+                if (half == 1) bw[cb] = __builtin_amdgcn_raw_buffer_load_b128(rb0, voff_bi + 64u * cb, 0, 0);
+            }
+            if (EPI == 1 || EPI == 2) v = f32x4{fmaxf(v[0], 0.f), fmaxf(v[1], 0.f), fmaxf(v[2], 0.f), fmaxf(v[3], 0.f)};
+            if (EPI == 2) {
+                const uint64_t b0 = __builtin_amdgcn_ballot_w64(v[0] > 0.f), b1 = __builtin_amdgcn_ballot_w64(v[1] > 0.f),
+                               b2 = __builtin_amdgcn_ballot_w64(v[2] > 0.f), b3 = __builtin_amdgcn_ballot_w64(v[3] > 0.f);
+                const uint32_t lo = ((uint32_t)b0 & bm[0]) | ((uint32_t)b1 & bm[1]) | ((uint32_t)b2 & bm[2]) | ((uint32_t)b3 & bm[3]);
+                const uint32_t hi = ((uint32_t)(b0 >> 32) & bm[0]) | ((uint32_t)(b1 >> 32) & bm[1]) | ((uint32_t)(b2 >> 32) & bm[2]) | ((uint32_t)(b3 >> 32) & bm[3]);
+                const uint32_t piece = ((lo & bm[4]) | (hi & ~bm[4])) >> bsh;
+                __builtin_amdgcn_raw_buffer_store_b16((short)piece, half ? rb1 : rb0, voff_bo + 64u * cb + 2u * half, 0, 0);
+            }
+            __builtin_amdgcn_raw_buffer_store_b128(__builtin_bit_cast(u32x4, v), half ? rc1 : rc0, voff_c + 64u * cb, (uint32_t)(16 * half) * g.ldc * 4u, 0);
+            if (EPI == 4) {
+                uint2 ph, pm, pl;
+                split4x3<false>(v[0], v[1], v[2], v[3], ph, pm, pl);
+                const uint32_t vo = voff_i ^ (32u * cb), so = half ? io1 : io0;
+                __builtin_amdgcn_raw_buffer_store_b64(u32x2{ph.x, ph.y}, half ? ri1 : ri0, vo, so, 0);
+                __builtin_amdgcn_raw_buffer_store_b64(u32x2{pm.x, pm.y}, half ? ri1 : ri0, vo, so + 8192u, 0);
+                __builtin_amdgcn_raw_buffer_store_b64(u32x2{pl.x, pl.y}, half ? ri1 : ri0, vo, so + 16384u, 0);
+            }
+        };
+        auto SX = [&](int i4, int part) __attribute__((always_inline)) { split_x(i4, part); };
+        auto LX = [&](int i4, int part) __attribute__((always_inline)) { load_x(i4, part, ra2); };
+        auto WX = [&](int i4, int pl) __attribute__((always_inline)) { write_x(Y, i4, pl); };
+        RB(0, 0, 0); RB(0, 0, 1); RB(0, 0, 2);
+        GAP_END;
+        if constexpr (KS == 8) {
+#include "gemm6s_body.inc"
+        } else if constexpr (NCB == 4) {
+#include "gemm6s_k128_body.inc"
+        } else {
+#include "gemm6s_k128n128_body.inc"
+        }
+        asm volatile("s_waitcnt lgkmcnt(0)\n\ts_barrier" ::: "memory");
+    };
+    const std::integral_constant<int, 0> H0;
+    const std::integral_constant<int, 1> H1;
+    for (int i = 0; i < nb + 1; i += 2) {
+#pragma unroll
+        for (int cb = 0; cb < NCB; ++cb)
+#pragma unroll
+            for (int k4 = 0; k4 < KS; k4 += 4)
+                asm volatile("" : "+a"(wh[cb][k4]), "+a"(wh[cb][k4 + 1]), "+a"(wh[cb][k4 + 2]), "+a"(wh[cb][k4 + 3]), "+a"(wm[cb][k4]), "+a"(wm[cb][k4 + 1]),
+                             "+a"(wm[cb][k4 + 2]), "+a"(wm[cb][k4 + 3]));
+        tick(H0, i);
+        tick(H1, i + 1);
+    }
+#undef GAP_END
+}
+
+}
diff --git a/ranked-list-truncation_amd/csrc/gemm6s_kv.hip b/ranked-list-truncation_amd/csrc/gemm6s_kv.hip
--- /dev/null
+++ b/ranked-list-truncation_amd/csrc/gemm6s_kv.hip
@@ -0,0 +1,10 @@
+#include "gemm6s_kernel.h"
+
+int rlt_gemm6s_kv_launch(const Gemm6sArgs& g, const GemmPlan& p, rlt_gemm_dispatch* rec, hipStream_t st) {
+    if (p.d.epilogue != 4 || !p.d.tb || p.d.kchunk != 256 || p.d.narrow || !g.kv_img || g.kv_ntile <= 0) return RLT_E_ARG;
+    const int rc = rlt_allow_lds(gemm6s_kernel<8, 4, true, 4>, p.lds_bytes);
+    if (rc) return rc;
+    *rec = p.d;
+    hipLaunchKernelGGL((gemm6s_kernel<8, 4, true, 4>), dim3(p.grid_x), dim3(p.wg), p.lds_bytes, st, g);
+    return 0;
+}
diff --git a/ranked-list-truncation_amd/csrc/gemm_plan.h b/ranked-list-truncation_amd/csrc/gemm_plan.h
--- a/ranked-list-truncation_amd/csrc/gemm_plan.h
+++ b/ranked-list-truncation_amd/csrc/gemm_plan.h
@@ -15,6 +15,9 @@
 };
 GemmPlan gemm_plan(const GemmCall& c);
 
+#define RLT_GEMM_KV_IMAGES 0x100
+#define RLT_GEMM_INTERNAL_FLAGS RLT_GEMM_KV_IMAGES
+
 struct GemmFamily { int bm, bn, wg; size_t lds; };
 constexpr GemmFamily GEMM_FAMILY[] = {
     {0, 0, 0, 0},
diff --git a/ranked-list-truncation_amd/csrc/gemm_plan.hip b/ranked-list-truncation_amd/csrc/gemm_plan.hip
--- a/ranked-list-truncation_amd/csrc/gemm_plan.hip
+++ b/ranked-list-truncation_amd/csrc/gemm_plan.hip
@@ -119,7 +119,8 @@
         p.tiles_m = nstream; p.tiles_n = npanel;
         p.grid_x = npanel * nstream; p.grid_z = 1;
         p.lds_bytes = K == 256 ? GEMM6S_LDS_K256 : GEMM6S_LDS_K128;
-        p.d = rlt_gemm_dispatch{family, 0, tb, 1, 0, 1, K, 0, bits_in ? 3 : bits_out ? 2 : relu ? 1 : 0, narrow};
+        const bool kv_images = (c.flags & RLT_GEMM_KV_IMAGES) && K == 256 && N == 768 && tb && M % 64 == 0 && !relu && !bits_in && !bits_out;
+        p.d = rlt_gemm_dispatch{family, 0, tb, 1, 0, 1, K, 0, kv_images ? 4 : bits_in ? 3 : bits_out ? 2 : relu ? 1 : 0, narrow};
         return p;
     }
     p.tiles_m = rlt_cdiv(M, f.bm); p.tiles_n = rlt_cdiv(N, f.bn);
diff --git a/ranked-list-truncation_amd/csrc/path.hip b/ranked-list-truncation_amd/csrc/path.hip
--- a/ranked-list-truncation_amd/csrc/path.hip
+++ b/ranked-list-truncation_amd/csrc/path.hip
@@ -1,4 +1,5 @@
-#include "common.h"
+#include "attention_common.h"
+#include "gemm6s.h"
 #include <stdio.h>
 #include <stdlib.h>
 
@@ -275,8 +276,19 @@
     const int T = (int)d.T;
     const uint32_t s_attn = drop_p > 0.f ? seeds[0] : 0u, s_ln1 = drop_p > 0.f ? seeds[1] : 0u,
                    s_ffn = drop_p > 0.f ? seeds[2] : 0u, s_ln2 = drop_p > 0.f ? seeds[3] : 0u;
-    RLT_TRY(gemm(0, 1, T, 3 * E, E, x, E, w->in_proj_weight, E, s.qkv, 3 * E, w->in_proj_bias, 0, nullptr, ws, ws_bytes, stream));
-    RLT_TRY(rlt_list_attention_fwd(s.qkv, S, B, H, d.HD, drop_p, s_attn, s.att, s.lse, s.images, s.images_bytes, RLT_PRECISION_DEFAULT, stream));
+    rlt_attention_plan ap;
+    RLT_TRY(rlt_list_attention_plan(S, B, H, d.HD, drop_p, s.images != nullptr, RLT_PRECISION_DEFAULT, &ap));
+    int images_written = 0;
+    if (ap.fwd == RLT_ATTN_X6H_PIPE && rlt_aligned16(s.images) && s.images_bytes >= ap.images_bytes) {
+        RLT_TRY(rlt_gemm_inproj_kv_images(T, E, B, x, w->in_proj_weight, w->in_proj_bias, s.qkv, s.images, ws, ws_bytes, &images_written, stream));
+    } else {
+        RLT_TRY(gemm(0, 1, T, 3 * E, E, x, E, w->in_proj_weight, E, s.qkv, 3 * E, w->in_proj_bias, 0, nullptr, ws, ws_bytes, stream));
+    }
+    if (images_written) {
+        RLT_TRY(rlt_list_attention_fwd_images_ready(s.qkv, S, B, H, d.HD, drop_p, s_attn, s.att, s.lse, s.images, s.images_bytes, stream));
+    } else {
+        RLT_TRY(rlt_list_attention_fwd(s.qkv, S, B, H, d.HD, drop_p, s_attn, s.att, s.lse, s.images, s.images_bytes, RLT_PRECISION_DEFAULT, stream));
+    }
     RLT_TRY(gemm(0, 1, T, E, E, s.att, E, w->out_proj_weight, E, s.proj, E, w->out_proj_bias, 0, nullptr, ws, ws_bytes, stream));
     RLT_TRY(rlt_add_layernorm_fwd(x, s.proj, w->norm1_weight, w->norm1_bias, T, E, eps, drop_p, s_ln1, s.h1, s.st1, stream));
     if (d.bits) {
diff --git a/ranked-list-truncation_amd/rlt_hip/build.py b/ranked-list-truncation_amd/rlt_hip/build.py
--- a/ranked-list-truncation_amd/rlt_hip/build.py
+++ b/ranked-list-truncation_amd/rlt_hip/build.py
@@ -11,7 +11,8 @@
          "-ffp-contract=off"]
 FILE_FLAGS = {"attention6.hip": ["-fno-slp-vectorize"], "attention6n.hip": ["-fno-slp-vectorize", "-mllvm", "-amdgpu-mfma-vgpr-form"],
               "attention6h.hip": ["-fno-slp-vectorize", "-mllvm", "-amdgpu-mfma-vgpr-form"],
-              "lstm6w.hip": ["-fno-slp-vectorize"], "gemm6s.hip": ["-fno-slp-vectorize"]}
+              "lstm6w.hip": ["-fno-slp-vectorize"], "gemm6s.hip": ["-fno-slp-vectorize"],
+              "gemm6s_kv.hip": ["-fno-slp-vectorize"]}
 
 
 def sources():
```
